# ieellee/uLLSAM

Hardware: AMD Instinct MI355X
Metric: images/s end-to-end (ViT+LLM+mask) 1024^2 (higher is better)
Workload: dtype bf16; 1 GPU; uLLSAM mask path (app.py:580-645): SAM ViT-H + InternLM2-7b-shaped prefill S=1081 + prompt encoder + mask decoder + x4 upsample/threshold, 1 point prompt/image, batch 4/GPU; batch_per_gpu=4, global_batch=4, seq_len=1081, vit_linears=bf16

## Files before the change

### include/ullsam_hip.h

```cpp
#ifndef ULLSAM_HIP_H
#define ULLSAM_HIP_H
#ifdef __cplusplus
extern "C" {
#endif

#define ULLSAM_DT_F32 0
#define ULLSAM_DT_BF16 1
#define ULLSAM_ACT_NONE 0
#define ULLSAM_ACT_GELU 1
#define ULLSAM_ACT_RELU 2
#define ULLSAM_ACT_SWIGLU 3

#define ULLSAM_ABI_VERSION 14

const char* ullsam_last_error_string(void);
int ullsam_abi_version(void);
int ullsam_device_count(void);
int ullsam_set_gemm_variant(int variant);
int ullsam_set_gemm_tuning(int key, int value);
int ullsam_set_attn_variant(int variant);
int ullsam_set_attn_debug(void* stamps);

#define ULLSAM_ACT_SPLITK_OK 256
int ullsam_gemm(int dtype, const void* A, long lda, const void* W, long ldw, void* C, long ldc, int out_f32,
                const float* bias, const float* residual, long ldr, int res_row_mod, int act, int M, int N, int K,
                void* workspace, long ws_bytes, void* stream);

int ullsam_gemm_qkv_rope(int dtype, const void* A, long lda, const void* W, long ldw, const float* bias, int B, int S, int K, int KVH,
                         int G, const int* pos, const float* cos_tab, const float* sin_tab, int tab_rows, void* q_out, void* k_cache,
                         void* v_cache, int cap, int cache_pos0, void* workspace, long ws_bytes, void* stream);

int ullsam_gemm_rmsnorm(const float* x, long ldx, const float* norm_w, float eps, const void* W, long ldw, void* C, long ldc, int out_f32,
                        const float* bias, const float* residual, long ldr, int act, int M, int N, int K, void* stream);
int ullsam_decode_qkv_rope(const void* a, const float* x, long ldx, const float* norm_w, float eps, const void* W, long ldw, const float* bias,
                           int B, int K, int KVH, int G, const int* pos, const float* cos_tab, const float* sin_tab, int tab_rows, void* q_out,
                           void* k_cache, void* v_cache, int cap, int cache_pos0, void* stream);

int ullsam_train_matmul(const float* A, const float* B, float* C, int M, int N, int K, int batch, long a_b, long a_m, long a_k, long b_b,
                        long b_k, long b_n, long c_b, long c_m, long c_n, int accumulate, void* stream);
int ullsam_train_matmul_bf16(const float* A, const float* B, float* C, int M, int N, int K, int batch, long a_b, long a_m, long a_k, long b_b,
                             long b_k, long b_n, long c_b, long c_m, long c_n, int accumulate, void* stream);
int ullsam_train_matmul_heads(const float* A, const float* B, float* C, int M, int N, int K, int outer, int heads, long a_o, long a_h, int a_hdiv, long a_m, long a_k,
                              long b_o, long b_h, int b_hdiv, long b_k, long b_n, long c_o, long c_h, long c_m, long c_n, int accumulate, int bf16, int tri, void* stream);
int ullsam_train_matmul_splitk(const float* A, const float* B, float* C, int M, int N, int K, int batch, long a_b, long a_m, long a_k, long b_b,
                               long b_k, long b_n, long c_b, long c_m, long c_n, int accumulate, int ksplit, float* partial, void* stream);
int ullsam_train_set_matmul_mfma(int on);
int ullsam_train_set_matmul_vec(int on);
int ullsam_train_colsum(const float* x, float* out, long rows, int cols, long ld, float* partial, void* stream);
int ullsam_train_ln_bwd(const float* x, const float* w, const float* dy, float* dx, float* dw, float* db, long rows, int D, float eps, float* ws, void* stream);
int ullsam_train_act(const float* x, const float* dy, float* out, long n, int kind, void* stream);
int ullsam_train_scale_shift(const float* x, const float* s, const float* t, const float* dy, float* out, float* ds, float* dt, long n, float* partial, void* stream);
int ullsam_train_attention(const float* q, const float* k, const float* v, const float* dout, float* out, float* dq, float* dk, float* dv,
                           int B, int H, int groups, int hd, int Sq, int Sk, int causal, const int* key_mask, long q_bs, long q_ts, long q_hs,
                           long k_bs, long k_ts, long k_hs, long v_bs, long v_ts, long v_hs, long o_bs, long o_ts, long o_hs, float scale,
                           const float* bias_h, const float* bias_w, float* dbias_h, float* dbias_w, int kw, void* stream);
int ullsam_train_col2im3x3(const float* dcols, float* dx, int B, int H, int W, int C, void* stream);
int ullsam_train_attn_rows(float* S, float* dP, const float* bias_h, const float* bias_w, float* dbias_h, float* dbias_w, const int* key_mask,
                           int B, int H, int Sq, int Sk, int kw, int causal, int have_p, void* stream);
int ullsam_train_set_rows_reg(int on);
int ullsam_train_rmsnorm_bwd(const float* x, const float* w, const float* dy, float* dx, float* dw_rows, long rows, int D, float eps, void* stream);
int ullsam_train_rope(const float* x, const int* pos, const float* cos_tab, const float* sin_tab, float* out, long tokens, int heads, int hd,
                      int tab_rows, int adjoint, void* stream);
int ullsam_train_swiglu(const float* g, const float* u, const float* dy, float* out, float* dg, float* du, long n, void* stream);
int ullsam_train_resize_bwd(const float* dout, float* din, long planes, int ih, int iw, int oh, int ow, void* stream);
int ullsam_train_seg_loss(const float* x, const float* t, float* sums, float* losses, int P, long npix, float smooth, float* partial, void* stream);
int ullsam_train_seg_loss_bwd(const float* x, const float* t, const float* sums, const float* gscale, float* dx, int P, long npix, float smooth, void* stream);
int ullsam_train_cross_entropy(const float* logits, long ld, const long long* labels, float* lse, float* loss_rows, float* out2, long rows, int V, void* stream);
int ullsam_train_cross_entropy_bwd(const float* logits, long ld, const long long* labels, const float* lse, const float* out2, const float* gscale, float* dlogits,
                                   long ldx, long rows, int V, void* stream);
int ullsam_train_cross_entropy_bwd_bf16(const float* logits, long ld, const long long* labels, const float* lse, const float* out2, const float* gscale,
                                        void* dlog, long ldd, void* dlogT, long ldt, long rows, int V, void* stream);
int ullsam_train_embedding_bwd(const float* dx, long ldx, const int* sorted_ids, const int* order, const int* skip, long rows, int D, int V, int padding_idx,
                               void* table_grad, int out_dtype, void* stream);
int ullsam_train_index_add_rows(const float* src, const int* idx, float* dst, long rows, int C, int nrows_dst, void* stream);

int ullsam_norm(const void* in, int in_dtype, long in_stride, void* out, int out_dtype, long out_stride, const float* w,
                const float* b, long rows, int D, float eps, int rms, int act, const float* post_scale,
                const float* post_shift, void* stream);
int ullsam_set_norm_variant(int v);

int ullsam_norm_fanout(const float* in, long rows, int D, const float* w, const float* b, float eps, float* out_f32, void* out_c,
                       void* out_c_pe, int c_dtype, const float* pe, long pe_rows, void* stream);

int ullsam_vit_attention(int dtype, const void* qkv, void* out, const void* rel_h, const void* rel_w, const void* qkv_bias,
                         int B, int heads, int hd, int grid_h, int grid_w, int window, void* stream);

int ullsam_causal_attention(int dtype, const void* q, const void* k, const void* v, void* out, const int* key_mask, int B,
                            int H, int KVH, int hd, int Sq, int Sk, int k_cap, int q_pos0, void* stream);

int ullsam_naive_attention(int dtype, const void* q, const void* k, const void* v, void* out, const int* key_mask, int B,
                           int H, int KVH, int hd, int Sq, int Sk, long q_bs, long q_ts, long q_hs, long k_bs, long k_ts,
                           long k_hs, long v_bs, long v_ts, long v_hs, long o_bs, long o_ts, long o_hs, float scale,
                           void* stream);

int ullsam_decode_attention(const void* q, const void* kc, const void* vc, const int* key_mask, void* out, int B, int H, int KVH,
                            int hd, int Sk, int cap, float scale, float* workspace, int nsplit, void* stream);

int ullsam_fewkeys_attention(const float* q, const float* k, const float* v, float* out, int B, int H, int hd, int Sq,
                             int Sk, float scale, long q_batch_stride, void* stream);

int ullsam_tok2img_attention(int kv_dtype, const float* q, const void* k, const void* v, float* out, int P, int H, int hd, int T,
                             int N, long k_batch_stride, long v_batch_stride, float scale, float* workspace, int nsplit,
                             void* stream);

int ullsam_patch_im2col(int dtype, const float* pixels, void* out, int B, int C, int Hs, int Ws, int S, int patch,
                        const float* mean, const float* stdv, void* stream);
int ullsam_im2col3x3(int dtype, const void* in, void* out, int B, int H, int W, int C, void* stream);
int ullsam_add_cast(const void* a, int a_dtype, long a_rows, const float* b, long b_rows, void* out, int out_dtype,
                    long rows, int cols, void* stream);
int ullsam_transpose_f32(const float* in, float* out, int B, int R, int C, void* stream);
int ullsam_transpose_to_bf16(int in_dtype, const void* in, void* out, int R, int C, int Rp, void* stream);
int ullsam_cast_transpose_bf16(const float* in, void* out_rm, void* out_t, float* colsum_out, float* colsum_ws, int R, int C, int Rp, void* stream);
int ullsam_pixel_shuffle_ln(int dtype, const float* in_nhwc, void* out, const float* w, const float* b, int B, int H, int W,
// ... 201 lines not shown
```

### ullsam_amd/_lib.py

```python
from __future__ import annotations

import ctypes as C
import os

_HERE = os.path.dirname(os.path.abspath(__file__))
LIB_PATH = os.environ.get("ULLSAM_HIP_LIB") or os.path.join(_HERE, "lib", "libullsam_hip.so")

ABI_VERSION = 14

_lib = None

vp, i32, i64, f32 = C.c_void_p, C.c_int, C.c_long, C.c_float

SIGNATURES = {
    "ullsam_gemm": [i32, vp, i64, vp, i64, vp, i64, i32, vp, vp, i64, i32, i32, i32, i32, i32, vp, i64, vp],
    "ullsam_gemm_qkv_rope": [i32, vp, i64, vp, i64, vp, i32, i32, i32, i32, i32, vp, vp, vp, i32, vp, vp, vp, i32, i32, vp, i64, vp],
    "ullsam_gemm_rmsnorm": [vp, i64, vp, f32, vp, i64, vp, i64, i32, vp, vp, i64, i32, i32, i32, i32, vp],
    "ullsam_decode_qkv_rope": [vp, vp, i64, vp, f32, vp, i64, vp, i32, i32, i32, i32, vp, vp, vp, i32, vp, vp, vp, i32, i32, vp],
    "ullsam_train_matmul": [vp, vp, vp, i32, i32, i32, i32] + [i64] * 9 + [i32, vp],
    "ullsam_train_matmul_bf16": [vp, vp, vp, i32, i32, i32, i32] + [i64] * 9 + [i32, vp],
    "ullsam_train_matmul_splitk": [vp, vp, vp, i32, i32, i32, i32] + [i64] * 9 + [i32, i32, vp, vp],
    "ullsam_train_matmul_heads": [vp, vp, vp, i32, i32, i32, i32, i32, i64, i64, i32, i64, i64, i64, i64, i32, i64, i64, i64, i64, i64, i64, i32, i32, i32, vp],
    "ullsam_train_colsum": [vp, vp, i64, i32, i64, vp, vp],
    "ullsam_train_ln_bwd": [vp, vp, vp, vp, vp, vp, i64, i32, f32, vp, vp],
    "ullsam_train_act": [vp, vp, vp, i64, i32, vp],
    "ullsam_train_scale_shift": [vp, vp, vp, vp, vp, vp, vp, i64, vp, vp],
    "ullsam_train_attention": [vp] * 8 + [i32] * 7 + [vp] + [i64] * 12 + [f32, vp, vp, vp, vp, i32, vp],
    "ullsam_train_col2im3x3": [vp, vp, i32, i32, i32, i32, vp],
    "ullsam_train_attn_rows": [vp, vp, vp, vp, vp, vp, vp, i32, i32, i32, i32, i32, i32, i32, vp],
    "ullsam_train_rmsnorm_bwd": [vp, vp, vp, vp, vp, i64, i32, f32, vp],
    "ullsam_train_rope": [vp, vp, vp, vp, vp, i64, i32, i32, i32, i32, vp],
    "ullsam_train_swiglu": [vp, vp, vp, vp, vp, vp, i64, vp],
    "ullsam_train_resize_bwd": [vp, vp, i64, i32, i32, i32, i32, vp],
    "ullsam_train_seg_loss": [vp, vp, vp, vp, i32, i64, f32, vp, vp],
    "ullsam_train_seg_loss_bwd": [vp, vp, vp, vp, vp, i32, i64, f32, vp],
    "ullsam_train_cross_entropy": [vp, i64, vp, vp, vp, vp, i64, i32, vp],
    "ullsam_train_cross_entropy_bwd": [vp, i64, vp, vp, vp, vp, vp, i64, i64, i32, vp],
    "ullsam_train_cross_entropy_bwd_bf16": [vp, i64, vp, vp, vp, vp, vp, i64, vp, i64, i64, i32, vp],
    "ullsam_train_embedding_bwd": [vp, i64, vp, vp, vp, i64, i32, i32, i32, vp, i32, vp],
    "ullsam_train_index_add_rows": [vp, vp, vp, i64, i32, i32, vp],
    "ullsam_norm": [vp, i32, i64, vp, i32, i64, vp, vp, i64, i32, f32, i32, i32, vp, vp, vp],
    "ullsam_norm_fanout": [vp, i64, i32, vp, vp, f32, vp, vp, vp, i32, vp, i64, vp],
    "ullsam_vit_attention": [i32, vp, vp, vp, vp, vp, i32, i32, i32, i32, i32, i32, vp],
    "ullsam_causal_attention": [i32, vp, vp, vp, vp, vp, i32, i32, i32, i32, i32, i32, i32, i32, vp],
    "ullsam_naive_attention": [i32, vp, vp, vp, vp, vp, i32, i32, i32, i32, i32, i32] + [i64] * 12 + [f32, vp],
    "ullsam_fewkeys_attention": [vp, vp, vp, vp, i32, i32, i32, i32, i32, f32, i64, vp],
    "ullsam_decode_attention": [vp, vp, vp, vp, vp, i32, i32, i32, i32, i32, i32, f32, vp, i32, vp],
    "ullsam_tok2img_attention": [i32, vp, vp, vp, vp, i32, i32, i32, i32, i32, i64, i64, f32, vp, i32, vp],
    "ullsam_patch_im2col": [i32, vp, vp, i32, i32, i32, i32, i32, i32, vp, vp, vp],
    "ullsam_im2col3x3": [i32, vp, vp, i32, i32, i32, i32, vp],
    "ullsam_add_cast": [vp, i32, i64, vp, i64, vp, i32, i64, i32, vp],
    "ullsam_transpose_f32": [vp, vp, i32, i32, i32, vp],
    "ullsam_transpose_to_bf16": [i32, vp, vp, i32, i32, i32, vp],
    "ullsam_cast_transpose_bf16": [vp, vp, vp, vp, vp, i32, i32, i32, vp],
    "ullsam_pixel_shuffle_ln": [i32, vp, vp, vp, vp, i32, i32, i32, i32, f32, vp],
    "ullsam_pixel_unshuffle": [vp, vp, i32, i32, i32, i32, vp],
    "ullsam_scan_image_tokens": [vp, vp, vp, i32, i32, C.c_longlong, vp],
    "ullsam_embed_tokens": [i32, vp, vp, vp, vp, vp, i32, i32, i32, i32, i64, vp],
    "ullsam_gather_rows": [vp, vp, vp, i32, i32, i32, i32, vp],
    "ullsam_rope_split": [i32, vp, vp, vp, vp, vp, vp, vp, i32, i32, i32, i32, i32, i32, i32, i32, vp],
    "ullsam_argmax": [vp, vp, i32, i64, i64, vp],
    "ullsam_sample_topk_topp": [vp, vp, i32, i64, i64, f32, i32, f32, vp, C.c_ulonglong, vp, vp, vp, vp, vp],
    "ullsam_small_linear": [vp, i64, vp, vp, vp, i64, vp, i64, i32, i32, i32, i32, vp],
    "ullsam_i2t_block": [vp, i64, vp, i64, vp, vp, vp, vp, vp, vp, vp, vp, f32, vp, i64, vp, vp, vp, i32, i32, i32, f32, vp],
    "ullsam_kv_proj": [vp, vp, vp, vp, vp, vp, vp, vp, i64, vp],
    "ullsam_up2_hyper_masks": [vp, vp, vp, vp, vp, i32, i32, i32, i32, vp],
    "ullsam_dec_tok_attn": [vp] * 14 + [f32, vp, vp, i32, i32, i32, i32, vp],
    "ullsam_dec_tok_mlp": [vp] * 10 + [f32] + [vp] * 6 + [f32] + [vp] * 4 + [i32, i32, i32, vp],
    "ullsam_dec_heads": [vp, vp, vp, vp, vp, i32, i32, i32, i32, i32, vp],
    "ullsam_concat_token_rows": [vp, i32, vp, i32, vp, i32, i32, vp],
    "ullsam_up1_ln_gelu": [vp, vp, vp, vp, vp, f32, vp, i64, vp],
    "ullsam_skinny_linear": [vp, i64, vp, vp, vp, i64, vp, i64, i32, i32, i32, i32, vp],
    "ullsam_sparse_embed": [vp, vp, vp, vp, vp, vp, i32, i32, i32, i32, f32, f32, vp],
    "ullsam_dense_pe": [vp, vp, i32, i32, i32, vp],
    "ullsam_mask_downscale": [vp, vp, i32, i32, i32, i32, i32, i32] + [vp] * 10 + [vp],
    "ullsam_hyper_masks": [i32, vp, vp, vp, i32, i32, i32, i32, i32, vp],
    "ullsam_resize_bilinear": [vp, i64, i32, i32, i32, vp, vp, i32, i32, i32, f32, vp],
    "ullsam_mask_iou_counts": [vp, vp, vp, i32, i64, vp],
    "ullsam_stability_score": [vp, i64, i64, f32, f32, vp, vp, vp],
    "ullsam_mask_to_box": [vp, i64, i32, i32, vp, vp],
    "ullsam_rle_pack": [vp, i64, i32, i32, vp, vp, vp, vp],
    "ullsam_rle_emit": [vp, vp, i64, i32, i32, vp, vp, vp],
    "ullsam_amg_postprocess": [vp, vp, i64] + [i32] * 11 + [f32, f32, vp, vp, vp, vp, vp, vp],
    "ullsam_nms_mask": [vp, i32, f32, vp, vp],
    "ullsam_threshold_u8": [vp, vp, i64, f32, vp],
    "ullsam_rle_to_mask": [vp, vp, i64, i32, i32, vp, vp, vp],
    "ullsam_label_regions": [vp, i64, i32, i32, i32, vp, vp],
    "ullsam_remove_small_regions": [vp, vp, i64, i32, i32, i32, i32, vp, i64, vp, vp],
    "ullsam_rle_paint_labels": [vp, vp, vp, i64, i32, i32, vp, vp, vp],
    "ullsam_label_stats": [vp, i64, i32, i32, vp, vp, vp],
    "ullsam_label_compact": [vp, vp, vp, i64, i32, vp, vp, vp, vp, vp, vp],
    "ullsam_label_remap": [vp, vp, i64, i32, i32, vp, vp],
    "ullsam_label_overlap": [vp, vp, i32, i32, i32, i32, vp, vp, vp],
    "ullsam_resize_nearest_i32": [vp, i64, i32, i32, i32, i32, i32, i32, i32, i32, vp, i64, vp],
    "ullsam_mosaic_seams": [vp, i32, i32, i32, vp, i64, vp, i32, i32, vp, vp, i64, i32, vp, vp, vp],
    "ullsam_mosaic_union": [vp, vp, i64, vp, i64, i64, i64, vp, vp, vp],
    "ullsam_mosaic_stats": [vp, i32, i32, i32, vp, i64, vp, i32, vp, i32, i32, vp, vp, vp, vp],
    "ullsam_mosaic_compact": [vp, vp, vp, i64, i32, vp, vp, vp, vp, vp],
    "ullsam_mosaic_paste": [vp, i32, i32, i32, vp, i64, vp, i32, vp, i32, i32, vp, vp],
# ... 95 lines not shown
```

### ullsam_amd/csrc/gemm.hip

```cpp
#include "common.h"
#include <type_traits>

struct GemmArgs {
    const void* A;
    const void* W;
    void* C;
    const float* bias;
    const float* residual;
    int M, N, K;
    long lda, ldw, ldc, ldr;
    int res_row_mod;
    int act;
    int out_f32;
    int vec_ok;
    int tiles_m, tiles_n;
    int full_tiles, ksplit;
    float* ws;
    size_t ws_bytes;
    const int* rope_pos; const float* rope_cos; const float* rope_sin; void* rope_q; void* rope_k; void* rope_v;
    int rope_S, rope_KVH, rope_G, rope_cap, rope_pos0, rope_rows;
    const float* row_scale;
    const float* col_scale;
    unsigned long long* dbg;
    const float* norm_x; const float* norm_w; float norm_eps; long ldx;
    int group_m;
};

#ifndef ULLSAM_RING_ASM_DMA
#define ULLSAM_RING_ASM_DMA 1
#endif
static constexpr bool g_asm_dma = ULLSAM_RING_ASM_DMA != 0;
static int g_split_tail = 1;
static int g_gemm_variant = 0;
static int g_dbg = 0;
static int g_auto_mask = 7;
static int g_group_m = 4;

template <typename T>
__device__ __forceinline__ Frag<T> lds_frag(const char* tile, int row, int ks, int g);
template <>
__device__ __forceinline__ Frag<bf16> lds_frag<bf16>(const char* tile, int row, int ks, int g) {
    const int c = (ks * 4 + g) ^ (row & 7);
    return load_frag(reinterpret_cast<const bf16*>(tile + row * 128 + (c << 4)));
}
template <>
__device__ __forceinline__ Frag<float> lds_frag<float>(const char* tile, int row, int ks, int g) {
    (void)ks;
    const int c0 = (2 * g) ^ (row & 7), c1 = (2 * g + 1) ^ (row & 7);
    const float4 a = *reinterpret_cast<const float4*>(tile + row * 128 + (c0 << 4));
    const float4 b = *reinterpret_cast<const float4*>(tile + row * 128 + (c1 << 4));
    Frag<float> f;
    f.v[0] = a.x; f.v[1] = a.y; f.v[2] = a.z; f.v[3] = a.w;
    f.v[4] = b.x; f.v[5] = b.y; f.v[6] = b.z; f.v[7] = b.w;
    return f;
}

template <typename OutT>
__device__ __forceinline__ void store_row8(OutT* dst, const float* v, int n_valid, bool vec);
template <>
__device__ __forceinline__ void store_row8<float>(float* dst, const float* v, int n_valid, bool vec) {
    if (vec && n_valid == 8) {
        *reinterpret_cast<float4*>(dst) = make_float4(v[0], v[1], v[2], v[3]);
        *reinterpret_cast<float4*>(dst + 4) = make_float4(v[4], v[5], v[6], v[7]);
    } else {
        for (int e = 0; e < n_valid; ++e) dst[e] = v[e];
    }
}
template <>
__device__ __forceinline__ void store_row8<bf16>(bf16* dst, const float* v, int n_valid, bool vec) {
    if (vec && n_valid == 8) {
        bf16x8_t o;
#pragma unroll
        for (int e = 0; e < 8; ++e) o[e] = (bf16)v[e];
        *reinterpret_cast<bf16x8_t*>(dst) = o;
    } else {
        for (int e = 0; e < n_valid; ++e) dst[e] = (bf16)v[e];
    }
}


template <typename T, typename OutT, int BM, int NTHREADS, int BN = 128, int EMODE = 0, bool RING16 = false>
__device__ __forceinline__ void epilogue_rows(const GemmArgs& p, const float* Cs, int m0, int n0, int tn, int tid) {
    constexpr int TPR = BN / 8;
    constexpr int RPP = NTHREADS / TPR;
    constexpr int PASSES = (BM + RPP - 1) / RPP;
    constexpr bool RAGGED = BM % RPP != 0;
    static_assert(NTHREADS % TPR == 0, "threads per pass must cover whole rows");
    if (RAGGED && tid >= NTHREADS) return;
    OutT* C = reinterpret_cast<OutT*>(p.C);
    if (p.act == 3) {
#pragma unroll
        for (int pass = 0; pass < PASSES; ++pass) {
            const int row = pass * RPP + tid / TPR;
            const int t = tid % TPR;
            const int grp = t >> 4, j0 = (t & 15) * 4;
            const int gm = m0 + row;
            if (gm >= p.M) continue;
            const float4 g = *reinterpret_cast<const float4*>(Cs + row * BN + grp * 128 + j0);
            const float4 u = *reinterpret_cast<const float4*>(Cs + row * BN + grp * 128 + 64 + j0);
            float4 o;
            if constexpr (RING16) {
                o = make_float4(g.x * __builtin_amdgcn_rcpf(1.0f + __expf(-g.x)) * u.x, g.y * __builtin_amdgcn_rcpf(1.0f + __expf(-g.y)) * u.y,
                                g.z * __builtin_amdgcn_rcpf(1.0f + __expf(-g.z)) * u.z, g.w * __builtin_amdgcn_rcpf(1.0f + __expf(-g.w)) * u.w);
            } else {
                o = make_float4(silu_f(g.x) * u.x, silu_f(g.y) * u.y, silu_f(g.z) * u.z, silu_f(g.w) * u.w);
            }
            OutT* dst = C + (size_t)gm * p.ldc + (size_t)tn * (BN / 2) + grp * 64 + j0;
// ... 491 lines not shown
#pragma unroll
    for (int e = 0; e < 4; ++e) { first[e] = odd ? recv[e] : lo[e]; second[e] = odd ? hi[e] : recv[e]; }
}

template <typename T, int EMODE = 0>
static int launch_gemm_v3_impl(GemmArgs a, hipStream_t stream) {
    static PerDeviceOnce attr_set;
    if (attr_set.first()) {
        (void)hipFuncSetAttribute(reinterpret_cast<const void*>(gemm256_kernel<T, EMODE>), hipFuncAttributeMaxDynamicSharedMemorySize, 131072);
    }
    a.tiles_m = (a.M + 255) / 256;
    a.tiles_n = (a.N + 255) / 256;
    const int T_ = a.tiles_m * a.tiles_n;
    const int nk = a.K / (128 / (int)sizeof(T));
    const int tail = T_ % 256;
    a.full_tiles = T_;
    a.ksplit = 1;
    if (g_split_tail && a.ws && T_ > 256 && tail > 0 && tail <= 64 && nk >= 64) {
        int S = 256 / tail;
        if (S > 8) S = 8;
        if (S > nk / 8) S = nk / 8;
        if (S >= 2 && (size_t)tail * S * 262144 <= a.ws_bytes) {
            a.full_tiles = T_ - tail;
            a.ksplit = S;
        }
    }
    gemm256_kernel<T, EMODE><<<dim3(a.full_tiles + (T_ - a.full_tiles) * a.ksplit), dim3(512), 131072, stream>>>(a);
    ULLSAM_LAUNCH_CHECK();
    if (a.ksplit > 1) {
        const int tail_tiles = T_ - a.full_tiles;
        if (tail_tiles * a.ksplit <= 128) gemm256_tail_reduce_kernel<T, 4, 128, EMODE><<<dim3(tail_tiles * 64), dim3(128), 0, stream>>>(a);
        else gemm256_tail_reduce_kernel<T, 16, 256, EMODE><<<dim3(tail_tiles * 16), dim3(256), 0, stream>>>(a);
        ULLSAM_LAUNCH_CHECK();
    }
    return 0;
}
template <typename T>
static int launch_gemm_v3(GemmArgs a, hipStream_t stream) {
    if (a.act == 4) return launch_gemm_v3_impl<T, 1>(a, stream);
    return launch_gemm_v3_impl<T, 0>(a, stream);
}

__device__ __forceinline__ void glds16_sbase(const char* base, unsigned int off, unsigned int lds_addr) {
    unsigned int keep;
    asm volatile("s_mov_b32 %0, m0\n\ts_mov_b32 m0, %3\n\ts_nop 0\n\tglobal_load_lds_dwordx4 %1, %2\n\ts_mov_b32 m0, %0"
                 : "=&s"(keep) : "v"(off), "s"(base), "s"(lds_addr) : "memory");
}

template <int MI0, int MI1, int NTW, bool STAMP = false, int EMODE = 0>
__global__ __launch_bounds__(512) void gemm_ring8_kernel(GemmArgs p) {
    extern __shared__ __attribute__((aligned(16))) char smem[];
    const unsigned long long t_entry = STAMP ? __builtin_amdgcn_s_memtime() : 0ull;
    typedef bf16 T;
    constexpr int BM = 16 * (MI0 + MI1), BN = 64 * NTW, MI = MI0 > MI1 ? MI0 : MI1;
    constexpr int PA = BM / 16, PB = BN / 16;
    constexpr int ASZ = BM * 64, STG = ASZ + BN * 64;
    static_assert(PA >= 8 && PA <= 24 && PB >= 8 && PB <= 24, "piece assignment below: one to three pieces per wave and operand");
    if constexpr (EMODE == 2) {
        p.K /= (int)gridDim.y;
        p.A = reinterpret_cast<const char*>(p.A) + (size_t)blockIdx.y * p.K * 2;
        p.W = reinterpret_cast<const char*>(p.W) + (size_t)blockIdx.y * p.K * 2;
        p.C = reinterpret_cast<float*>(p.C) + (size_t)blockIdx.y * p.M * p.ldc;
    }

    const int nblk = p.full_tiles;
    const int bid = blockIdx.x;
    const int q8 = nblk >> 3, r8 = nblk & 7, xcd = bid & 7;
    const int swz = (xcd < r8 ? xcd * (q8 + 1) : r8 * (q8 + 1) + (xcd - r8) * q8) + (bid >> 3);
    const int GM = p.group_m;
    const int width = GM * p.tiles_n;
    const int group = swz / width;
    const int first_m = group * GM;
    const int gsize = min(p.tiles_m - first_m, GM);
    const int tm = first_m + (swz % width) % gsize;
    const int tn = (swz % width) / gsize;
    const int m0 = tm * BM, n0 = tn * BN;

    const int tid = threadIdx.x, lane = tid & 63;
    const int wave = __builtin_amdgcn_readfirstlane(tid >> 6);
    const int wm = wave >> 2, wn = wave & 3, grp = wave >> 2;
    const int g4 = lane >> 4, mm = lane & 15;

    const char* a_base = reinterpret_cast<const char*>(p.A) + (size_t)m0 * p.lda * 2;
    const char* b_base = reinterpret_cast<const char*>(p.W) + (size_t)n0 * p.ldw * 2;
    const int na = (PA - wave + 7) / 8, nb = (PB - wave + 7) / 8;
    static_assert(NTW == 4 || NTW == 5, "epilogue layouts below: four sub-tiles in two pairs, optionally a fifth on its own");
    constexpr int WW = 16 * NTW;
    const int perm = EMODE == 1 ? 2 : p.out_f32 ? 0 : (p.act == 3 ? 2 : 1);
    auto w_row = [&](int R) {
        const int wb = R / WW, q = R - wb * WW, j = q >> 4, r = q & 15;
        if (perm == 1) return j < 4 ? WW * wb + 32 * (j >> 1) + 8 * (r >> 2) + 4 * (j & 1) + (r & 3) : WW * wb + 64 + r;
        if (perm == 2) return 128 * (wb >> 1) + 64 * (j >> 1) + 32 * (wb & 1) + 8 * (r >> 2) + 4 * (j & 1) + (r & 3);
        return R;
    };
    unsigned int a_off[3], b_off[3];
#pragma unroll
    for (int i = 0; i < 3; ++i) {
        const int row = (wave + 8 * i) * 16 + (lane >> 2);
        const int c = (lane & 3) ^ ((row >> 2) & 2);
        a_off[i] = (unsigned int)((size_t)(min(m0 + row, p.M - 1) - m0) * p.lda * 2) + (c << 4);
        b_off[i] = (unsigned int)((size_t)(min(n0 + w_row(row), p.N - 1) - n0) * p.ldw * 2) + (c << 4);
    }
    const int st1 = p.K >> 5;

    const int mi = wm == 0 ? MI0 : MI1;
    const int row_w = wm == 0 ? 0 : MI0 * 16;
    f32x4 acc[MI][NTW];
#pragma unroll
    for (int i = 0; i < MI; ++i)
#pragma unroll
        for (int j = 0; j < NTW; ++j) acc[i][j] = (f32x4){0.f, 0.f, 0.f, 0.f};

    auto stage = [&](int s) {
        char* base = smem + (s & 3) * STG;
        const char* ak = a_base + (size_t)s * 64;
        const char* bk = b_base + (size_t)s * 64;
#pragma unroll
        for (int i = 0; i < 3; ++i) {
            if (i < na) __builtin_amdgcn_global_load_lds(GLB_PTR(ak + a_off[i]), LDS_PTR(base + (wave + 8 * i) * 1024), 16, 0, 0);
            if (i < nb) __builtin_amdgcn_global_load_lds(GLB_PTR(bk + b_off[i]), LDS_PTR(base + ASZ + (wave + 8 * i) * 1024), 16, 0, 0);
        }
    };
    auto frag = [&](const char* tile, int row) -> Frag<T> {
        return load_frag(reinterpret_cast<const T*>(tile + row * 64 + ((g4 ^ ((row >> 2) & 2)) << 4)));
    };
    const int npc = na + nb;
    auto wait_one_left = [&]() {
        if (npc == 4) asm volatile("s_waitcnt vmcnt(4)" ::: "memory");
        else if (npc == 2) asm volatile("s_waitcnt vmcnt(2)" ::: "memory");
        else if (npc == 5) asm volatile("s_waitcnt vmcnt(5)" ::: "memory");
        else if (npc == 6) asm volatile("s_waitcnt vmcnt(6)" ::: "memory");
        else asm volatile("s_waitcnt vmcnt(3)" ::: "memory");
    };

    const bool has_bias = p.bias && p.act != 3 && EMODE == 0;
    char* const bias_lds = smem + (st1 & 3) * STG;
    auto bias_dma = [&]() __attribute__((always_inline)) {
        if (has_bias && wave < (BN * 4 + 1023) / 1024) {
            const int c = min(n0 + wave * 256 + lane * 4, p.N - 4);
            __builtin_amdgcn_global_load_lds(GLB_PTR(p.bias + c), LDS_PTR(bias_lds + wave * 1024), 16, 0, 0);
        }
    };
    stage(0);
    if (1 < st1) { stage(1); wait_one_left(); }
    else asm volatile("s_waitcnt vmcnt(0)" ::: "memory");
    __builtin_amdgcn_s_barrier();
    if (grp == 1) __builtin_amdgcn_s_barrier();
    auto stamp = [&](int kk) {
        if (STAMP && p.dbg && (tid & 255) == 0) p.dbg[((size_t)bid * 2 + grp) * 4 + kk] = __builtin_amdgcn_s_memtime();
    };
    auto stamp16 = [&](int kk) {
        if (STAMP && p.dbg && (tid & 255) == 0) p.dbg[(1 << 19) + ((size_t)bid * 2 + grp) * 8 + kk] = __builtin_amdgcn_s_memtime();
    };
    stamp(0);
    {
        auto body = [&](int s, auto NA_c, auto NB_c, auto MORE_c) __attribute__((always_inline)) {
            constexpr int NA = decltype(NA_c)::value, NB = decltype(NB_c)::value;
            constexpr bool MORE = decltype(MORE_c)::value;
            const char* Ab = smem + (s & 3) * STG;
            const char* Bb = Ab + ASZ;
            Frag<T> a8[MI], b[NTW];
            {
                char* base = smem + ((s + 2) & 3) * STG;
                const char* ak = a_base + (size_t)(s + 2) * 64;
                const char* bk = b_base + (size_t)(s + 2) * 64;
                auto request = [&](int qi) __attribute__((always_inline)) {
                    const int i = qi >> 1;
                    if (g_asm_dma) {
                        if (MORE && !(qi & 1) && i < NA) glds16_sbase(ak, a_off[i], (unsigned int)(uintptr_t)LDS_PTR(base + (wave + 8 * i) * 1024));
                        if (MORE && (qi & 1) && i < NB) glds16_sbase(bk, b_off[i], (unsigned int)(uintptr_t)LDS_PTR(base + ASZ + (wave + 8 * i) * 1024));
                    } else {
                        if (MORE && !(qi & 1) && i < NA) __builtin_amdgcn_global_load_lds(GLB_PTR(ak + a_off[i]), LDS_PTR(base + (wave + 8 * i) * 1024), 16, 0, 0);
                        if (MORE && (qi & 1) && i < NB) __builtin_amdgcn_global_load_lds(GLB_PTR(bk + b_off[i]), LDS_PTR(base + ASZ + (wave + 8 * i) * 1024), 16, 0, 0);
                    }
                    __builtin_amdgcn_sched_barrier(0);
                };
                int qi = 0;
                request(qi++);
#pragma unroll
                for (int r = 0; r < NTW + MI; ++r) {
                    if (r < NTW) b[r] = frag(Bb, wn * (16 * NTW) + r * 16 + mm);
                    else if ((r - NTW) < MI1 || (r - NTW) < mi) a8[r - NTW] = frag(Ab, row_w + (r - NTW) * 16 + mm);
                    __builtin_amdgcn_sched_barrier(0);
                    if ((r % 3) == 2 && qi < 6) request(qi++);
                }
#pragma unroll
                for (; qi < 6; ++qi) request(qi);
            }
            if constexpr (!MORE) asm volatile("s_waitcnt vmcnt(0)" ::: "memory");
            else if constexpr (NA + NB == 4) asm volatile("s_waitcnt vmcnt(4)" ::: "memory");
            else if constexpr (NA + NB == 5) asm volatile("s_waitcnt vmcnt(5)" ::: "memory");
            else if constexpr (NA + NB == 6) asm volatile("s_waitcnt vmcnt(6)" ::: "memory");
            else if constexpr (NA + NB == 3) asm volatile("s_waitcnt vmcnt(3)" ::: "memory");
            else asm volatile("s_waitcnt vmcnt(2)" ::: "memory");
            __builtin_amdgcn_sched_barrier(0);
            __builtin_amdgcn_s_barrier();
            __builtin_amdgcn_s_setprio(1);
#pragma unroll
            for (int i = 0; i < MI; ++i)
                if (i < MI1 || i < mi) {
#pragma unroll
                    for (int j = 0; j < NTW; ++j) mma16(b[j], a8[i], acc[i][j]);
                }
            __builtin_amdgcn_s_setprio(0);
            __builtin_amdgcn_sched_barrier(0);
            __builtin_amdgcn_s_barrier();
        };
        auto run = [&](auto NA_c, auto NB_c) __attribute__((always_inline)) {
            int s = 0;
            for (; s + 2 < st1; ++s) body(s, NA_c, NB_c, std::true_type{});
            bias_dma();
            for (; s < st1; ++s) body(s, NA_c, NB_c, std::false_type{});
        };
        constexpr int NA_LO = PA / 8, NA_HI = (PA + 7) / 8, NB_LO = PB / 8, NB_HI = (PB + 7) / 8;
        if (NA_HI != NA_LO && na == NA_HI) {
            if (NB_HI != NB_LO && nb == NB_HI) run(std::integral_constant<int, NA_HI>{}, std::integral_constant<int, NB_HI>{});
            else run(std::integral_constant<int, NA_HI>{}, std::integral_constant<int, NB_LO>{});
        } else {
            if (NB_HI != NB_LO && nb == NB_HI) run(std::integral_constant<int, NA_LO>{}, std::integral_constant<int, NB_HI>{});
            else run(std::integral_constant<int, NA_LO>{}, std::integral_constant<int, NB_LO>{});
        }
    }
    if (grp == 0) __builtin_amdgcn_s_barrier();
    stamp(1);
    float bv[4 * NTW];
#pragma unroll
    for (int e = 0; e < 4 * NTW; ++e) bv[e] = 0.f;
    if (has_bias) {
#pragma unroll
        for (int t = 0; t < NTW; ++t) {
            const int col = wn * WW + ((p.out_f32 || t == 4) ? 16 * t + 4 * g4 : 32 * (t >> 1) + 8 * g4 + 4 * (t & 1));
            const float4 x = *reinterpret_cast<const float4*>(bias_lds + col * 4);
            bv[4 * t] = x.x; bv[4 * t + 1] = x.y; bv[4 * t + 2] = x.z; bv[4 * t + 3] = x.w;
        }
    }

    {
        const bool odd = mm & 1;
        const int row0 = m0 + row_w + mm;
        const int rowp = row0 & ~1;
        const bool direct = p.vec_ok && (p.N & 7) == 0 && (p.M & 1) == 0 && (p.out_f32 || !p.residual);
        auto gst = [&](void* ptr, u32x4 v) __attribute__((always_inline)) { *reinterpret_cast<u32x4*>(ptr) = v; };
        if constexpr (EMODE == 1) {
            const int slot = (n0 >> 7) + (wn >> 1), d = 32 * (wn & 1) + 8 * g4;
            const int gs = p.rope_G + 2, kv = slot / gs, g = slot - kv * gs;
            const bool live = slot < p.rope_KVH * gs;
            const bool rotate = g != gs - 1;
            float bl[8], bh[8];
// ... 172 lines not shown
                if (perm == 1) return j < 4 ? WW * wn + 32 * (j >> 1) + 8 * g4 + 4 * (j & 1) : WW * wn + 64 + 4 * g4;
                if (perm == 2) return 128 * (wn >> 1) + 64 * (j >> 1) + 32 * (wn & 1) + 8 * g4 + 4 * (j & 1);
                return WW * wn + 16 * j + 4 * g4;
            };
            auto staged = [&](auto half_c) __attribute__((always_inline)) {
                constexpr int half = decltype(half_c)::value;
                constexpr int ROWS = 16 * (half == 0 ? MI0 : MI1);
                constexpr int NT_E = (512 / (BN / 8)) * (BN / 8);
                __syncthreads();
                if (wm == half) {
#pragma unroll
                    for (int i = 0; i < (half == 0 ? MI0 : MI1); ++i)
#pragma unroll
                        for (int j = 0; j < NTW; ++j)
                            *reinterpret_cast<float4*>(Cs + (i * 16 + mm) * BN + ncol(j)) = make_float4(acc[i][j][0], acc[i][j][1], acc[i][j][2], acc[i][j][3]);
                }
                __syncthreads();
                if (p.out_f32) epilogue_rows<T, float, ROWS, NT_E, BN>(p, Cs, m0 + half * 16 * MI0, n0, tn, tid);
                else epilogue_rows<T, T, ROWS, NT_E, BN, 0, true>(p, Cs, m0 + half * 16 * MI0, n0, tn, tid);
            };
            staged(std::integral_constant<int, 0>{});
            staged(std::integral_constant<int, 1>{});
        }
    }
    stamp(2);
    if (STAMP && p.dbg && (tid & 255) == 0) p.dbg[((size_t)bid * 2 + grp) * 4 + 3] = t_entry;
}

template <int MI0, int MI1, int NTW, int EMODE = 0>
static int launch_gemm_ring8(GemmArgs a, hipStream_t stream) {
    constexpr int BM = 16 * (MI0 + MI1), BN = 64 * NTW;
    constexpr int LDS = (4 * (BM + BN) * 64 > 16 * MI0 * BN * 4) ? 4 * (BM + BN) * 64 : 16 * MI0 * BN * 4;
    static_assert(LDS <= 163840, "160 KiB of LDS per CU");
    static PerDeviceOnce attr_set;
    if (attr_set.first()) {
        (void)hipFuncSetAttribute(reinterpret_cast<const void*>(gemm_ring8_kernel<MI0, MI1, NTW, false, EMODE>), hipFuncAttributeMaxDynamicSharedMemorySize, LDS);
        if constexpr (EMODE == 0) (void)hipFuncSetAttribute(reinterpret_cast<const void*>(gemm_ring8_kernel<MI0, MI1, NTW, true>), hipFuncAttributeMaxDynamicSharedMemorySize, LDS);
    }
    a.tiles_m = (a.M + BM - 1) / BM;
    a.tiles_n = (a.N + BN - 1) / BN;
    a.full_tiles = a.tiles_m * a.tiles_n;
    a.ksplit = 1;
    if constexpr (EMODE == 0) {
        if (a.dbg) {
            gemm_ring8_kernel<MI0, MI1, NTW, true><<<dim3(a.full_tiles), dim3(512), LDS, stream>>>(a);
            ULLSAM_LAUNCH_CHECK();
            return 0;
        }
    }
    gemm_ring8_kernel<MI0, MI1, NTW, false, EMODE><<<dim3(a.full_tiles), dim3(512), LDS, stream>>>(a);
    ULLSAM_LAUNCH_CHECK();
    return 0;
}
template <typename TO>
__global__ __launch_bounds__(256) void splitk_finish_kernel(const float* __restrict__ ws, TO* __restrict__ C, long ldc, const float* __restrict__ bias,
                                                            const float* __restrict__ residual, long ldr, int res_row_mod, int M, int N, int S) {
    const long q = (long)blockIdx.x * 256 + threadIdx.x, nq = N >> 2;
    if (q >= (long)M * nq) return;
    const int m = (int)(q / nq), c = (int)(q - (long)m * nq) * 4;
    const size_t plane = (size_t)M * N;
    const float* src = ws + (size_t)m * N + c;
    float4 v[8];
#pragma unroll
    for (int k = 0; k < 8; ++k) if (k < S) v[k] = *reinterpret_cast<const float4*>(src + k * plane);
    float4 s = v[0];
#pragma unroll
    for (int k = 1; k < 8; ++k) if (k < S) { s.x += v[k].x; s.y += v[k].y; s.z += v[k].z; s.w += v[k].w; }
    if (bias) { const float4 b = *reinterpret_cast<const float4*>(bias + c); s.x += b.x; s.y += b.y; s.z += b.z; s.w += b.w; }
    if (residual) {
        const int rr = res_row_mod > 0 ? m % res_row_mod : m;
        const float4 r = *reinterpret_cast<const float4*>(residual + (size_t)rr * ldr + c);
        s.x += r.x; s.y += r.y; s.z += r.z; s.w += r.w;
    }
    if constexpr (sizeof(TO) == 4) *reinterpret_cast<float4*>(C + (size_t)m * ldc + c) = s;
    else *reinterpret_cast<uint2*>(C + (size_t)m * ldc + c) = make_uint2(pack_bf16x2(s.x, s.y), pack_bf16x2(s.z, s.w));
}
template <int MI0, int MI1, int NTW>
static int launch_gemm_ring_splitk(const GemmArgs& a, int S, hipStream_t stream) {
    constexpr int BM = 16 * (MI0 + MI1), BN = 64 * NTW;
    constexpr int LDS = (4 * (BM + BN) * 64 > 16 * MI0 * BN * 4) ? 4 * (BM + BN) * 64 : 16 * MI0 * BN * 4;
    static PerDeviceOnce attr_set;
    if (attr_set.first()) (void)hipFuncSetAttribute(reinterpret_cast<const void*>(gemm_ring8_kernel<MI0, MI1, NTW, false, 2>), hipFuncAttributeMaxDynamicSharedMemorySize, LDS);
    GemmArgs b = a;
    b.C = a.ws; b.ldc = a.N; b.out_f32 = 1; b.bias = nullptr; b.residual = nullptr; b.act = 0; b.vec_ok = 1; b.dbg = nullptr;
    b.tiles_m = (a.M + BM - 1) / BM;
    b.tiles_n = (a.N + BN - 1) / BN;
    b.full_tiles = b.tiles_m * b.tiles_n;
    b.ksplit = 1;
    gemm_ring8_kernel<MI0, MI1, NTW, false, 2><<<dim3(b.full_tiles, S), dim3(512), LDS, stream>>>(b);
    ULLSAM_LAUNCH_CHECK();
    const long quads = (long)a.M * (a.N >> 2);
    if (a.out_f32) splitk_finish_kernel<float><<<dim3((unsigned)((quads + 255) / 256)), 256, 0, stream>>>(a.ws, static_cast<float*>(a.C), a.ldc, a.bias, a.residual, a.ldr, a.res_row_mod, a.M, a.N, S);
    else splitk_finish_kernel<bf16><<<dim3((unsigned)((quads + 255) / 256)), 256, 0, stream>>>(a.ws, static_cast<bf16*>(a.C), a.ldc, a.bias, a.residual, a.ldr, a.res_row_mod, a.M, a.N, S);
    ULLSAM_LAUNCH_CHECK();
    return 0;
}
static int g_ring_splitk = 1;
static int ring_splitk_plan(const GemmArgs& a, int* shape) {
    if (a.act != 0 || !a.vec_ok || !a.ws || (a.N & 7) != 0 || a.M < 1024 || a.N < 256 || a.dbg) return 0;
    const long t272 = (long)((a.M + 271) / 272) * ((a.N + 255) / 256), t256 = (long)((a.M + 255) / 256) * ((a.N + 255) / 256);
    const long t320 = a.N % 320 == 0 ? (long)((a.M + 255) / 256) * (a.N / 320) : 1l << 40;
    const double a272 = 1.0625 * t272, a256 = 1.0 * t256, a320 = 1.25 * t320;
    long t; if (a320 <= a272 && a320 <= a256) { t = t320; *shape = 8; } else if (a272 < a256) { t = t272; *shape = 9; } else { t = t256; *shape = 6; }
    if (t > 128) return 0;
    int S = (int)(256 / t); if (S > 8) S = 8;
    while (S >= 2 && (a.K % (64 * S) != 0 || a.K / S < 1280 || (size_t)S * a.M * a.N * 4 > a.ws_bytes)) --S;
    return (S >= 2 && S * t >= 224) ? S : 0;
}
#include "gemm_ring8p.h"
static int g_persist = 2;
static int cu_count() {
    static int n[32] = {};
    int d = 0;
    (void)hipGetDevice(&d);
    d &= 31;
    if (!n[d]) { int v = 0; if (hipDeviceGetAttribute(&v, hipDeviceAttributeMultiprocessorCount, d) != hipSuccess || v <= 0) v = 256; n[d] = v; }
    return n[d];
}
template <int BM, int BN, int NTW, int EMODE>
static bool ring_persist_ok(const GemmArgs& a) {
    if (!g_persist || a.N % BN != 0 || a.K % 128 != 0 || a.K < 384 || (a.dbg && !(g_dbg & 2))) return false;
    const long tiles = (long)((a.M + BM - 1) / BM) * (a.N / BN);
    if (tiles <= cu_count()) return false;
    if (((size_t)(a.M + BM) * a.lda + a.K) * 2 >= (1ull << 32) || ((size_t)a.N * a.ldw + a.K) * 2 >= (1ull << 32)) return false;
    if (EMODE == 1) return true;
    if (!(a.vec_ok && (a.N & 7) == 0 && (a.M & 1) == 0)) return false;
    if (!a.out_f32) return !a.residual && (a.act != 3 || NTW == 4);
    return a.act == 0;
}
template <int MI0, int MI1, int NTW, int EMODE = 0>
static int launch_ring(const GemmArgs& a, hipStream_t stream) {
    return ring_persist_ok<16 * (MI0 + MI1), 64 * NTW, NTW, EMODE>(a) ? launch_gemm_ring8p<MI0, MI1, NTW, EMODE>(a, stream, cu_count())
                                                                      : launch_gemm_ring8<MI0, MI1, NTW, EMODE>(a, stream);
}
static int launch_gemm_v6(const GemmArgs& a, hipStream_t stream) { return launch_ring<8, 8, 4>(a, stream); }
static int launch_gemm_v8(const GemmArgs& a, hipStream_t stream) { return launch_ring<8, 8, 5>(a, stream); }
static int launch_gemm_v9(const GemmArgs& a, hipStream_t stream) { return launch_ring<9, 8, 4>(a, stream); }
static int launch_gemm_ring_rope(const GemmArgs& a, hipStream_t stream, int force) {
    auto cost = [&](int bm) { const long t = (long)((a.M + bm - 1) / bm) * ((a.N + 255) / 256); return (double)((t + 255) / 256) * bm / 256.0; };
    const double c208 = cost(208), c256 = cost(256), c272 = cost(272);
    int pick = (c208 < c256 && c208 < c272) ? 208 : (c272 < c256 ? 272 : 256);
    if (force) pick = force;
    if (pick == 208) return launch_ring<7, 6, 4, 1>(a, stream);
    if (pick == 272) return launch_ring<9, 8, 4, 1>(a, stream);
    return launch_ring<8, 8, 4, 1>(a, stream);
}

typedef __attribute__((ext_vector_type(8))) int i32x8;
__device__ __forceinline__ int f8_swz(int row) { return (row & 6) | ((row >> 3) & 1); }
__device__ __forceinline__ i32x8 lds_frag8(const char* tile, int row, int g) {
    const int f = f8_swz(row);
    const int4 lo = *reinterpret_cast<const int4*>(tile + row * 128 + (((2 * g) ^ f) << 4));
    const int4 hi = *reinterpret_cast<const int4*>(tile + row * 128 + (((2 * g + 1) ^ f) << 4));
    return (i32x8){lo.x, lo.y, lo.z, lo.w, hi.x, hi.y, hi.z, hi.w};
}
__global__ __launch_bounds__(512) void gemm256f8_kernel(GemmArgs p) {
    extern __shared__ __attribute__((aligned(16))) char smem[];
    constexpr int STAGE = 65536;
    const int nblk = p.tiles_m * p.tiles_n;
    const int bid = blockIdx.x;
    const int q8 = nblk >> 3, r8 = nblk & 7, xcd = bid & 7;
    const int swz = (xcd < r8 ? xcd * (q8 + 1) : r8 * (q8 + 1) + (xcd - r8) * q8) + (bid >> 3);
    const int GM = 4;
    const int width = GM * p.tiles_n;
    const int group = swz / width;
    const int first_m = group * GM;
    const int gsize = min(p.tiles_m - first_m, GM);
    const int tm = first_m + (swz % width) % gsize;
    const int tn = (swz % width) / gsize;
    const int m0 = tm * 256, n0 = tn * 256;
    const int tid = threadIdx.x, lane = tid & 63;
    const int wave = __builtin_amdgcn_readfirstlane(tid >> 6);
    const int wm = wave >> 2, wn = wave & 3, grp = wave >> 2;
    const int g4 = lane >> 4, mm = lane & 15;

    const char* a_base = reinterpret_cast<const char*>(p.A) + (size_t)m0 * p.lda;
    const char* b_base = reinterpret_cast<const char*>(p.W) + (size_t)n0 * p.ldw;
    unsigned int a_off[4], b_off[4];
#pragma unroll
    for (int i = 0; i < 4; ++i) {
        const int row = (wave * 4 + i) * 8 + (lane >> 3);
        const int c = (lane & 7) ^ f8_swz(row);
        a_off[i] = (unsigned int)((size_t)(min(m0 + row, p.M - 1) - m0) * p.lda) + (c << 4);
        b_off[i] = (unsigned int)((size_t)(min(n0 + row, p.N - 1) - n0) * p.ldw) + (c << 4);
    }
    const int nk = p.K >> 7;
    f32x4 acc[8][4];
#pragma unroll
    for (int i = 0; i < 8; ++i)
#pragma unroll
        for (int j = 0; j < 4; ++j) acc[i][j] = (f32x4){0.f, 0.f, 0.f, 0.f};
    auto stage = [&](int buf, int kt) {
        char* base = smem + buf * STAGE;
        const char* ak = a_base + (size_t)kt * 128;
        const char* bk = b_base + (size_t)kt * 128;
#pragma unroll
        for (int i = 0; i < 4; ++i) {
            __builtin_amdgcn_global_load_lds(GLB_PTR(ak + a_off[i]), LDS_PTR(base + (wave * 4 + i) * 1024), 16, 0, 0);
            __builtin_amdgcn_global_load_lds(GLB_PTR(bk + b_off[i]), LDS_PTR(base + 32768 + (wave * 4 + i) * 1024), 16, 0, 0);
        }
    };
    const int one = 0x7f7f7f7f;
    stage(0, 0);
    asm volatile("s_waitcnt vmcnt(0)" ::: "memory");
    __builtin_amdgcn_s_barrier();
    if (grp == 1) __builtin_amdgcn_s_barrier();
    for (int kt = 0; kt < nk; ++kt) {
        const char* Ab = smem + (kt & 1) * STAGE;
        const char* Bb = Ab + 32768;
        i32x8 a[4], b[4];
        if (kt + 1 < nk) stage((kt + 1) & 1, kt + 1);
#pragma unroll
        for (int j = 0; j < 4; ++j) b[j] = lds_frag8(Bb, wn * 64 + j * 16 + mm, g4);
#pragma unroll
        for (int i = 0; i < 4; ++i) a[i] = lds_frag8(Ab, wm * 128 + i * 16 + mm, g4);
        __builtin_amdgcn_sched_barrier(0);
        __builtin_amdgcn_s_barrier();
        __builtin_amdgcn_s_setprio(1);
#pragma unroll
        for (int i = 0; i < 4; ++i)
#pragma unroll
            for (int j = 0; j < 4; ++j) acc[i][j] = __builtin_amdgcn_mfma_scale_f32_16x16x128_f8f6f4(a[i], b[j], acc[i][j], 0, 0, 0, one, 0, one);
        __builtin_amdgcn_s_setprio(0);
        __builtin_amdgcn_sched_barrier(0);
        __builtin_amdgcn_s_barrier();
#pragma unroll
        for (int i = 0; i < 4; ++i) a[i] = lds_frag8(Ab, wm * 128 + (4 + i) * 16 + mm, g4);
        asm volatile("s_waitcnt vmcnt(0)" ::: "memory");
        __builtin_amdgcn_sched_barrier(0);
        __builtin_amdgcn_s_barrier();
        __builtin_amdgcn_s_setprio(1);
#pragma unroll
        for (int i = 0; i < 4; ++i)
#pragma unroll
            for (int j = 0; j < 4; ++j) acc[4 + i][j] = __builtin_amdgcn_mfma_scale_f32_16x16x128_f8f6f4(a[i], b[j], acc[4 + i][j], 0, 0, 0, one, 0, one);
        __builtin_amdgcn_s_setprio(0);
        __builtin_amdgcn_sched_barrier(0);
        __builtin_amdgcn_s_barrier();
    }
    if (grp == 0) __builtin_amdgcn_s_barrier();

    float* Cs = reinterpret_cast<float*>(smem);
#pragma unroll
    for (int half = 0; half < 2; ++half) {
        __syncthreads();
        if (wm == half) {
#pragma unroll
            for (int i = 0; i < 8; ++i)
#pragma unroll
                for (int j = 0; j < 4; ++j)
#pragma unroll
                    for (int r = 0; r < 4; ++r) Cs[(i * 16 + 4 * g4 + r) * 256 + wn * 64 + j * 16 + mm] = acc[i][j][r];
        }
        __syncthreads();
        if (p.out_f32) epilogue_rows<bf16, float, 128, 512, 256, 2>(p, Cs, m0 + half * 128, n0, tn, tid);
        else epilogue_rows<bf16, bf16, 128, 512, 256, 2>(p, Cs, m0 + half * 128, n0, tn, tid);
    }
}

extern "C" int ullsam_gemm_fp8(const void* A8, long lda, const float* a_scale, const void* W8, long ldw, const float* w_scale, void* C,
                               long ldc, int out_f32, const float* bias, const float* residual, long ldr, int act, int M, int N, int K,
                               void* stream) {
    ULLSAM_CHECK(M > 0 && N > 0 && K > 0 && K % 128 == 0, "ullsam_gemm_fp8: K=%d must be a positive multiple of 128", K);
    ULLSAM_CHECK(((uintptr_t)A8 & 15) == 0 && ((uintptr_t)W8 & 15) == 0 && lda % 16 == 0 && ldw % 16 == 0, "ullsam_gemm_fp8: 16-byte aligned rows needed");
    ULLSAM_CHECK(a_scale && w_scale, "ullsam_gemm_fp8: scales are required");
    ULLSAM_CHECK(act >= 0 && act <= 2, "ullsam_gemm_fp8: bad act %d", act);
    GemmArgs a;
    a.A = A8; a.W = W8; a.C = C; a.bias = bias; a.residual = residual;
    a.M = M; a.N = N; a.K = K; a.lda = lda; a.ldw = ldw; a.ldc = ldc; a.ldr = ldr;
    a.res_row_mod = 0; a.act = act; a.out_f32 = out_f32;
    const int osz = out_f32 ? 4 : 2;
    bool vec = ((uintptr_t)C & 15) == 0 && (ldc * osz) % 16 == 0 && (N % 8 == 0);
    if (residual) vec = vec && ((uintptr_t)residual & 15) == 0 && (ldr % 4 == 0);
    a.group_m = 4;
    a.vec_ok = vec ? 1 : 0;
    a.ws = nullptr; a.ws_bytes = 0; a.ksplit = 1;
    a.row_scale = a_scale; a.col_scale = w_scale; a.dbg = nullptr;
    a.tiles_m = (M + 255) / 256; a.tiles_n = (N + 255) / 256; a.full_tiles = a.tiles_m * a.tiles_n;
    static PerDeviceOnce attr_set;
    if (attr_set.first()) (void)hipFuncSetAttribute(reinterpret_cast<const void*>(gemm256f8_kernel), hipFuncAttributeMaxDynamicSharedMemorySize, 131072);
    gemm256f8_kernel<<<dim3(a.full_tiles), dim3(512), 131072, reinterpret_cast<hipStream_t>(stream)>>>(a);
    ULLSAM_LAUNCH_CHECK();
    return 0;
}

extern "C" int ullsam_set_gemm_tuning(int key, int value) {
    if (key == 0 && value >= 1 && value <= 1024) { g_group_m = value; return 0; }
    if (key == 1 && value >= 0 && value <= 7) { g_auto_mask = value; return 0; }
    if (key == 2 && (value == 0 || value == 2)) { g_persist = value; return 0; }
    if (key == 3 && value >= 0 && value <= 2) { g_ring_splitk = value; return 0; }
    ullsam_set_error("ullsam_set_gemm_tuning: unknown key %d / bad value %d", key, value);
    return -1;
}
extern "C" int ullsam_set_gemm_variant(int v) {
    g_gemm_variant = v & 15; g_split_tail = (v & 64) ? 0 : 1; g_dbg = (v >> 15) & 3;
    return 0;
}

template <typename T, int EMODE = 0>
static int launch_gemm(GemmArgs a, hipStream_t stream) {
    static PerDeviceOnce attr_set;
    if (attr_set.first()) {
        (void)hipFuncSetAttribute(reinterpret_cast<const void*>(gemm128_kernel<T, EMODE>), hipFuncAttributeMaxDynamicSharedMemorySize, 65536);
    }
    const int T_ = a.tiles_m * a.tiles_n;
    const int C_ = 512;
    a.full_tiles = T_;
    a.ksplit = 1;
    const int nk = a.K / (128 / (int)sizeof(T));
    const int tail = T_ % C_;
    if (g_split_tail && a.ws && T_ > C_ && tail > 0 && tail <= C_ / 2 && nk >= 128) {
        int S = C_ / tail;
        if (S > 16) S = 16;
        if (S > nk / 4) S = nk / 4;
        if (S >= 2 && (size_t)tail * S * 65536 <= a.ws_bytes) {
            a.full_tiles = T_ - tail;
            a.ksplit = S;
        }
    }
    const int grid = a.full_tiles + (T_ - a.full_tiles) * a.ksplit;
    gemm128_kernel<T, EMODE><<<dim3(grid), dim3(256), 65536, stream>>>(a);
    ULLSAM_LAUNCH_CHECK();
    if (a.ksplit > 1) {
        gemm_tail_reduce_kernel<T, EMODE><<<dim3((T_ - a.full_tiles) * 4), dim3(256), 0, stream>>>(a);
        ULLSAM_LAUNCH_CHECK();
    }
    return 0;
}

#ifndef ULLSAM_SKINNY_NT
#define ULLSAM_SKINNY_NT 1
#endif
__device__ __forceinline__ uint4 load_w16(const bf16* ptr) {
#if ULLSAM_SKINNY_NT
    const u32x4 v = __builtin_nontemporal_load(reinterpret_cast<const u32x4*>(ptr));
    return make_uint4(v[0], v[1], v[2], v[3]);
#else
    return *reinterpret_cast<const uint4*>(ptr);
#endif
}
template <bool W8> struct SkinnyW { using elem = bf16; using vec = uint4; };
template <> struct SkinnyW<true> { using elem = unsigned char; using vec = uint2; };
__device__ __forceinline__ uint2 load_w16(const unsigned char* ptr) {
#if ULLSAM_SKINNY_NT
    const u32x2 v = __builtin_nontemporal_load(reinterpret_cast<const u32x2*>(ptr));
    return make_uint2(v[0], v[1]);
#else
    return *reinterpret_cast<const uint2*>(ptr);
#endif
}
__device__ __forceinline__ uint4 widen_w(const uint4 w) { return w; }
__device__ __forceinline__ uint4 widen_w(const uint2 w) {
    typedef __bf16 bf16x2_t __attribute__((ext_vector_type(2)));
    uint4 o;
    o.x = __builtin_bit_cast(unsigned int, (bf16x2_t)__builtin_amdgcn_cvt_scalef32_pk_bf16_fp8(w.x, 1.0f, false));
    o.y = __builtin_bit_cast(unsigned int, (bf16x2_t)__builtin_amdgcn_cvt_scalef32_pk_bf16_fp8(w.x, 1.0f, true));
    o.z = __builtin_bit_cast(unsigned int, (bf16x2_t)__builtin_amdgcn_cvt_scalef32_pk_bf16_fp8(w.y, 1.0f, false));
    o.w = __builtin_bit_cast(unsigned int, (bf16x2_t)__builtin_amdgcn_cvt_scalef32_pk_bf16_fp8(w.y, 1.0f, true));
    return o;
}

__device__ __forceinline__ void bf16x8_to_f32(const uint4 u, float (&o)[8]) {
    const unsigned int d[4] = {u.x, u.y, u.z, u.w};
#pragma unroll
    for (int j = 0; j < 4; ++j) { o[2 * j] = __uint_as_float(d[j] << 16); o[2 * j + 1] = __uint_as_float(d[j] & 0xffff0000u); }
}
__device__ __forceinline__ void dot2c(float& acc, const unsigned int a, const unsigned int b) {
    asm("v_dot2c_f32_bf16 %0, %1, %2" : "+v"(acc) : "v"(a), "v"(b));
}
__device__ __forceinline__ void dot_fence() { asm volatile("s_nop 4" ::: "memory"); }
template <int NV>
__device__ __forceinline__ float wave_sum_many(float (&v)[NV]) {
    static_assert(NV == 16 || NV == 32, "");
// ... 386 lines not shown
        const int gs = p.rope_G + 2, kv = slot / gs, g = slot - kv * gs;
        const int b = m / p.rope_S, sq = m - b * p.rope_S;
        bf16* dst;
        float o1 = x1, o2 = x2;
        if (g == gs - 1) {
            dst = reinterpret_cast<bf16*>(p.rope_v) + (((long)b * p.rope_KVH + kv) * p.rope_cap + p.rope_pos0 + sq) * 128;
        } else {
            const int ps = min(max(p.rope_pos[m], 0), p.rope_rows - 1);
            const float* cp = p.rope_cos + (size_t)ps * 128 + d;
            const float* sp = p.rope_sin + (size_t)ps * 128 + d;
            o1 = x1 * cp[0] - x2 * sp[0];
            o2 = x2 * cp[64] + x1 * sp[64];
            dst = g == gs - 2 ? reinterpret_cast<bf16*>(p.rope_k) + (((long)b * p.rope_KVH + kv) * p.rope_cap + p.rope_pos0 + sq) * 128
                              : reinterpret_cast<bf16*>(p.rope_q) + (long)m * ((long)p.rope_KVH * p.rope_G * 128) + ((long)kv * p.rope_G + g) * 128;
        }
        dst[d] = (bf16)o1;
        dst[d + 64] = (bf16)o2;
        return;
    }
    const long n = n0 + r;
    if (n >= p.N) return;
    float v = total(tid, n);
    if (p.bias) v += p.bias[n];
    if (p.act == 1) v = gelu_erf(v);
    else if (p.act == 2) v = fmaxf(v, 0.f);
    if (p.residual) v += p.residual[(size_t)(p.res_row_mod > 0 ? m % p.res_row_mod : m) * p.ldr + n];
    if (p.out_f32) reinterpret_cast<float*>(p.C)[(size_t)m * p.ldc + n] = v;
    else reinterpret_cast<bf16*>(p.C)[(size_t)m * p.ldc + n] = (bf16)v;
}

template <bool W8 = false>
static int launch_gemm_skinny(const GemmArgs& a, hipStream_t stream) {
    const bool normed = a.norm_x != nullptr;
    if (normed && (a.M > 4 || a.K > 4096 || a.K % 2048 != 0 || a.ldx % 4 != 0)) { ullsam_set_error("skinny GEMM: the fused RMSNorm prologue needs M <= 4, K <= 4096, K %% 2048 == 0 (M=%d K=%d)", a.M, a.K); return -1; }
    if (a.act == 4 && (a.M > 4 || a.K % 2048 != 0 || a.N % 128 != 0)) { ullsam_set_error("skinny GEMM: the RoPE epilogue needs M <= 4, K %% 2048 == 0 (M=%d K=%d)", a.M, a.K); return -1; }
    if (a.act == 4 || (a.act != 3 && a.N <= 8192 && a.K % 2048 == 0)) {
        const dim3 g4((unsigned)((a.N + 3) / 4)), g8((unsigned)((a.N + 7) / 8));
        const size_t lds = normed ? (size_t)4 * a.K * 2 : 0;
        if (normed) gemm_skinny_ksplit_kernel<4, 8, true, W8><<<g8, 256, lds, stream>>>(a);
        else if (a.act == 4) gemm_skinny_ksplit_kernel<4, 8, false, W8><<<g8, 256, 0, stream>>>(a);
        else if (a.M > 4) gemm_skinny_ksplit_kernel<8, 4, false, W8><<<g4, 256, 0, stream>>>(a);
        else gemm_skinny_ksplit_kernel<4, 8, false, W8><<<g8, 256, 0, stream>>>(a);
        ULLSAM_LAUNCH_CHECK();
        return 0;
    }
    const int MM = a.M <= 4 ? 4 : 8;
    const size_t lds = (size_t)MM * a.K * 2;
    const long waves = a.act == 3 ? (long)a.N / 4 : ((long)a.N + 3) / 4;
    if (MM == 4 && (normed || a.act == 3) && waves >= 4096 && lds + 256 <= 64 * 1024) {
        static PerDeviceOnce cu_once; static int n_cu = 256;
        if (cu_once.first()) { int dev = 0; hipDeviceProp_t pr; if (hipGetDevice(&dev) == hipSuccess && hipGetDeviceProperties(&pr, dev) == hipSuccess && pr.multiProcessorCount > 0) n_cu = pr.multiProcessorCount; }
        const int n_wg = n_cu * 2;
        int W = 8; double best = 1e30;
        for (int w = 8; w >= 4; --w) {
            const long per = (long)n_wg * w, trips = (waves + per - 1) / per;
            const double waste = (double)(trips * per) / (double)waves;
            if (waste < best - 1e-9) { best = waste; W = w; }
        }
        if (normed) gemm_skinny_persist_kernel<true, W8><<<n_wg, W * 64, lds, stream>>>(a, (int)waves);
        else gemm_skinny_persist_kernel<false, W8><<<n_wg, W * 64, lds, stream>>>(a, (int)waves);
        ULLSAM_LAUNCH_CHECK();
        return 0;
    }
    const dim3 grid((unsigned)((waves + 3) / 4));
    static PerDeviceOnce attr4, attr8;
    if (normed) {
        gemm_skinny_kernel<4, true, W8><<<grid, 256, lds, stream>>>(a);
    } else if (MM == 4) {
        if (attr4.first()) { (void)hipFuncSetAttribute(reinterpret_cast<const void*>(gemm_skinny_kernel<4, false, W8>), hipFuncAttributeMaxDynamicSharedMemorySize, 159 * 1024); }
        gemm_skinny_kernel<4, false, W8><<<grid, 256, lds, stream>>>(a);
    } else {
        if (attr8.first()) { (void)hipFuncSetAttribute(reinterpret_cast<const void*>(gemm_skinny_kernel<8, false, W8>), hipFuncAttributeMaxDynamicSharedMemorySize, 159 * 1024); }
        gemm_skinny_kernel<8, false, W8><<<grid, 256, lds, stream>>>(a);
    }
    ULLSAM_LAUNCH_CHECK();
    return 0;
}

struct RopeEpilogue { const int* pos; const float* cos; const float* sin; void* q; void* k; void* v; int S, KVH, G, cap, pos0, rows; };
struct NormPrologue { const float* x; long ldx; const float* w; float eps; };

static int gemm_impl(int dtype, const void* A, long lda, const void* W, long ldw, void* C, long ldc, int out_f32,
                     const float* bias, const float* residual, long ldr, int res_row_mod, int act, int M, int N,
                     int K, void* workspace, long ws_bytes, void* stream, const RopeEpilogue* rope, const NormPrologue* norm = nullptr) {
    ULLSAM_CHECK(dtype == ULLSAM_DT_F32 || dtype == ULLSAM_DT_BF16, "ullsam_gemm: bad dtype %d", dtype);
    ULLSAM_CHECK(M > 0 && N > 0 && K > 0, "ullsam_gemm: empty problem M=%d N=%d K=%d", M, N, K);
    const int esz = dtype == ULLSAM_DT_F32 ? 4 : 2;
    const int bk = 128 / esz;
    ULLSAM_CHECK(K % bk == 0, "ullsam_gemm: K=%d must be a multiple of %d", K, bk);
    ULLSAM_CHECK(((uintptr_t)A & 15) == 0 && ((uintptr_t)W & 15) == 0, "ullsam_gemm: A/W must be 16-byte aligned");
    ULLSAM_CHECK((lda * esz) % 16 == 0 && (ldw * esz) % 16 == 0, "ullsam_gemm: lda/ldw rows must be 16-byte multiples");
    const bool split_ok = (act & 256) != 0;
    act &= 255;
    ULLSAM_CHECK(act >= 0 && act <= 4 && (act == 4) == (rope != nullptr), "ullsam_gemm: bad act %d", act);
    if (act == 3) ULLSAM_CHECK(N % 128 == 0 && !bias && !residual, "ullsam_gemm: swiglu needs N%%128==0, no bias/residual");
    GemmArgs a;
    a.rope_pos = nullptr; a.rope_cos = a.rope_sin = nullptr; a.rope_q = a.rope_k = a.rope_v = nullptr;
    a.rope_S = a.rope_KVH = a.rope_G = a.rope_cap = a.rope_pos0 = a.rope_rows = 0;
    if (rope) {
        a.rope_pos = rope->pos; a.rope_cos = rope->cos; a.rope_sin = rope->sin; a.rope_q = rope->q; a.rope_k = rope->k; a.rope_v = rope->v;
        a.rope_S = rope->S; a.rope_KVH = rope->KVH; a.rope_G = rope->G; a.rope_cap = rope->cap; a.rope_pos0 = rope->pos0; a.rope_rows = rope->rows;
    }
    a.norm_x = nullptr; a.norm_w = nullptr; a.norm_eps = 0.f; a.ldx = 0;
    if (norm) {
        ULLSAM_CHECK(norm->x && norm->w && ((uintptr_t)norm->x & 15) == 0 && ((uintptr_t)norm->w & 15) == 0 && norm->ldx % 4 == 0,
                     "ullsam_gemm: the RMSNorm prologue needs 16-byte aligned fp32 rows and weight");
        a.norm_x = norm->x; a.norm_w = norm->w; a.norm_eps = norm->eps; a.ldx = norm->ldx;
    }
    a.A = A; a.W = W; a.C = C; a.bias = bias; a.residual = residual;
    a.M = M; a.N = N; a.K = K;
    a.lda = lda; a.ldw = ldw; a.ldc = ldc; a.ldr = ldr;
    a.res_row_mod = res_row_mod; a.act = act; a.out_f32 = out_f32;
    const int osz = out_f32 ? 4 : esz;
    const int n_out = act == 3 ? N / 2 : N;
    bool vec = ((uintptr_t)C & 15) == 0 && (ldc * osz) % 16 == 0 && (n_out % 8 == 0);
    if (residual) vec = vec && ((uintptr_t)residual & 15) == 0 && (ldr % 4 == 0);
    a.vec_ok = vec ? 1 : 0;
    a.ws = reinterpret_cast<float*>(workspace);
    a.ws_bytes = workspace ? (size_t)ws_bytes : 0;
    a.group_m = g_group_m;
    a.row_scale = nullptr;
    a.col_scale = nullptr;
    a.dbg = (g_dbg && workspace && ws_bytes >= (56l << 20)) ? reinterpret_cast<unsigned long long*>(reinterpret_cast<char*>(workspace) + (48l << 20)) : nullptr;
    a.ksplit = 1;
    a.tiles_m = (M + 127) / 128;
    a.tiles_n = (N + 127) / 128;
    a.full_tiles = a.tiles_m * a.tiles_n;
    hipStream_t s = reinterpret_cast<hipStream_t>(stream);
    const int variant = g_gemm_variant;
    if ((variant == 0 || norm) && (act != 4 || (M <= 4 && K % 2048 == 0)) && dtype == ULLSAM_DT_BF16 && M <= 8 && K % 512 == 0 && lda % 8 == 0 && ldw % 8 == 0 &&
        (size_t)(M <= 4 ? 4 : 8) * K * 2 <= 144 * 1024 && (act != 3 || N % 128 == 0))
        return launch_gemm_skinny<false>(a, s);
    ULLSAM_CHECK(!norm, "ullsam_gemm: the RMSNorm prologue exists in the decode-step kernels only (bf16, M <= 4, K <= 4096; got M=%d K=%d)", M, K);
    const long t256 = (long)((M + 255) / 256) * ((N + 255) / 256);
    const double fill = (double)t256 / (double)(((t256 + 255) / 256) * 256);
    const long tail256 = t256 % 256;
    const bool v3_split = g_split_tail && workspace && t256 > 256 && tail256 > 0 && tail256 <= 64 && K >= 64 * bk;
    const bool big = M >= 1024 && N >= 256 && K >= 8 * bk && (act != 3 || N % 256 == 0);
    const bool bias_v4 = !bias || (N % 4 == 0 && ((uintptr_t)bias & 15) == 0);
    const bool ring_ok = dtype == ULLSAM_DT_BF16 && act <= 3 && K % 64 == 0 && K >= 128 && bias_v4 && (act != 3 || N % 256 == 0);
    if (act == 4 && dtype == ULLSAM_DT_BF16 && M >= 1024 && K % 64 == 0 && K >= 256 && (variant == 0 || variant == 6 || variant == 9 || variant == 10) &&
        (((uintptr_t)rope->q | (uintptr_t)rope->k | (uintptr_t)rope->v) & 15) == 0 && (!bias || ((uintptr_t)bias & 15) == 0))
        return launch_gemm_ring_rope(a, s, variant == 6 ? 256 : variant == 9 ? 272 : variant == 10 ? 208 : 0);
    if (variant == 6 || variant == 8 || variant == 9) {
        if (!ring_ok || (variant == 8 && act == 3)) { ullsam_set_error("ullsam_gemm: the ring kernels need bf16, K %% 64 == 0, K >= 128, no RoPE epilogue (256x320: no SwiGLU)"); return -1; }
        return variant == 6 ? launch_gemm_v6(a, s) : variant == 8 ? launch_gemm_v8(a, s) : launch_gemm_v9(a, s);
    }
    if (variant == 1) return a.act == 4 ? (dtype == ULLSAM_DT_F32 ? launch_gemm<float, 1>(a, s) : launch_gemm<bf16, 1>(a, s))
                                        : (dtype == ULLSAM_DT_F32 ? launch_gemm<float>(a, s) : launch_gemm<bf16>(a, s));
    if (variant == 3) {
        if (act == 3 && N % 256 != 0) { ullsam_set_error("ullsam_gemm: the 256x256 kernel's SwiGLU epilogue needs N %% 256 == 0"); return -1; }
        return dtype == ULLSAM_DT_F32 ? launch_gemm_v3<float>(a, s) : launch_gemm_v3<bf16>(a, s);
    }
    if (ring_ok && variant == 0 && (g_ring_splitk == 2 || (g_ring_splitk == 1 && split_ok))) {
        int shape = 0;
        const int S = ring_splitk_plan(a, &shape);
        if (S) return shape == 8 ? launch_gemm_ring_splitk<8, 8, 5>(a, S, s) : shape == 9 ? launch_gemm_ring_splitk<9, 8, 4>(a, S, s) : launch_gemm_ring_splitk<8, 8, 4>(a, S, s);
    }
    if (ring_ok && M >= 1024 && N >= 256 && K >= 256) {
        const double c256 = v3_split ? (double)(t256 / 256) + 0.5 : (double)((t256 + 255) / 256);
        const long t320 = (long)((M + 255) / 256) * (N / 320), t272 = (long)((M + 271) / 272) * ((N + 255) / 256);
        const double c320 = (N % 320 == 0 && act != 3 && (g_auto_mask & 2)) ? 1.25 * (double)((t320 + 255) / 256) : 1e9;
        const double c272 = (g_auto_mask & 4) ? 1.0625 * (double)((t272 + 255) / 256) : 1e9;
        if (c320 <= 0.96 * c256 || (act == 1 && c320 <= c256)) return launch_gemm_v8(a, s);
        if (c272 <= 0.96 * c256) return launch_gemm_v9(a, s);
        if ((g_auto_mask & 1) && big && fill >= 0.74 && !v3_split) return launch_gemm_v6(a, s);
    }
    const bool v3 = big && (fill >= 0.74 || v3_split);
    if (v3) return dtype == ULLSAM_DT_F32 ? launch_gemm_v3<float>(a, s) : launch_gemm_v3<bf16>(a, s);
    if (a.act == 4) return dtype == ULLSAM_DT_F32 ? launch_gemm<float, 1>(a, s) : launch_gemm<bf16, 1>(a, s);
    return dtype == ULLSAM_DT_F32 ? launch_gemm<float>(a, s) : launch_gemm<bf16>(a, s);
}

extern "C" int ullsam_gemm(int dtype, const void* A, long lda, const void* W, long ldw, void* C, long ldc, int out_f32,
                           const float* bias, const float* residual, long ldr, int res_row_mod, int act, int M, int N,
                           int K, void* workspace, long ws_bytes, void* stream) {
    ULLSAM_CHECK(act != 4, "ullsam_gemm: act 4 is ullsam_gemm_qkv_rope");
    return gemm_impl(dtype, A, lda, W, ldw, C, ldc, out_f32, bias, residual, ldr, res_row_mod, act, M, N, K, workspace, ws_bytes, stream, nullptr);
}

extern "C" int ullsam_gemm_rmsnorm(const float* x, long ldx, const float* norm_w, float eps, const void* W, long ldw, void* C, long ldc,
                                   int out_f32, const float* bias, const float* residual, long ldr, int act, int M, int N, int K, void* stream) {
    ULLSAM_CHECK(act != 4, "ullsam_gemm_rmsnorm: act 4 is ullsam_decode_qkv_rope");
    NormPrologue n{x, ldx, norm_w, eps};
    return gemm_impl(ULLSAM_DT_BF16, nullptr, K, W, ldw, C, ldc, out_f32, bias, residual, ldr, 0, act, M, N, K, nullptr, 0, stream, nullptr, &n);
}

extern "C" int ullsam_decode_qkv_rope(const void* a, const float* x, long ldx, const float* norm_w, float eps, const void* W, long ldw,
                                      const float* bias, int B, int K, int KVH, int G, const int* pos, const float* cos_tab,
                                      const float* sin_tab, int tab_rows, void* q_out, void* k_cache, void* v_cache, int cap, int cache_pos0,
                                      void* stream) {
    ULLSAM_CHECK(B > 0 && B <= 4 && KVH > 0 && G > 0 && tab_rows > 0 && K % 2048 == 0, "ullsam_decode_qkv_rope: B=%d (1..4) K=%d (%% 2048)", B, K);
    ULLSAM_CHECK(cache_pos0 + 1 <= cap, "ullsam_decode_qkv_rope: cache overflow (%d + 1 > %d)", cache_pos0, cap);
    RopeEpilogue r{pos, cos_tab, sin_tab, q_out, k_cache, v_cache, 1, KVH, G, cap, cache_pos0, tab_rows};
    NormPrologue n{x, ldx, norm_w, eps};
    const int N = KVH * (G + 2) * 128;
    return gemm_impl(ULLSAM_DT_BF16, norm_w ? nullptr : a, K, W, ldw, q_out, (long)KVH * G * 128, 0, bias, nullptr, 0, 0, 4, B, N, K, nullptr, 0,
                     stream, &r, norm_w ? &n : nullptr);
}

static int gemm_w8_impl(const char* who, const void* A, const NormPrologue* norm, const void* W8, long ldw, const float* w_scale, void* C, long ldc, int out_f32,
                        const float* bias, const float* residual, long ldr, int act, int M, int N, int K, void* stream, const RopeEpilogue* rope) {
    ULLSAM_CHECK(W8 && w_scale && C, "%s: null weights, scales or output", who);
    ULLSAM_CHECK(M > 0 && M <= 8 && N > 0 && K > 0 && K % 512 == 0, "%s: decode-step shapes only (1 <= M <= 8, K %% 512 == 0; got M=%d N=%d K=%d)", who, M, N, K);
    ULLSAM_CHECK((size_t)(M <= 4 ? 4 : 8) * K * 2 <= 144 * 1024, "%s: K=%d: the activation rows do not fit the LDS", who, K);
    ULLSAM_CHECK(act >= 0 && act <= 4 && (act == 4) == (rope != nullptr), "%s: bad act %d", who, act);
    ULLSAM_CHECK(((uintptr_t)W8 & 7) == 0 && ldw % 8 == 0 && ldw >= K, "%s: weight rows must be 8-byte aligned (ldw=%ld)", who, ldw);
    if (act == 3) ULLSAM_CHECK(N % 128 == 0 && !bias && !residual, "%s: swiglu needs N %% 128 == 0, no bias / residual", who);
    GemmArgs a{};
    if (rope) {
        a.rope_pos = rope->pos; a.rope_cos = rope->cos; a.rope_sin = rope->sin; a.rope_q = rope->q; a.rope_k = rope->k; a.rope_v = rope->v;
        a.rope_S = rope->S; a.rope_KVH = rope->KVH; a.rope_G = rope->G; a.rope_cap = rope->cap; a.rope_pos0 = rope->pos0; a.rope_rows = rope->rows;
    }
    if (norm) {
        ULLSAM_CHECK(norm->x && norm->w && ((uintptr_t)norm->x & 15) == 0 && ((uintptr_t)norm->w & 15) == 0 && norm->ldx % 4 == 0,
                     "%s: the RMSNorm prologue needs 16-byte aligned fp32 rows and weight", who);
        a.norm_x = norm->x; a.norm_w = norm->w; a.norm_eps = norm->eps; a.ldx = norm->ldx;
    } else {
        ULLSAM_CHECK(A && ((uintptr_t)A & 15) == 0, "%s: bf16 activations must be 16-byte aligned", who);
    }
    a.A = A; a.W = W8; a.C = C; a.bias = bias; a.residual = residual; a.col_scale = w_scale;
    a.M = M; a.N = N; a.K = K;
    a.lda = K; a.ldw = ldw; a.ldc = ldc; a.ldr = ldr;
    a.act = act; a.out_f32 = out_f32;
    a.group_m = g_group_m; a.ksplit = 1;
    return launch_gemm_skinny<true>(a, reinterpret_cast<hipStream_t>(stream));
}

extern "C" int ullsam_gemm_w8(const void* A, const float* x, long ldx, const float* norm_w, float eps, const void* W8, long ldw, const float* w_scale,
                              void* C, long ldc, int out_f32, const float* bias, const float* residual, long ldr, int act, int M, int N, int K,
                              void* stream) {
    ULLSAM_CHECK(act != 4, "ullsam_gemm_w8: act 4 is ullsam_decode_qkv_rope_w8");
    NormPrologue n{x, ldx, norm_w, eps};
    return gemm_w8_impl("ullsam_gemm_w8", norm_w ? nullptr : A, norm_w ? &n : nullptr, W8, ldw, w_scale, C, ldc, out_f32, bias, residual, ldr, act, M, N, K, stream, nullptr);
}

extern "C" int ullsam_decode_qkv_rope_w8(const void* a, const float* x, long ldx, const float* norm_w, float eps, const void* W8, long ldw,
                                         const float* w_scale, const float* bias, int B, int K, int KVH, int G, const int* pos, const float* cos_tab,
                                         const float* sin_tab, int tab_rows, void* q_out, void* k_cache, void* v_cache, int cap, int cache_pos0,
                                         void* stream) {
    ULLSAM_CHECK(B > 0 && B <= 4 && KVH > 0 && G > 0 && tab_rows > 0 && K > 0 && K % 2048 == 0, "ullsam_decode_qkv_rope_w8: B=%d (1..4) K=%d (%% 2048)", B, K);
    ULLSAM_CHECK(cache_pos0 >= 0 && cache_pos0 + 1 <= cap, "ullsam_decode_qkv_rope_w8: cache overflow (%d + 1 > %d)", cache_pos0, cap);
    ULLSAM_CHECK(pos && cos_tab && sin_tab && q_out && k_cache && v_cache, "ullsam_decode_qkv_rope_w8: null argument");
    RopeEpilogue r{pos, cos_tab, sin_tab, q_out, k_cache, v_cache, 1, KVH, G, cap, cache_pos0, tab_rows};
    NormPrologue n{x, ldx, norm_w, eps};
    const int N = KVH * (G + 2) * 128;
    return gemm_w8_impl("ullsam_decode_qkv_rope_w8", norm_w ? nullptr : a, norm_w ? &n : nullptr, W8, ldw, w_scale, q_out, (long)KVH * G * 128, 0, bias, nullptr, 0, 4, B, N, K,
                        stream, &r);
}

extern "C" int ullsam_gemm_qkv_rope(int dtype, const void* A, long lda, const void* W, long ldw, const float* bias, int B, int S, int K,
                                    int KVH, int G, const int* pos, const float* cos_tab, const float* sin_tab, int tab_rows, void* q_out,
                                    void* k_cache, void* v_cache, int cap, int cache_pos0, void* workspace, long ws_bytes, void* stream) {
    ULLSAM_CHECK(B > 0 && S > 0 && KVH > 0 && G > 0 && tab_rows > 0, "ullsam_gemm_qkv_rope: bad dims");
    ULLSAM_CHECK(cache_pos0 + S <= cap, "ullsam_gemm_qkv_rope: cache overflow (%d + %d > %d)", cache_pos0, S, cap);
    ULLSAM_CHECK(((uintptr_t)q_out & 15) == 0 && ((uintptr_t)k_cache & 15) == 0 && ((uintptr_t)v_cache & 15) == 0, "ullsam_gemm_qkv_rope: 16-byte aligned outputs needed");
    RopeEpilogue r{pos, cos_tab, sin_tab, q_out, k_cache, v_cache, S, KVH, G, cap, cache_pos0, tab_rows};
    const int N = KVH * (G + 2) * 128;
    return gemm_impl(dtype, A, lda, W, ldw, q_out, (long)KVH * G * 128, 0, bias, nullptr, 0, 0, 4, B * S, N, K, workspace, ws_bytes, stream, &r);
}
```

### ullsam_amd/csrc/gemm_ring8p.h

```cpp

__device__ __forceinline__ void blds16(u32x4 desc, unsigned int voff, unsigned int soff, unsigned int lds_addr) {
    unsigned int keep;
    asm volatile("s_mov_b32 %0, m0\n\ts_mov_b32 m0, %4\n\ts_nop 0\n\tbuffer_load_dwordx4 %1, %2, %3 offen lds\n\ts_mov_b32 m0, %0"
                 : "=&s"(keep) : "v"(voff), "s"(desc), "s"(soff), "s"(lds_addr) : "memory");
}
#pragma clang diagnostic push
#pragma clang diagnostic ignored "-Winline-asm"
template <int MOFF>
__device__ __forceinline__ void blds16_imm(u32x4 desc, unsigned int voff, unsigned int soff, unsigned int wave_lds_base) {
    asm volatile("s_add_i32 m0, %3, %4\n\ts_nop 0\n\tbuffer_load_dwordx4 %0, %1, %2 offen lds"
                 :: "v"(voff), "s"(desc), "s"(soff), "s"(wave_lds_base), "n"(MOFF) : "memory", "m0");
}
template <int N> __device__ __forceinline__ void wait_vmcnt() {
    static_assert(N >= 0 && N <= 6, "counted waits of the ring: one stage of a wave's pieces (at most three per operand) in flight");
    asm volatile("s_waitcnt vmcnt(%0)" :: "n"(N) : "memory");
}
#pragma clang diagnostic pop
__device__ __forceinline__ int fresh_lane() {
    int ln;
    asm volatile("v_mbcnt_lo_u32_b32 %0, -1, 0\n\tv_mbcnt_hi_u32_b32 %0, -1, %0" : "=v"(ln));
    return ln;
}
__device__ __forceinline__ u32x4 raw_desc(const void* base, unsigned int bytes) {
    const uintptr_t b = reinterpret_cast<uintptr_t>(base);
    u32x4 d;
    d[0] = __builtin_amdgcn_readfirstlane((unsigned int)b);
    d[1] = __builtin_amdgcn_readfirstlane((unsigned int)(b >> 32) & 0xffffu);
    d[2] = __builtin_amdgcn_readfirstlane(bytes);
    d[3] = 0x00020000u;
    return d;
}

template <int MI0, int MI1, int NTW, int EMODE = 0, bool STAMP = false>
__global__ __launch_bounds__(512) void gemm_ring8p_kernel(GemmArgs p) {
    extern __shared__ __attribute__((aligned(16))) char smem[];
    typedef bf16 T;
    constexpr int BM = 16 * (MI0 + MI1), BN = 64 * NTW;
    constexpr int PA = BM / 16, PB = BN / 16;
    constexpr int ASZ = BM * 64, STG = ASZ + BN * 64;
    constexpr int BIAS_LDS = 4 * STG;
    static_assert(PA >= 8 && PA <= 24 && PB >= 8 && PB <= 24, "piece assignment below: one to three pieces per wave and operand");
    static_assert(NTW == 4 || NTW == 5, "epilogue layouts below: four sub-tiles in two pairs, optionally a fifth on its own");
    constexpr int WW = 16 * NTW;

    const int nblk = p.full_tiles;
    const int q8 = nblk >> 3, r8 = nblk & 7;
    const int GMr = p.group_m;
    const int width = GMr * p.tiles_n;
    auto tile_of = [&](int v, int& tm, int& tn) __attribute__((always_inline)) {
        const int xcd = v & 7;
        const int swz = (xcd < r8 ? xcd * (q8 + 1) : r8 * (q8 + 1) + (xcd - r8) * q8) + (v >> 3);
        const int group = swz / width;
        const int first_m = group * GMr;
        const int gsize = min(p.tiles_m - first_m, GMr);
        const int rem = swz - group * width;
        tn = rem / gsize;
        tm = first_m + (rem - tn * gsize);
    };

    const int tid = threadIdx.x, lane = tid & 63;
    const int wave = __builtin_amdgcn_readfirstlane(tid >> 6);
    const int wm = wave >> 2, wn = wave & 3, grp = wave >> 2;
    const int na = (PA - wave + 7) / 8, nb = (PB - wave + 7) / 8;
    const int perm = EMODE == 1 ? 2 : p.out_f32 ? 0 : (p.act == 3 ? 2 : 1);
    auto w_row = [&](int R) {
        const int wb = R / WW, q = R - wb * WW, j = q >> 4, r = q & 15;
        if (perm == 1) return j < 4 ? WW * wb + 32 * (j >> 1) + 8 * (r >> 2) + 4 * (j & 1) + (r & 3) : WW * wb + 64 + r;
        if (perm == 2) return 128 * (wb >> 1) + 64 * (j >> 1) + 32 * (wb & 1) + 8 * (r >> 2) + 4 * (j & 1) + (r & 3);
        return R;
    };
    unsigned int a_off[3], b_off[3];
    auto set_offsets = [&](int ln) __attribute__((always_inline)) {
#pragma unroll
        for (int i = 0; i < 3; ++i) {
            const int row = (wave + 8 * i) * 16 + (ln >> 2);
            const int c = (ln & 3) ^ ((row >> 2) & 2);
            a_off[i] = (unsigned int)row * (unsigned int)(p.lda * 2) + (c << 4);
            b_off[i] = (unsigned int)w_row(row) * (unsigned int)(p.ldw * 2) + (c << 4);
        }
    };
    set_offsets(lane);
    const u32x4 a_desc = raw_desc(p.A, (unsigned int)(((size_t)(p.M - 1) * p.lda + p.K) * 2));
    const u32x4 b_desc = raw_desc(p.W, (unsigned int)(((size_t)(p.N - 1) * p.ldw + p.K) * 2));
    const unsigned int a_tile = (unsigned int)(p.lda * 2) * BM, b_tile = (unsigned int)(p.ldw * 2) * BN;
    const int st1 = p.K >> 5;
    const unsigned int wbase = __builtin_amdgcn_readfirstlane((unsigned int)(uintptr_t)LDS_PTR(smem + wave * 1024));
    const bool has_bias = p.bias && p.act != 3 && EMODE == 0;
    const int G = gridDim.x;

    auto bias_dma = [&](int n0t, int buf) __attribute__((always_inline)) {
        if (has_bias && wave < 2) {
            const int c = min(n0t + wave * 256 + fresh_lane() * 4, p.N - 4);
            glds16_sbase(reinterpret_cast<const char*>(p.bias), (unsigned int)c * 4u, (unsigned int)(uintptr_t)LDS_PTR(smem + BIAS_LDS + buf * 2048 + wave * 1024));
        }
    };
    auto request_stage = [&](unsigned int ra, unsigned int rb, int slot) __attribute__((always_inline)) {
        char* base = smem + slot * STG;
#pragma unroll
        for (int i = 0; i < 3; ++i) {
            if (i < na) blds16(a_desc, a_off[i], ra, (unsigned int)(uintptr_t)LDS_PTR(base + (wave + 8 * i) * 1024));
            if (i < nb) blds16(b_desc, b_off[i], rb, (unsigned int)(uintptr_t)LDS_PTR(base + ASZ + (wave + 8 * i) * 1024));
        }
    };
    auto stamp = [&](int tile_k, int kk) __attribute__((always_inline)) {
        if (STAMP && p.dbg && (tid & 255) == 0 && tile_k < 8) p.dbg[(((size_t)blockIdx.x * 2 + grp) * 8 + tile_k) * 4 + kk] = __builtin_amdgcn_s_memtime();
    };

    int tm0, tn0;
    tile_of(blockIdx.x, tm0, tn0);
    bias_dma(tn0 * BN, 0);
    request_stage(tm0 * a_tile, tn0 * b_tile, 0);
    request_stage(tm0 * a_tile + 64, tn0 * b_tile + 64, 1);
    asm volatile("s_waitcnt vmcnt(0)" ::: "memory");
    __builtin_amdgcn_s_barrier();
    if (grp == 1) __builtin_amdgcn_s_barrier();

    auto core = [&](auto MIW_c, auto ROWW_c) __attribute__((always_inline)) {
        constexpr int MIW = decltype(MIW_c)::value;
        constexpr int DG = 2;
        const int row_w = decltype(ROWW_c)::value >= 0 ? decltype(ROWW_c)::value : wm * (MI0 * 16);
        f32x4 acc[MIW][NTW];
#pragma unroll
        for (int i = 0; i < MIW; ++i)
#pragma unroll
            for (int j = 0; j < NTW; ++j) acc[i][j] = (f32x4){0.f, 0.f, 0.f, 0.f};
        unsigned int rd_a = 0, rd_b = 0;
        auto set_lane_state = [&]() __attribute__((always_inline)) {
            const int ln = fresh_lane();
            set_offsets(ln);
            const unsigned int lane_part = (unsigned int)((ln & 15) * 64 + (((ln >> 4) ^ (((ln & 15) >> 2) & 2)) << 4));
            rd_a = (unsigned int)(uintptr_t)LDS_PTR(smem) + (unsigned int)row_w * 64u + lane_part;
            rd_b = (unsigned int)(uintptr_t)LDS_PTR(smem) + (unsigned int)(ASZ + wn * (16 * NTW) * 64) + lane_part;
        };
        auto stage = [&](auto J_c, unsigned int so_a, unsigned int so_b, auto NA_c, auto NB_c) __attribute__((always_inline)) {
            constexpr int J = decltype(J_c)::value;
            constexpr int NA = decltype(NA_c)::value, NB = decltype(NB_c)::value;
            constexpr int RS = (J + DG) & 3, KOFF = 64 * (J + DG);
            const unsigned int rq_a = so_a + KOFF, rq_b = so_b + KOFF;
            unsigned int t_a = rd_a, t_b = rd_b;
            if constexpr (J != 0) {
                asm volatile("v_add_u32 %0, %1, %2" : "=v"(t_a) : "n"(J * STG), "v"(rd_a));
                asm volatile("v_add_u32 %0, %1, %2" : "=v"(t_b) : "n"(J * STG), "v"(rd_b));
            }
            auto frag_at = [&](unsigned int addr) -> Frag<T> {
                Frag<T> f;
                f.v = *reinterpret_cast<const __attribute__((address_space(3))) bf16x8_t*>(addr);
                return f;
            };
            Frag<T> a8[MIW], b[NTW];
            {
                auto request = [&](auto QI_c) __attribute__((always_inline)) {
                    constexpr int qi = decltype(QI_c)::value, i = qi >> 1;
                    if constexpr (!(qi & 1) && i < NA) blds16_imm<RS * STG + i * 8192>(a_desc, a_off[i], rq_a, wbase);
                    if constexpr ((qi & 1) && i < NB) blds16_imm<RS * STG + ASZ + i * 8192>(b_desc, b_off[i], rq_b, wbase);
                    __builtin_amdgcn_sched_barrier(0);
                };
                auto rd = [&](auto R_c) __attribute__((always_inline)) {
                    constexpr int r = decltype(R_c)::value;
                    if constexpr (r < NTW + MIW) {
                        if constexpr (r < NTW) b[r] = frag_at(t_b + r * 1024);
                        else a8[r - NTW] = frag_at(t_a + (r - NTW) * 1024);
                        __builtin_amdgcn_sched_barrier(0);
                    }
                };
                request(std::integral_constant<int, 0>{});
                rd(std::integral_constant<int, 0>{}); rd(std::integral_constant<int, 1>{}); rd(std::integral_constant<int, 2>{});
                request(std::integral_constant<int, 1>{});
                rd(std::integral_constant<int, 3>{}); rd(std::integral_constant<int, 4>{}); rd(std::integral_constant<int, 5>{});
                request(std::integral_constant<int, 2>{});
                rd(std::integral_constant<int, 6>{}); rd(std::integral_constant<int, 7>{}); rd(std::integral_constant<int, 8>{});
                request(std::integral_constant<int, 3>{});
                rd(std::integral_constant<int, 9>{}); rd(std::integral_constant<int, 10>{}); rd(std::integral_constant<int, 11>{});
                request(std::integral_constant<int, 4>{});
                rd(std::integral_constant<int, 12>{}); rd(std::integral_constant<int, 13>{});
                request(std::integral_constant<int, 5>{});
            }
            wait_vmcnt<NA + NB>();
            __builtin_amdgcn_sched_barrier(0);
            __builtin_amdgcn_s_barrier();
            __builtin_amdgcn_s_setprio(1);
#pragma unroll
            for (int i = 0; i < MIW; ++i)
#pragma unroll
                for (int j = 0; j < NTW; ++j) mma16(b[j], a8[i], acc[i][j]);
            __builtin_amdgcn_s_setprio(0);
            __builtin_amdgcn_sched_barrier(0);
            __builtin_amdgcn_s_barrier();
        };
        auto run_tile = [&](auto NA_c, auto NB_c, unsigned int sa, unsigned int sb, unsigned int san, unsigned int sbn) __attribute__((always_inline)) {
            using I0 = std::integral_constant<int, 0>; using I1 = std::integral_constant<int, 1>; using I2 = std::integral_constant<int, 2>; using I3 = std::integral_constant<int, 3>;
            const int ntrip = st1 >> 2;
            unsigned int ra = sa, rb = sb;
            for (int t = 0; t < ntrip; ++t) {
                const bool last = t == ntrip - 1;
                const unsigned int ha = last ? san - 256u : ra, hb = last ? sbn - 256u : rb;
                stage(I0{}, ra, rb, NA_c, NB_c);
                stage(I1{}, ra, rb, NA_c, NB_c);
                stage(I2{}, ha, hb, NA_c, NB_c);
                stage(I3{}, ha, hb, NA_c, NB_c);
                ra += 256; rb += 256;
            }
        };

        int v = blockIdx.x, tm = tm0, tn = tn0, par = 0, tile_k = 0;
        while (true) {
            stamp(tile_k, 0);
            const int vn = v + G;
            const bool has_next = vn < nblk;
            int tmn = tm, tnn = tn;
            if (has_next) tile_of(vn, tmn, tnn);
            const unsigned int sa = tm * a_tile, sb = tn * b_tile, san = tmn * a_tile, sbn = tnn * b_tile;
            {
                set_lane_state();
                constexpr int NA_LO = PA / 8, NA_HI = (PA + 7) / 8, NB_LO = PB / 8, NB_HI = (PB + 7) / 8;
                if (NA_HI != NA_LO && na == NA_HI) {
                    if (NB_HI != NB_LO && nb == NB_HI) run_tile(std::integral_constant<int, NA_HI>{}, std::integral_constant<int, NB_HI>{}, sa, sb, san, sbn);
                    else run_tile(std::integral_constant<int, NA_HI>{}, std::integral_constant<int, NB_LO>{}, sa, sb, san, sbn);
                } else {
                    if (NB_HI != NB_LO && nb == NB_HI) run_tile(std::integral_constant<int, NA_LO>{}, std::integral_constant<int, NB_HI>{}, sa, sb, san, sbn);
                    else run_tile(std::integral_constant<int, NA_LO>{}, std::integral_constant<int, NB_LO>{}, sa, sb, san, sbn);
                }
            }
            stamp(tile_k, 1);
            auto border_sync = [&](int i, int at) __attribute__((always_inline)) {
                if (i == at && grp == 0) { __builtin_amdgcn_sched_barrier(0); __builtin_amdgcn_s_barrier(); __builtin_amdgcn_sched_barrier(0); }
            };
            const int m0 = tm * BM, n0 = tn * BN;
            const int lane_e = fresh_lane();
            const int g4 = lane_e >> 4, mm = lane_e & 15;
            const char* bias_lds = smem + BIAS_LDS + par * 2048;
            float bv[4 * NTW];
#pragma unroll
            for (int e = 0; e < 4 * NTW; ++e) bv[e] = 0.f;
            if (has_bias) {
#pragma unroll
                for (int t = 0; t < NTW; ++t) {
                    const int col = wn * WW + ((p.out_f32 || t == 4) ? 16 * t + 4 * g4 : 32 * (t >> 1) + 8 * g4 + 4 * (t & 1));
                    const float4 x = *reinterpret_cast<const float4*>(bias_lds + col * 4);
                    bv[4 * t] = x.x; bv[4 * t + 1] = x.y; bv[4 * t + 2] = x.z; bv[4 * t + 3] = x.w;
                }
            }
            {
                const bool odd = mm & 1;
                const int row0 = m0 + row_w + mm;
                const int rowp = row0 & ~1;
                auto gst = [&](void* ptr, u32x4 vv) __attribute__((always_inline)) { *reinterpret_cast<u32x4*>(ptr) = vv; };
                if constexpr (EMODE == 1) {
                    const int slot = (n0 >> 7) + (wn >> 1), d = 32 * (wn & 1) + 8 * g4;
                    const int gs = p.rope_G + 2, kv = slot / gs, g = slot - kv * gs;
                    const bool live = slot < p.rope_KVH * gs;
                    const bool rotate = g != gs - 1;
                    float bl[8], bh[8];
    #pragma unroll
                    for (int e = 0; e < 8; ++e) { bl[e] = (p.bias && live) ? p.bias[slot * 128 + d + e] : 0.f; bh[e] = (p.bias && live) ? p.bias[slot * 128 + d + 64 + e] : 0.f; }
                    T* const Q = reinterpret_cast<T*>(p.rope_q);
                    T* const KVc = reinterpret_cast<T*>(g == gs - 2 ? p.rope_k : p.rope_v);
                    int ps[MIW];
    #pragma unroll
                    for (int i = 0; i < MIW; ++i) {
                        const int gm = row0 + 16 * i;
                        ps[i] = (live && rotate && gm < p.M) ? min(max(p.rope_pos[gm], 0), p.rope_rows - 1) : 0;
                    }
                    float4 cn[2], sn[2];
                    auto load_cs = [&](int i, float4 (&c)[2], float4 (&s_)[2]) __attribute__((always_inline)) {
                        const float* cp = p.rope_cos + (size_t)ps[i] * 128 + d;
                        const float* sp = p.rope_sin + (size_t)ps[i] * 128 + d;
                        c[0] = *reinterpret_cast<const float4*>(cp); c[1] = *reinterpret_cast<const float4*>(cp + 4);
                        s_[0] = *reinterpret_cast<const float4*>(sp); s_[1] = *reinterpret_cast<const float4*>(sp + 4);
                    };
                    if (rotate) load_cs(0, cn, sn);
    #pragma unroll
                    for (int i = 0; i < MIW; ++i) {
                        border_sync(i, 1);
                        const float4 c0 = cn[0], c1 = cn[1], s0 = sn[0], s1 = sn[1];
                        if (rotate && i + 1 < MIW) load_cs(i + 1, cn, sn);
                        const int gm = row0 + 16 * i;
                        if (gm >= p.M || !live) continue;
                        float x[8], y[8], lo[8], hi[8];
    #pragma unroll
                        for (int e = 0; e < 8; ++e) { x[e] = acc[i][e >> 2][e & 3] + bl[e]; y[e] = acc[i][2 + (e >> 2)][e & 3] + bh[e]; }
                        if (rotate) {
                            const float cv[8] = {c0.x, c0.y, c0.z, c0.w, c1.x, c1.y, c1.z, c1.w}, sv[8] = {s0.x, s0.y, s0.z, s0.w, s1.x, s1.y, s1.z, s1.w};
    #pragma unroll
// ... 186 lines not shown
```

### ullsam_amd/modeling/common.py

```python
from __future__ import annotations

from typing import Callable, Dict, Optional, Tuple, Type

import torch
from torch import nn

from .. import ops


class PackCache:

    def __init__(self):
        self._store: Dict[str, Tuple[tuple, torch.Tensor]] = {}

    def get(self, name: str, srcs, fn: Callable[[], torch.Tensor]) -> torch.Tensor:
        if isinstance(srcs, torch.Tensor):
            srcs = (srcs,)
        key = tuple((s.data_ptr(), s._version, s.dtype, str(s.device)) for s in srcs)
        hit = self._store.get(name)
        if hit is not None and hit[0] == key:
            return hit[1]
        with torch.no_grad():
            val = fn()
        self._store[name] = (key, val)
        return val


class Packed(nn.Module):

    def __init__(self):
        super().__init__()
        object.__setattr__(self, "_packs", PackCache())

    def pk(self, name, srcs, fn):
        return self._packs.get(name, srcs, fn)

    def f32(self, name: str, p: torch.Tensor) -> torch.Tensor:
        return self.pk(name + ":f32", p, lambda: p.detach().float().contiguous())

    def cdt(self, name: str, p: torch.Tensor, dtype: torch.dtype) -> torch.Tensor:
        return self.pk(name + ":cdt", p, lambda: p.detach().to(dtype).contiguous())


class Linear(Packed):

    def __init__(self, in_features: int, out_features: int, bias: bool = True):
        super().__init__()
        self.in_features, self.out_features = in_features, out_features
        self.weight = nn.Parameter(torch.empty(out_features, in_features))
        self.bias = nn.Parameter(torch.empty(out_features)) if bias else None
        nn.init.normal_(self.weight, std=in_features ** -0.5)
        if bias:
            nn.init.zeros_(self.bias)

    def w(self, dtype):
        return self.cdt("w", self.weight, dtype)

    def b(self):
        return None if self.bias is None else self.f32("b", self.bias)

    def w8(self):
        pair = self.pk("w8", self.weight, lambda: ops.rows_fp8(self.weight.detach().contiguous()))
        return pair

    def w8d(self):
        return self.pk("w8d", self.weight, lambda: ops.rows_fp8_pow2(self.weight.detach().contiguous()))

    def tok(self, x: torch.Tensor, act: int = ops.ACT_NONE, res: Optional[torch.Tensor] = None) -> torch.Tensor:
        M = x.numel() // self.in_features
        if M >= 64 and self.in_features % 128 == 0:
            wt = self.pk("w32t", self.weight, lambda: self.weight.detach().float().t().contiguous())
            return ops.skinny_linear(x, wt, self.b(), act, res)
        return ops.small_linear(x, self.f32("w32", self.weight), self.b(), act, res)

    def forward(self, x: torch.Tensor) -> torch.Tensor:
        dt = self.weight.dtype
        y = ops.gemm(ops.cast(x.reshape(-1, self.in_features).contiguous(), dt), self.w(dt), self.b())
        return y.reshape(*x.shape[:-1], self.out_features)


class LayerNorm(Packed):
    def __init__(self, dim: int, eps: float = 1e-5):
        super().__init__()
        self.eps = eps
        self.normalized_shape = (dim,)
        self.weight = nn.Parameter(torch.ones(dim))
        self.bias = nn.Parameter(torch.zeros(dim))

    def wb(self):
        return self.f32("w", self.weight), self.f32("b", self.bias)

    def forward(self, x: torch.Tensor) -> torch.Tensor:
        w, b = self.wb()
        return ops.norm(x.contiguous(), w, b, self.eps, x.dtype)


class LayerNorm2d(Packed):

    def __init__(self, num_channels: int, eps: float = 1e-6):
        super().__init__()
        self.weight = nn.Parameter(torch.ones(num_channels))
        self.bias = nn.Parameter(torch.zeros(num_channels))
        self.eps = eps

    def wb(self):
        return self.f32("w", self.weight), self.f32("b", self.bias)

    def forward(self, x: torch.Tensor) -> torch.Tensor:
        B, C, H, W = x.shape
        w, b = self.wb()
        nhwc = ops.transpose(x.float().contiguous().reshape(B, C, H * W), B, C, H * W)
        y = ops.norm(nhwc, w, b, self.eps, torch.float32)
        return ops.transpose(y, B, H * W, C).reshape(B, C, H, W).to(x.dtype)


class MLPBlock(Packed):

    def __init__(self, embedding_dim: int, mlp_dim: int, act: Type[nn.Module] = nn.GELU):
        super().__init__()
        self.lin1 = Linear(embedding_dim, mlp_dim)
        self.lin2 = Linear(mlp_dim, embedding_dim)
        self.act = act()
        self.act_code = ops.ACT_GELU if isinstance(self.act, nn.GELU) else ops.ACT_RELU

    def forward(self, x: torch.Tensor) -> torch.Tensor:
        dt = self.lin1.weight.dtype
        h = ops.gemm(ops.cast(x.reshape(-1, x.shape[-1]).contiguous(), dt), self.lin1.w(dt), self.lin1.b(), act=self.act_code)
        y = ops.gemm(h, self.lin2.w(dt), self.lin2.b())
        return y.reshape(x.shape)
```

### ullsam_amd/modeling/image_encoder.py

```python
from __future__ import annotations

from typing import Optional, Tuple, Type

import torch
from torch import nn

from .. import ops
from ..packing import pack_conv3x3
from .common import LayerNorm, LayerNorm2d, Linear, MLPBlock, Packed


class _Conv2dParams(Packed):

    def __init__(self, cin, cout, k, bias=True):
        super().__init__()
        self.weight = nn.Parameter(torch.empty(cout, cin, k, k))
        self.bias = nn.Parameter(torch.zeros(cout)) if bias else None
        nn.init.normal_(self.weight, std=(cin * k * k) ** -0.5)


class PatchEmbed(Packed):

    def __init__(self, kernel_size=(16, 16), stride=(16, 16), padding=(0, 0), in_chans=3, embed_dim=768):
        super().__init__()
# ... 21 lines not shown
        n = 2 * size - 1
        if p.shape[0] == n:
            return self.cdt(name, p, dtype)

        def make():
            t = p.detach().float().t().contiguous().reshape(p.shape[1], 1, p.shape[0])
            out, _ = ops.resize_bilinear(t, (1, n))
            return out.reshape(p.shape[1], n).t().contiguous().to(dtype)
        return self.pk(f"{name}:interp{n}", p, make)


class Block(Packed):

    def __init__(self, dim, num_heads, mlp_ratio=4.0, qkv_bias=True, norm_layer=LayerNorm, act_layer=nn.GELU,
                 use_rel_pos=False, rel_pos_zero_init=True, window_size=0, input_size=None):
        super().__init__()
        self.norm1 = _make_norm(norm_layer, dim)
        self.attn = Attention(dim, num_heads, qkv_bias, use_rel_pos, rel_pos_zero_init,
                              input_size if window_size == 0 else (window_size, window_size))
        self.norm2 = _make_norm(norm_layer, dim)
        self.mlp = MLPBlock(embedding_dim=dim, mlp_dim=int(dim * mlp_ratio), act=act_layer)
        self.window_size = window_size


def _make_norm(norm_layer, dim) -> LayerNorm:
    probe = norm_layer(dim)
    eps = getattr(probe, "eps", 1e-5)
    return LayerNorm(dim, eps=eps)


class ImageEncoderViT(Packed):
    def __init__(self, img_size: int = 1024, patch_size: int = 16, in_chans: int = 3, embed_dim: int = 768, depth: int = 12,
                 num_heads: int = 12, mlp_ratio: float = 4.0, out_chans: int = 256, qkv_bias: bool = True,
                 norm_layer: Type[nn.Module] = nn.LayerNorm, act_layer: Type[nn.Module] = nn.GELU, use_abs_pos: bool = True,
                 use_rel_pos: bool = False, rel_pos_zero_init: bool = True, window_size: int = 0,
                 global_attn_indexes: Tuple[int, ...] = ()) -> None:
        super().__init__()
        self.img_size = img_size
        self.patch_size = patch_size
        self.embed_dim, self.num_heads, self.out_chans = embed_dim, num_heads, out_chans
        self.patch_embed = PatchEmbed((patch_size, patch_size), (patch_size, patch_size), in_chans=in_chans, embed_dim=embed_dim)
        self.pos_embed: Optional[nn.Parameter] = None
        g = img_size // patch_size
        if use_abs_pos:
            self.pos_embed = nn.Parameter(torch.zeros(1, g, g, embed_dim))
        self.blocks = nn.ModuleList()
        for i in range(depth):
            self.blocks.append(Block(dim=embed_dim, num_heads=num_heads, mlp_ratio=mlp_ratio, qkv_bias=qkv_bias,
                                     norm_layer=norm_layer, act_layer=act_layer, use_rel_pos=use_rel_pos,
                                     rel_pos_zero_init=rel_pos_zero_init,
                                     window_size=window_size if i not in global_attn_indexes else 0, input_size=(g, g)))
        self.neck = nn.Sequential(_Conv2dParams(embed_dim, out_chans, 1, bias=False), LayerNorm2d(out_chans),
                                  _Conv2dParams(out_chans, out_chans, 3, bias=False), LayerNorm2d(out_chans))
        if not use_rel_pos:
            raise NotImplementedError("the HIP attention kernel implements SAM's use_rel_pos=True configuration")
        self.fp8_linears = False
        self.stage_probe = None

    @property
    def compute_dtype(self) -> torch.dtype:
        return self.patch_embed.proj.weight.dtype

    def forward_tokens(self, x: torch.Tensor, pixel_mean: Optional[torch.Tensor] = None,
                       pixel_std: Optional[torch.Tensor] = None) -> torch.Tensor:
        dt = self.compute_dtype
        S, p = self.img_size, self.patch_size
        g = S // p
        N = g * g
        B = x.shape[0]
        D = self.embed_dim
        cols = ops.patch_im2col(x.float().contiguous(), S, p, dt, pixel_mean, pixel_std)
        pe = self.patch_embed.proj
        wp = self.pk("patch_w", pe.weight, lambda: pe.weight.detach().reshape(D, -1).to(dt).contiguous())
        pos = None if self.pos_embed is None else self.f32("pos", self.pos_embed).reshape(N, D)
        xres = ops.gemm(cols, wp, None if pe.bias is None else self.f32("patch_b", pe.bias), residual=pos, res_row_mod=N, out_f32=True)
        fp8 = bool(self.fp8_linears) and dt == torch.bfloat16 and D % 128 == 0
        for bi, blk in enumerate(self.blocks):
            at = blk.attn
            if fp8:
                q8, sa = ops.rows_fp8(xres, *blk.norm1.wb(), blk.norm1.eps)
                qkv = ops.gemm_fp8(q8, sa, *at.qkv.w8(), at.qkv.b())
            else:
                xn = ops.norm(xres, *blk.norm1.wb(), blk.norm1.eps, dt)
                qkv = ops.gemm(xn, at.qkv.w(dt), at.qkv.b())
            qb = at.qkv.bias if at.qkv.bias is not None else torch.zeros(3 * D, device=x.device)
            n_rel = blk.window_size if blk.window_size > 0 else g
            att = ops.vit_attention(qkv, at.rel_table("rh", at.rel_pos_h, n_rel, dt), at.rel_table("rw", at.rel_pos_w, n_rel, dt), at.cdt("qb", qb, dt),
                                    B, self.num_heads, at.head_dim, g, g, blk.window_size)
            ops.gemm(att, at.proj.w(dt), at.proj.b(), residual=xres, out_f32=True, out=xres)
            if fp8:
                q8, sa = ops.rows_fp8(xres, *blk.norm2.wb(), blk.norm2.eps)
                h = ops.gemm_fp8(q8, sa, *blk.mlp.lin1.w8(), blk.mlp.lin1.b(), act=blk.mlp.act_code)
            else:
                xn = ops.norm(xres, *blk.norm2.wb(), blk.norm2.eps, dt)
                h = ops.gemm(xn, blk.mlp.lin1.w(dt), blk.mlp.lin1.b(), act=blk.mlp.act_code)
            ops.gemm(h, blk.mlp.lin2.w(dt), blk.mlp.lin2.b(), residual=xres, out_f32=True, out=xres)
            if self.stage_probe is not None:
                self.stage_probe(bi, xres)
        n0, n1, n2, n3 = self.neck[0], self.neck[1], self.neck[2], self.neck[3]
        C = self.out_chans
        w0 = self.pk("neck0", n0.weight, lambda: n0.weight.detach().reshape(C, D).to(dt).contiguous())
        y = ops.gemm(ops.cast(xres, dt), w0, out_f32=True)
        yn = ops.norm(y, *n1.wb(), n1.eps, dt)
        w2 = self.pk("neck2", n2.weight, lambda: pack_conv3x3(n2.weight.detach()).to(dt).contiguous())
        z = ops.gemm(ops.im2col3x3(yn, B, g, g, C), w2, out_f32=True)
        out = ops.norm(z, *n3.wb(), n3.eps, torch.float32)
        return out.reshape(B, N, C)

    def forward(self, x: torch.Tensor) -> torch.Tensor:
        from .. import training
        if training.wants_autograd(self, x):
            return training.vision_forward(self, x)
        with torch.no_grad():
            B = x.shape[0]
            g = self.img_size // self.patch_size
            tok = self.forward_tokens(x)
            return ops.transpose(tok, B, g * g, self.out_chans).reshape(B, self.out_chans, g, g).to(self.compute_dtype)
```

### ullsam_amd/modeling/modeling_internlm2.py

```python
from __future__ import annotations

from typing import List, Optional, Tuple

import torch
from torch import nn

from .. import ops
from ..packing import pack_w13
from ..sampling import row_seeds
from .common import Linear, Packed
from .configuration_internlm2 import InternLM2Config
from .outputs import BaseModelOutputWithPast, CausalLMOutputWithPast


class InternLM2RMSNorm(Packed):

    def __init__(self, hidden_size, eps=1e-6):
        super().__init__()
        self.weight = nn.Parameter(torch.ones(hidden_size))
        self.variance_epsilon = eps

    def w(self):
        return self.f32("w", self.weight)

    def forward(self, hidden_states: torch.Tensor) -> torch.Tensor:
        return ops.norm(hidden_states.contiguous(), self.w(), None, self.variance_epsilon, hidden_states.dtype, rms=True)


class InternLM2MLP(Packed):
    def __init__(self, config):
        super().__init__()
        self.w1 = Linear(config.hidden_size, config.intermediate_size, bias=False)
        self.w3 = Linear(config.hidden_size, config.intermediate_size, bias=False)
        self.w2 = Linear(config.intermediate_size, config.hidden_size, bias=False)
        if config.hidden_act != "silu":
            raise NotImplementedError("the fused SwiGLU epilogue implements hidden_act='silu'")

    def w13(self, dt):
        return self.pk("w13", (self.w1.weight, self.w3.weight), lambda: pack_w13(self.w1.weight.detach().to(dt), self.w3.weight.detach().to(dt)))

    def w13_w8d(self, dt):
        return self.pk("w13:w8d", (self.w1.weight, self.w3.weight), lambda: ops.rows_fp8_pow2(self.w13(dt)))


class InternLM2Attention(Packed):
    def __init__(self, config: InternLM2Config):
        super().__init__()
        self.hidden_size = config.hidden_size
        self.num_heads = config.num_attention_heads
        self.head_dim = self.hidden_size // self.num_heads
        self.num_key_value_heads = config.num_key_value_heads
        self.num_key_value_groups = self.num_heads // self.num_key_value_heads
        if self.head_dim * self.num_heads != self.hidden_size:
            raise ValueError(f"hidden_size must be divisible by num_heads (got `hidden_size`: {self.hidden_size}"
                             f" and `num_heads`: {self.num_heads}).")
        self.wqkv = Linear(self.hidden_size, (self.num_heads + 2 * self.num_key_value_heads) * self.head_dim, bias=config.bias)
        self.wo = Linear(self.num_heads * self.head_dim, self.hidden_size, bias=config.bias)


class InternLM2DecoderLayer(Packed):
    def __init__(self, config: InternLM2Config):
        super().__init__()
        self.attention = InternLM2Attention(config)
        self.feed_forward = InternLM2MLP(config)
        self.attention_norm = InternLM2RMSNorm(config.hidden_size, eps=config.rms_norm_eps)
        self.ffn_norm = InternLM2RMSNorm(config.hidden_size, eps=config.rms_norm_eps)


class _Embedding(Packed):
    def __init__(self, n, d, padding_idx=None):
        super().__init__()
        self.padding_idx = padding_idx
        self.weight = nn.Parameter(torch.empty(n, d))

    def forward(self, ids: torch.Tensor) -> torch.Tensor:
        shp = ids.shape
        out = ops.embed_tokens(self.weight.detach(), ids.reshape(1, -1).contiguous(), None, None)
        return out.reshape(*shp, self.weight.shape[1])


class KVCache:

    def __init__(self, layers, B, kvh, cap, hd, dtype, device):
        self.k = [torch.empty((B, kvh, cap, hd), dtype=dtype, device=device) for _ in range(layers)]
        self.v = [torch.empty((B, kvh, cap, hd), dtype=dtype, device=device) for _ in range(layers)]
        self.len, self.cap = 0, cap

    def to_tuple(self):
        return tuple((k[:, :, :self.len], v[:, :, :self.len]) for k, v in zip(self.k, self.v))

    def grow(self, cap: int):
        if cap <= self.cap:
            return
        for buf in (self.k, self.v):
            for i, old in enumerate(buf):
                new = torch.empty((old.shape[0], old.shape[1], cap, old.shape[3]), dtype=old.dtype, device=old.device)
                new[:, :, :self.len].copy_(old[:, :, :self.len])
                buf[i] = new
        self.cap = cap


class InternLM2Model(Packed):
    def __init__(self, config: InternLM2Config):
        super().__init__()
        self.config = config
        self.padding_idx = config.pad_token_id
        self.vocab_size = config.vocab_size
        self.tok_embeddings = _Embedding(config.vocab_size, config.hidden_size, self.padding_idx)
        self.layers = nn.ModuleList([InternLM2DecoderLayer(config) for _ in range(config.num_hidden_layers)])
        self.norm = InternLM2RMSNorm(config.hidden_size, eps=config.rms_norm_eps)
        self._rope = None
        self.collect_all_hidden_states = False
        self.fuse_decode = True
        self.fp8_decode = False
        self.stage_probe = None

    def get_input_embeddings(self):
        return self.tok_embeddings

    @property
    def compute_dtype(self):
        return self.layers[0].attention.wqkv.weight.dtype

    def rope_tables(self, seq_len: int, device):
        cfg = self.config
        hd = cfg.hidden_size // cfg.num_attention_heads
        rs = cfg.rope_scaling
        dynamic = rs is not None and rs["type"] == "dynamic"
        if self._rope is not None and self._rope[0][0] >= seq_len and self._rope[0][1] == str(device):
            return self._rope[1], self._rope[2]
        base = float(cfg.rope_theta)
        scale_t = 1.0
        rows = max(seq_len, 2048)
        if rs is not None and rs["type"] == "linear":
            scale_t = float(rs["factor"])
        elif dynamic and seq_len > cfg.max_position_embeddings:
            f = float(rs["factor"])
            base = base * ((f * seq_len / cfg.max_position_embeddings) - (f - 1)) ** (hd / (hd - 2))
            rows = seq_len
        elif dynamic:
            rows = min(rows, cfg.max_position_embeddings)
        inv_freq = 1.0 / (base ** (torch.arange(0, hd, 2).float() / hd))
        t = torch.arange(rows, dtype=inv_freq.dtype) / scale_t
        freqs = torch.einsum("i,j->ij", t, inv_freq)
        emb = torch.cat((freqs, freqs), dim=-1)
        cos, sin = emb.cos().to(device).contiguous(), emb.sin().to(device).contiguous()
        self._rope = ((rows, str(device)), cos, sin)
        return cos, sin

    def new_cache(self, B: int, cap: int, device) -> KVCache:
        c = self.config
        return KVCache(c.num_hidden_layers, B, c.num_key_value_heads, cap, c.hidden_size // c.num_attention_heads, self.compute_dtype, device)

    def run_layers(self, x: torch.Tensor, B: int, S: int, pos: torch.Tensor, key_mask: Optional[torch.Tensor],
                   cache: Optional[KVCache], collect: Optional[list] = None) -> torch.Tensor:
        cfg = self.config
        dt = self.compute_dtype
        H, KVH = cfg.num_attention_heads, cfg.num_key_value_heads
        hd, G = cfg.hidden_size // H, H // KVH
        past = cache.len if cache is not None else 0
        Sk = past + S
        cos, sin = self.rope_tables(Sk, x.device)
        tmp_k = tmp_v = None
        if cache is None:
            tmp_k = torch.empty((B, KVH, S, hd), dtype=dt, device=x.device)
            tmp_v = torch.empty_like(tmp_k)
        fused = S == 1 and cache is not None and hd == 128 and ops.decode_fusable(B, cfg.hidden_size, dt) and self.fuse_decode
        w8 = bool(getattr(self, "fp8_decode", False)) and fused and x.is_cuda
        w8_wo, w8_w2 = w8 and ops.decode_w8_ok(B, H * hd), w8 and ops.decode_w8_ok(B, cfg.intermediate_size)
        for li, layer in enumerate(self.layers):
            if collect is not None:
                collect.append(x.reshape(B, S, -1).to(dt))
            at, ff = layer.attention, layer.feed_forward
            kc, vc = (cache.k[li], cache.v[li]) if cache is not None else (tmp_k, tmp_v)
            if w8:
                q = ops.decode_qkv_rope_w8(x, layer.attention_norm.w(), layer.attention_norm.variance_epsilon, *at.wqkv.w8d(), at.wqkv.b(), kc, vc,
                                           pos, cos, sin, B, KVH, G, past)
            elif fused:
                q = ops.decode_qkv_rope(x, layer.attention_norm.w(), layer.attention_norm.variance_epsilon, at.wqkv.w(dt), at.wqkv.b(), kc, vc,
                                        pos, cos, sin, B, KVH, G, past)
            else:
                xn = ops.norm(x, layer.attention_norm.w(), None, layer.attention_norm.variance_epsilon, dt, rms=True)
                if hd == 128 and S > 8:
                    q = ops.gemm_qkv_rope(xn, at.wqkv.w(dt), at.wqkv.b(), kc, vc, pos, cos, sin, B, S, KVH, G, past)
                else:
                    qkv = ops.gemm(xn, at.wqkv.w(dt), at.wqkv.b())
                    q = ops.rope_split(qkv, kc, vc, pos, cos, sin, B, S, KVH, G, hd, past)
            if S > 1:
                a = ops.causal_attention(q, kc, vc, key_mask, B, H, KVH, hd, S, Sk, past)
            elif dt == torch.bfloat16 and hd == 128 and G <= 8:
                a = ops.decode_attention(q, kc, vc, key_mask, B, H, KVH, hd, Sk)
            else:
                cap = kc.shape[2]
                a = ops.naive_attention(q, kc, vc, B, H, KVH, hd, 1, Sk, (H * hd, H * hd, hd), (KVH * cap * hd, hd, cap * hd),
                                        (KVH * cap * hd, hd, cap * hd), (H * hd, H * hd, hd), hd ** -0.5, key_mask=key_mask)
            if w8_wo:
                ops.gemm_w8(a, *at.wo.w8d(), at.wo.b(), residual=x, out_f32=True, out=x)
            else:
                ops.gemm(a, at.wo.w(dt), at.wo.b(), residual=x, out_f32=True, out=x)
            if w8:
                hmid = ops.gemm_w8(x, *ff.w13_w8d(dt), act=ops.ACT_SWIGLU, norm_w=layer.ffn_norm.w(), eps=layer.ffn_norm.variance_epsilon)
            elif fused:
                hmid = ops.gemm_rmsnorm(x, layer.ffn_norm.w(), layer.ffn_norm.variance_epsilon, ff.w13(dt), act=ops.ACT_SWIGLU)
            else:
                xn = ops.norm(x, layer.ffn_norm.w(), None, layer.ffn_norm.variance_epsilon, dt, rms=True)
                hmid = ops.gemm(xn, ff.w13(dt), act=ops.ACT_SWIGLU)
            if w8_w2:
                ops.gemm_w8(hmid, *ff.w2.w8d(), None, residual=x, out_f32=True, out=x)
            else:
                ops.gemm(hmid, ff.w2.w(dt), None, residual=x, out_f32=True, out=x)
            if self.stage_probe is not None:
                self.stage_probe(li, x)
        if cache is not None:
            cache.len = Sk
        return ops.norm(x, self.norm.w(), None, self.norm.variance_epsilon, dt, rms=True)

    @torch.no_grad()
    def forward(self, input_ids=None, attention_mask=None, position_ids=None, past_key_values=None, inputs_embeds=None,
                use_cache=None, output_attentions=None, output_hidden_states=None, return_dict=None):
        cfg = self.config
        if output_attentions:
            raise NotImplementedError("attention probabilities are never materialised by the fused attention kernels")
        use_cache = use_cache if use_cache is not None else cfg.use_cache
        if input_ids is not None and inputs_embeds is not None:
            raise ValueError("You cannot specify both input_ids and inputs_embeds at the same time")
        if input_ids is None and inputs_embeds is None:
            raise ValueError("You have to specify either input_ids or inputs_embeds")
        if inputs_embeds is None:
            B, S = input_ids.shape[:2]
            x = ops.embed_tokens(self.tok_embeddings.weight.detach(), input_ids.contiguous(), None, None)
            dev = input_ids.device
        else:
            B, S = inputs_embeds.shape[:2]
            dev = inputs_embeds.device
            x = inputs_embeds.reshape(B * S, -1).float().contiguous().clone()
        cache = past_key_values if isinstance(past_key_values, KVCache) else None
        if past_key_values is not None and cache is None:
            raise TypeError("past_key_values must be the KVCache returned by a previous call (use_cache=True)")
        past = cache.len if cache is not None else 0
        if cache is None and use_cache:
            cache = self.new_cache(B, max(2 * S, S + 256), dev)
        if cache is not None and past + S > cache.cap:
            cache.grow(max(2 * cache.cap, past + S))
        if position_ids is None:
            position_ids = torch.arange(past, past + S, dtype=torch.long, device=dev).unsqueeze(0).expand(B, S)
        pos = position_ids.to(torch.int32).expand(B, S).contiguous()
        key_mask = None
        if attention_mask is not None:
            key_mask = attention_mask.to(torch.int32).contiguous()
            if key_mask.shape != (B, past + S):
                raise ValueError(f"Attention mask should be of size {(B, past + S)}, but is {tuple(key_mask.shape)}")
        collect = [] if (output_hidden_states and self.collect_all_hidden_states) else None
        h = self.run_layers(x, B, S, pos, key_mask, cache, collect).reshape(B, S, -1)
        all_h = None
        if output_hidden_states:
            all_h = tuple(collect) + (h,) if collect is not None else (None,) * len(self.layers) + (h,)
        return BaseModelOutputWithPast(last_hidden_state=h, past_key_values=cache if use_cache else None, hidden_states=all_h)


class InternLM2ForCausalLM(Packed):
    def __init__(self, config):
        super().__init__()
        self.config = config
        self.model = InternLM2Model(config)
        self.vocab_size = config.vocab_size
        self.output = Linear(config.hidden_size, config.vocab_size, bias=False)
        self.fp8_decode = False

    @property
    def fp8_decode(self) -> bool:
        return bool(getattr(self.model, "fp8_decode", False))

    @fp8_decode.setter
    def fp8_decode(self, on: bool):
        self.model.fp8_decode = bool(on)

    @fp8_decode.deleter
    def fp8_decode(self):
        if "fp8_decode" in self.model.__dict__:
            del self.model.fp8_decode

    def get_input_embeddings(self):
        return self.model.tok_embeddings

    def get_output_embeddings(self):
        return self.output

    def lm_head(self, hidden: torch.Tensor, prefill: bool = False) -> torch.Tensor:
        dt = self.model.compute_dtype
        h2 = hidden.reshape(-1, hidden.shape[-1]).contiguous()
        if not prefill and self.fp8_decode and self.model.fuse_decode and h2.is_cuda and ops.decode_fusable(h2.shape[0], h2.shape[1], dt):
            return ops.gemm_w8(ops.cast(h2, dt), *self.output.w8d(), None, out_f32=True).reshape(*hidden.shape[:-1], self.vocab_size)
        return ops.gemm(ops.cast(h2, dt), self.output.w(dt), None, out_f32=True).reshape(*hidden.shape[:-1], self.vocab_size)
# ... 122 lines not shown
```

### ullsam_amd/modeling/modeling_internvl_sam.py

```python
from __future__ import annotations

import math
import warnings
from typing import List, Optional

import torch
from torch import nn

from .. import ops
from .common import LayerNorm, Linear, Packed
from .configuration_internvl_chat import InternVLChatConfig
from .modeling_internlm2 import InternLM2ForCausalLM
from .outputs import CausalLMOutputWithPast

INTERNLM2_CHAT_SYSTEM = ("You are an AI assistant whose name is InternLM (书生·浦语).")


class InternVLSAMModel(Packed):
    config_class = InternVLChatConfig
    main_input_name = "pixel_values"
    base_model_prefix = "language_model"

    def __init__(self, config: InternVLChatConfig, vision_model=None, prompt_encoder=None, mask_decoder=None, language_model=None,
                 use_flash_attn=True):
        super().__init__()
        self.config = config
        self.patch_size = 16
        self.select_layer = config.select_layer
        self.template = config.template
        self.num_image_token = 64 * 64 * (config.downsample_ratio ** 2)
        self.downsample_ratio = config.downsample_ratio
        self.ps_version = config.ps_version
        if config.downsample_ratio != 0.5 or config.ps_version == "v1":
            raise NotImplementedError("the HIP shuffle kernels implement downsample_ratio=0.5, ps_version='v2' "
                                      "(what uLLSAM constructs, train_joint_v2.py:1424-1431)")
        if vision_model is not None:
            self.vision_model = vision_model
        if prompt_encoder is not None:
            self.prompt_encoder = prompt_encoder
        if mask_decoder is not None:
            self.mask_decoder = mask_decoder
        if language_model is not None:
            self.language_model = language_model
        elif config.llm_config.architectures[0] == "InternLM2ForCausalLM":
            self.language_model = InternLM2ForCausalLM(config.llm_config)
        else:
            raise NotImplementedError(f"{config.llm_config.architectures[0]} is not implemented.")
        sam_hidden_size = 256
        llm_hidden_size = config.llm_config.hidden_size
        c4 = sam_hidden_size * int(1 / self.downsample_ratio) ** 2
        self.mlp1 = nn.Sequential(LayerNorm(c4), Linear(c4, llm_hidden_size), nn.GELU(), Linear(llm_hidden_size, llm_hidden_size))
        self.mlp2 = nn.Sequential(LayerNorm(llm_hidden_size), Linear(llm_hidden_size, c4), nn.GELU(), Linear(c4, c4))
        self.img_context_token_id = 92546
        self.system_message = INTERNLM2_CHAT_SYSTEM

    @property
    def device(self):
        return self.mlp1[1].weight.device

    @property
    def dtype(self):
        return self.mlp1[1].weight.dtype

    def _mlp1_tokens(self, img_tok: torch.Tensor, B: int) -> torch.Tensor:
        dt = self.dtype
        ln, l1, l3 = self.mlp1[0], self.mlp1[1], self.mlp1[3]
        f = ops.pixel_shuffle_ln(img_tok, *ln.wb(), B, 64, 64, 256, ln.eps, dt)
        h = ops.gemm(f, l1.w(dt), l1.b(), act=ops.ACT_GELU)
        return ops.gemm(h, l3.w(dt), l3.b(), out_f32=True)

    def _mlp2_tokens(self, rows: torch.Tensor, B: int) -> torch.Tensor:
        dt = self.dtype
        ln, l1, l3 = self.mlp2[0], self.mlp2[1], self.mlp2[3]
        f = ops.norm(rows, *ln.wb(), ln.eps, dt)
        f = ops.gemm(f, l1.w(dt), l1.b(), act=ops.ACT_GELU)
        f = ops.gemm(f, l3.w(dt), l3.b(), out_f32=True)
        return ops.pixel_unshuffle(f, B, 64, 64, 256)

    @torch.no_grad()
    def extract_feature(self, pixel_values):
        B = pixel_values.shape[0]
        img_tok = self.vision_model.forward_tokens(pixel_values)
        vit = self._mlp1_tokens(img_tok, B).reshape(B, 1024, -1)
        feats = ops.transpose(img_tok, B, 4096, 256).reshape(B, 256, 64, 64).to(self.dtype)
        return vit.to(self.dtype), feats

    @torch.no_grad()
    def text_aware_dense_feature(self, features):
        B = features.shape[0]
        tok = self._mlp2_tokens(ops.cast(features.reshape(B * features.shape[1], -1).contiguous(), self.dtype), B)
        return ops.transpose(tok, B, 4096, 256).reshape(B, 256, 64, 64)

    def pixel_shuffle(self, x, scale_factor=0.5):
        n, h, w, c = x.size()
        x = x.reshape(n, h, int(w * scale_factor), int(c / scale_factor)).permute(0, 2, 1, 3).contiguous()
        x = x.reshape(n, int(w * scale_factor), int(h * scale_factor), int(c / (scale_factor * scale_factor)))
        return x.permute(0, 2, 1, 3).contiguous()

    def forward(self, pixel_values, input_ids=None, attention_mask=None, position_ids=None, image_flags=None, past_key_values=None,
                labels=None, use_cache=None, output_attentions=None, output_hidden_states=None, return_dict=None,
                img_context_token_id=None):
        if return_dict is False:
            raise NotImplementedError("tuple outputs are not provided; use return_dict=True (what app.py / train_joint_v2.py pass)")
        from .. import training
        if training.wants_autograd(self) and past_key_values is None and position_ids is None:
            return training.composite_forward(self, pixel_values, input_ids, attention_mask, labels, output_hidden_states)
        with torch.no_grad():
            return self._forward_inference(pixel_values, input_ids, attention_mask, position_ids, image_flags, past_key_values, labels, use_cache,
                                           output_attentions, output_hidden_states, return_dict, img_context_token_id)

    def _forward_inference(self, pixel_values, input_ids=None, attention_mask=None, position_ids=None, image_flags=None, past_key_values=None,
                           labels=None, use_cache=None, output_attentions=None, output_hidden_states=None, return_dict=None,
                           img_context_token_id=None):
        B, S = input_ids.shape
        dev = input_ids.device
        lm = self.language_model
        ids = input_ids.contiguous()
        rank, rng = ops.scan_image_tokens(ids, self.img_context_token_id)
        capturing = torch.cuda.is_current_stream_capturing()
        if not capturing:
            rng_host = torch.empty((B, 2), dtype=torch.int32, pin_memory=True)
            rng_host.copy_(rng, non_blocking=True)
            ev = torch.cuda.Event()
            ev.record()
        img_tok = self.vision_model.forward_tokens(pixel_values)
        vit_embeds = self._mlp1_tokens(img_tok, B)
        x = ops.embed_tokens(lm.model.tok_embeddings.weight.detach(), ids, rank, vit_embeds)
        out = lm(inputs_embeds=x.reshape(B, S, -1), attention_mask=attention_mask, position_ids=position_ids,
                 past_key_values=past_key_values, use_cache=use_cache, output_attentions=output_attentions,
                 output_hidden_states=output_hidden_states, labels=labels, lazy_logits=True)
        g = 64
        image_embeddings = ops.transpose(img_tok, B, g * g, 256).reshape(B, 256, g, g).to(self.dtype)
        hidden_states = out.hidden_states
        dense_tok = None
        if out.hidden_states is not None:
            n_img = int(self.num_image_token)
            rows = ops.gather_rows(out.hidden_states[-1].reshape(B * S, -1), rng, B, S, n_img)
            dense_tok = self._mlp2_tokens(rows, B)
            hidden_states = ops.transpose(dense_tok, B, g * g, 256).reshape(B, 256, g, g)
            if not capturing:
                ev.synchronize()
                r = rng_host.numpy()
                if (r[:, 1] <= r[:, 0]).any():
                    raise ValueError("Can not find vision token!")
                if ((r[:, 1] - r[:, 0]) != n_img).any():
                    raise RuntimeError(f"image-token span {(r[:, 1] - r[:, 0]).tolist()} != {n_img}: text_aware_dense_feature needs a "
                                       "32x32 token grid (the reference's reshape fails the same way)")
        ret = CausalLMOutputWithPast(loss=out.loss, logits=out._logits, logits_fn=out._logits_fn, past_key_values=out.past_key_values,
                                     hidden_states=hidden_states, attentions=None)
        ret.image_embeddings = image_embeddings
        ret.image_tokens = img_tok
        ret.dense_feature_tokens = dense_tok
        return ret

    @torch.no_grad()
    def generate(self, pixel_values=None, input_ids=None, attention_mask=None, visual_features=None, generation_config=None,
                 output_hidden_states=None, **generate_kwargs) -> torch.LongTensor:
        assert self.img_context_token_id is not None
        lm = self.language_model
# ... 43 lines not shown
```

### ullsam_amd/ops.py

```python
from __future__ import annotations

from typing import Optional

import numpy as np
import torch

from . import _lib

ACT_NONE, ACT_GELU, ACT_RELU, ACT_SWIGLU = 0, 1, 2, 3
ACT_SPLITK_OK = 256
_DT = {torch.float32: 0, torch.bfloat16: 1}


def dt_code(dtype: torch.dtype) -> int:
    try:
        return _DT[dtype]
    except KeyError:
        raise TypeError(f"ullsam_amd supports float32 and bfloat16 compute, got {dtype}") from None


def _stream() -> int:
    return torch.cuda.current_stream().cuda_stream


def _p(t: Optional[torch.Tensor]):
    return None if t is None else t.data_ptr()


def _chk(t: torch.Tensor, name: str, dtype=None):
    if not t.is_cuda:
        raise _lib.UllsamError(f"{name} must live on the GPU (ullsam_amd has no CPU path)")
    if t.device.index != torch.cuda.current_device():
        raise _lib.UllsamError(f"{name} lives on {t.device} but the current device is cuda:{torch.cuda.current_device()}; "
                               f"run the call under `with torch.cuda.device({t.device.index}):`")
    if not t.is_contiguous():
        raise ValueError(f"{name} must be contiguous")
    if dtype is not None and t.dtype != dtype:
        raise TypeError(f"{name} must be {dtype}, got {t.dtype}")
    return t


_WS = {}


def _gemm_workspace(device) -> torch.Tensor:
    key = (str(device), torch.cuda.current_stream().cuda_stream)
    ws = _WS.get(key)
    if ws is None:
        ws = _WS[key] = torch.empty(128 << 20, dtype=torch.uint8, device=device)
    return ws


def gemm(a: torch.Tensor, w: torch.Tensor, bias: Optional[torch.Tensor] = None, residual: Optional[torch.Tensor] = None,
         act: int = ACT_NONE, out_f32: bool = False, out: Optional[torch.Tensor] = None, res_row_mod: int = 0, splitk_ok: bool = False) -> torch.Tensor:
    _chk(a, "a"); _chk(w, "w", a.dtype)
    M, K = a.shape
    N = w.shape[0]
    assert w.shape[1] == K, (a.shape, w.shape)
    n_out = N // 2 if act == ACT_SWIGLU else N
    odt = torch.float32 if out_f32 else a.dtype
    if out is None:
        out = torch.empty((M, n_out), dtype=odt, device=a.device)
    else:
        _chk(out, "out", odt)
        assert out.shape == (M, n_out)
    if bias is not None:
        _chk(bias, "bias", torch.float32)
    ldr = 0
    if residual is not None:
        _chk(residual, "residual", torch.float32)
        ldr = residual.shape[-1]
    ws = _gemm_workspace(a.device)
    _lib.call("ullsam_gemm", dt_code(a.dtype), a.data_ptr(), K, w.data_ptr(), K, out.data_ptr(), n_out, int(out_f32),
              _p(bias), _p(residual), ldr, res_row_mod, act | (ACT_SPLITK_OK if splitk_ok else 0), M, N, K, ws.data_ptr(), ws.numel(), _stream())
    return out


def rows_fp8(x: torch.Tensor, ln_w: Optional[torch.Tensor] = None, ln_b: Optional[torch.Tensor] = None, eps: float = 0.0):
    _chk(x, "x")
    D = x.shape[-1]
    rows = x.numel() // D
    q = torch.empty((rows, D), dtype=torch.uint8, device=x.device)
    sc = torch.empty((rows,), dtype=torch.float32, device=x.device)
    if ln_w is not None:
        _chk(ln_w, "ln_w", torch.float32); _chk(ln_b, "ln_b", torch.float32)
    _lib.call("ullsam_rows_fp8", x.data_ptr(), dt_code(x.dtype), D, q.data_ptr(), D, sc.data_ptr(), _p(ln_w), _p(ln_b), rows, D, float(eps), _stream())
    return q, sc


def gemm_fp8(a8: torch.Tensor, a_scale: torch.Tensor, w8: torch.Tensor, w_scale: torch.Tensor, bias: Optional[torch.Tensor] = None,
             act: int = ACT_NONE, out_dtype: torch.dtype = torch.bfloat16, residual: Optional[torch.Tensor] = None) -> torch.Tensor:
    _chk(a8, "a8", torch.uint8); _chk(w8, "w8", torch.uint8); _chk(a_scale, "a_scale", torch.float32); _chk(w_scale, "w_scale", torch.float32)
    M, K = a8.shape
    N = w8.shape[0]
    assert w8.shape[1] == K and a_scale.numel() == M and w_scale.numel() == N
    out_f32 = out_dtype == torch.float32
    out = torch.empty((M, N), dtype=out_dtype, device=a8.device)
    if bias is not None:
        _chk(bias, "bias", torch.float32)
    ldr = 0
    if residual is not None:
        _chk(residual, "residual", torch.float32)
        ldr = residual.shape[-1]
    _lib.call("ullsam_gemm_fp8", a8.data_ptr(), K, a_scale.data_ptr(), w8.data_ptr(), K, w_scale.data_ptr(), out.data_ptr(), N, int(out_f32),
              _p(bias), _p(residual), ldr, act, M, N, K, _stream())
    return out


def norm(x: torch.Tensor, w: Optional[torch.Tensor], b: Optional[torch.Tensor], eps: float, out_dtype: torch.dtype,
         rms: bool = False, act: int = ACT_NONE, post_scale: Optional[torch.Tensor] = None,
         post_shift: Optional[torch.Tensor] = None, out: Optional[torch.Tensor] = None) -> torch.Tensor:
    _chk(x, "x")
    D = x.shape[-1]
    rows = x.numel() // D
    if out is None:
        out = torch.empty(x.shape, dtype=out_dtype, device=x.device)
    for t in (w, b, post_scale, post_shift):
        if t is not None:
            _chk(t, "norm param", torch.float32)
    _lib.call("ullsam_norm", x.data_ptr(), dt_code(x.dtype), D, out.data_ptr(), dt_code(out.dtype), D, _p(w), _p(b), rows, D,
              float(eps), int(rms), act, _p(post_scale), _p(post_shift), _stream())
    return out


def norm_fanout(x: torch.Tensor, w, b, eps: float, cdt: torch.dtype, pe: Optional[torch.Tensor], want_f32: bool = True,
                want_c: bool = True):
    _chk(x, "x", torch.float32)
    D = x.shape[-1]
    rows = x.numel() // D
    f32c = cdt == torch.float32
    out_f = torch.empty((rows, D), dtype=torch.float32, device=x.device) if (want_f32 or (f32c and want_c)) else None
    out_c = torch.empty((rows, D), dtype=cdt, device=x.device) if (want_c and not f32c) else None
    out_pe = torch.empty((rows, D), dtype=cdt, device=x.device) if pe is not None else None
    if pe is not None:
        _chk(pe, "pe", torch.float32)
    _lib.call("ullsam_norm_fanout", x.data_ptr(), rows, D, _p(w), _p(b), float(eps), _p(out_f), _p(out_c), _p(out_pe), dt_code(cdt),
              _p(pe), pe.numel() // D if pe is not None else 0, _stream())
    return out_f, (out_f if f32c else out_c), out_pe


def i2t_block(xin: torch.Tensor, res: torch.Tensor, wq: torch.Tensor, bq, ktok: torch.Tensor, vtok: torch.Tensor, wo: torch.Tensor, bo,
              lnw, lnb, eps: float, key_pe: Optional[torch.Tensor], P: int, T: int, N: int, scale: float, shared: bool, want_f32: bool = True,
              want_c: bool = True):
    _chk(xin, "xin", torch.bfloat16); _chk(res, "res", torch.float32); _chk(wq, "wq", torch.bfloat16); _chk(wo, "wo", torch.bfloat16)
    _chk(ktok, "ktok", torch.float32); _chk(vtok, "vtok", torch.float32)
    assert wq.shape == (128, 256) and wo.shape == (256, 128) and ktok.numel() == P * T * 128 and vtok.numel() == P * T * 128
    assert xin.numel() == (N if shared else P * N) * 256 and res.numel() == xin.numel()
    rows = P * N
    out_f = torch.empty((rows, 256), dtype=torch.float32, device=xin.device) if want_f32 else None
    out_c = torch.empty((rows, 256), dtype=torch.bfloat16, device=xin.device) if want_c else None
    out_pe = torch.empty((rows, 256), dtype=torch.bfloat16, device=xin.device) if key_pe is not None else None
    if key_pe is not None:
        _chk(key_pe, "key_pe", torch.float32)
    _lib.call("ullsam_i2t_block", xin.data_ptr(), N if shared else 0, res.data_ptr(), N if shared else 0, wq.data_ptr(), _p(bq), ktok.data_ptr(), vtok.data_ptr(),
              wo.data_ptr(), _p(bo), _p(lnw), _p(lnb), float(eps), _p(key_pe), key_pe.numel() // 256 if key_pe is not None else 0, _p(out_f), _p(out_c), _p(out_pe),
# ... 194 lines not shown
    _lib.call("ullsam_transpose_f32", x.data_ptr(), out.data_ptr(), B, R, C, _stream())
    return out


def transpose_to_bf16(x: torch.Tensor, pad_to: int = 1) -> torch.Tensor:
    _chk(x, "x")
    R, Cn = x.shape
    Rp = -(-R // pad_to) * pad_to
    out = torch.empty((Cn, Rp), dtype=torch.bfloat16, device=x.device)
    _lib.call("ullsam_transpose_to_bf16", dt_code(x.dtype), x.data_ptr(), out.data_ptr(), R, Cn, Rp, _stream())
    return out


def cast_transpose_bf16(x: torch.Tensor, pad_to: int = 64, row_major: bool = True, colsum: bool = False):
    _chk(x, "x", torch.float32)
    R, Cn = x.shape
    assert Cn % 4 == 0 and pad_to % 4 == 0
    Rp = -(-R // pad_to) * pad_to
    rm = torch.empty((R, Cn), dtype=torch.bfloat16, device=x.device) if row_major else None
    xt = torch.empty((Cn, Rp), dtype=torch.bfloat16, device=x.device)
    cs = ws = None
    if colsum:
        cs = torch.empty((Cn,), dtype=torch.float32, device=x.device)
        ws = torch.empty((-(-Rp // 64) * Cn,), dtype=torch.float32, device=x.device)
    _lib.call("ullsam_cast_transpose_bf16", x.data_ptr(), _p(rm), xt.data_ptr(), _p(cs), _p(ws), R, Cn, Rp, _stream())
    return rm, xt, cs


def pixel_shuffle_ln(x_nhwc: torch.Tensor, w, b, B, H, W, C, eps, dtype) -> torch.Tensor:
    _chk(x_nhwc, "x", torch.float32)
    out = torch.empty((B * (H // 2) * (W // 2), 4 * C), dtype=dtype, device=x_nhwc.device)
    _lib.call("ullsam_pixel_shuffle_ln", dt_code(dtype), x_nhwc.data_ptr(), out.data_ptr(), w.data_ptr(), b.data_ptr(), B, H, W, C,
              float(eps), _stream())
    return out


def pixel_unshuffle(x: torch.Tensor, B, H, W, C) -> torch.Tensor:
    _chk(x, "x", torch.float32)
    out = torch.empty((B, H * W, C), dtype=torch.float32, device=x.device)
    _lib.call("ullsam_pixel_unshuffle", x.data_ptr(), out.data_ptr(), B, H, W, C, _stream())
    return out


def scan_image_tokens(ids: torch.Tensor, img_id: int):
    _chk(ids, "input_ids", torch.int64)
    B, S = ids.shape
    rank = torch.empty((B, S), dtype=torch.int32, device=ids.device)
    rng = torch.empty((B, 2), dtype=torch.int32, device=ids.device)
    _lib.call("ullsam_scan_image_tokens", ids.data_ptr(), rank.data_ptr(), rng.data_ptr(), B, S, int(img_id), _stream())
    return rank, rng


def embed_tokens(table: torch.Tensor, ids: torch.Tensor, rank: Optional[torch.Tensor], vit: Optional[torch.Tensor]) -> torch.Tensor:
    _chk(table, "tok_embeddings"); _chk(ids, "ids", torch.int64)
    B, S = ids.shape
    V, D = table.shape
    n_img = 0
    if vit is not None:
        _chk(vit, "vit_embeds", torch.float32)
        n_img = vit.numel() // (B * D)
    out = torch.empty((B * S, D), dtype=torch.float32, device=ids.device)
    _lib.call("ullsam_embed_tokens", dt_code(table.dtype), table.data_ptr(), ids.data_ptr(), _p(rank), _p(vit), out.data_ptr(), B, S, D,
              max(n_img, 1), V, _stream())
    return out


def gather_rows(x: torch.Tensor, rng: torch.Tensor, B: int, S: int, n: int) -> torch.Tensor:
    _chk(x, "x"); _chk(rng, "range", torch.int32)
    D = x.shape[-1]
    out = torch.empty((B * n, D), dtype=x.dtype, device=x.device)
    _lib.call("ullsam_gather_rows", x.data_ptr(), out.data_ptr(), rng.data_ptr(), B, S, n, D * x.element_size(), _stream())
    return out


def rope_split(qkv, k_cache, v_cache, pos, cos_tab, sin_tab, B, S, KVH, G, hd, cache_pos0) -> torch.Tensor:
    _chk(qkv, "qkv"); _chk(pos, "position_ids", torch.int32); _chk(cos_tab, "cos", torch.float32); _chk(sin_tab, "sin", torch.float32)
    q = torch.empty((B * S, KVH * G * hd), dtype=qkv.dtype, device=qkv.device)
    _lib.call("ullsam_rope_split", dt_code(qkv.dtype), qkv.data_ptr(), q.data_ptr(), k_cache.data_ptr(), v_cache.data_ptr(),
              pos.data_ptr(), cos_tab.data_ptr(), sin_tab.data_ptr(), B, S, KVH, G, hd, k_cache.shape[2], cache_pos0, cos_tab.shape[0], _stream())
    return q


def gemm_qkv_rope(x: torch.Tensor, wqkv: torch.Tensor, bias: Optional[torch.Tensor], k_cache, v_cache, pos, cos_tab, sin_tab, B, S, KVH, G,
                  cache_pos0) -> torch.Tensor:
    _chk(x, "x"); _chk(wqkv, "wqkv", x.dtype); _chk(pos, "position_ids", torch.int32); _chk(cos_tab, "cos", torch.float32); _chk(sin_tab, "sin", torch.float32)
    _chk(k_cache, "k_cache", x.dtype); _chk(v_cache, "v_cache", x.dtype)
    K = x.shape[1]
    assert wqkv.shape == (KVH * (G + 2) * 128, K) and x.shape[0] == B * S and cos_tab.shape[1] == 128
    if bias is not None:
        _chk(bias, "bias", torch.float32)
    q = torch.empty((B * S, KVH * G * 128), dtype=x.dtype, device=x.device)
    ws = _gemm_workspace(x.device)
    _lib.call("ullsam_gemm_qkv_rope", dt_code(x.dtype), x.data_ptr(), K, wqkv.data_ptr(), K, _p(bias), B, S, K, KVH, G, pos.data_ptr(),
              cos_tab.data_ptr(), sin_tab.data_ptr(), cos_tab.shape[0], q.data_ptr(), k_cache.data_ptr(), v_cache.data_ptr(), k_cache.shape[2],
              cache_pos0, ws.data_ptr(), ws.numel(), _stream())
    return q


def decode_fusable(M: int, K: int, dtype: torch.dtype) -> bool:
    return dtype == torch.bfloat16 and 1 <= M <= 4 and K <= 4096 and K % 2048 == 0


def decode_w8_ok(M: int, K: int) -> bool:
    return 1 <= M <= 8 and K % 512 == 0 and (4 if M <= 4 else 8) * K * 2 <= 144 * 1024


def gemm_rmsnorm(x: torch.Tensor, norm_w: torch.Tensor, eps: float, w: torch.Tensor, act: int = ACT_NONE) -> torch.Tensor:
    _chk(x, "x", torch.float32); _chk(norm_w, "norm_w", torch.float32); _chk(w, "w", torch.bfloat16)
    M, K = x.shape
    N = w.shape[0]
    assert w.shape[1] == K and decode_fusable(M, K, w.dtype), (x.shape, w.shape)
    n_out = N // 2 if act == ACT_SWIGLU else N
    out = torch.empty((M, n_out), dtype=torch.bfloat16, device=x.device)
    _lib.call("ullsam_gemm_rmsnorm", x.data_ptr(), K, norm_w.data_ptr(), float(eps), w.data_ptr(), K, out.data_ptr(), n_out, 0, None, None, 0,
              act, M, N, K, _stream())
    return out


def decode_qkv_rope(x: torch.Tensor, norm_w: Optional[torch.Tensor], eps: float, wqkv: torch.Tensor, bias: Optional[torch.Tensor], k_cache, v_cache,
                    pos, cos_tab, sin_tab, B, KVH, G, cache_pos0) -> torch.Tensor:
    _chk(wqkv, "wqkv", torch.bfloat16); _chk(pos, "position_ids", torch.int32); _chk(cos_tab, "cos", torch.float32); _chk(sin_tab, "sin", torch.float32)
    _chk(k_cache, "k_cache", torch.bfloat16); _chk(v_cache, "v_cache", torch.bfloat16)
    _chk(x, "x", torch.float32 if norm_w is not None else torch.bfloat16)
    K = x.shape[1]
    assert wqkv.shape == (KVH * (G + 2) * 128, K) and x.shape[0] == B and cos_tab.shape[1] == 128 and decode_fusable(B, K, wqkv.dtype)
    if bias is not None:
        _chk(bias, "bias", torch.float32)
    if norm_w is not None:
        _chk(norm_w, "norm_w", torch.float32)
    q = torch.empty((B, KVH * G * 128), dtype=torch.bfloat16, device=x.device)
    _lib.call("ullsam_decode_qkv_rope", None if norm_w is not None else x.data_ptr(), x.data_ptr() if norm_w is not None else None, K, _p(norm_w),
              float(eps), wqkv.data_ptr(), K, _p(bias), B, K, KVH, G, pos.data_ptr(), cos_tab.data_ptr(), sin_tab.data_ptr(), cos_tab.shape[0],
              q.data_ptr(), k_cache.data_ptr(), v_cache.data_ptr(), k_cache.shape[2], cache_pos0, _stream())
    return q


def rows_fp8_pow2(w: torch.Tensor):
    _chk(w, "w")
    assert w.dim() == 2 and w.shape[1] % 4 == 0, w.shape
    N, K = w.shape
    q = torch.empty((N, K), dtype=torch.uint8, device=w.device)
    sc = torch.empty((N,), dtype=torch.float32, device=w.device)
    _lib.call("ullsam_rows_fp8_pow2", w.data_ptr(), dt_code(w.dtype), K, q.data_ptr(), K, sc.data_ptr(), N, K, _stream())
    return q, sc


def gemm_w8(a: torch.Tensor, w8: torch.Tensor, w_scale: torch.Tensor, bias: Optional[torch.Tensor] = None, residual: Optional[torch.Tensor] = None,
            act: int = ACT_NONE, out_f32: bool = False, out: Optional[torch.Tensor] = None, norm_w: Optional[torch.Tensor] = None, eps: float = 0.0) -> torch.Tensor:
    _chk(a, "a", torch.float32 if norm_w is not None else torch.bfloat16); _chk(w8, "w8", torch.uint8); _chk(w_scale, "w_scale", torch.float32)
    M, K = a.shape
    N = w8.shape[0]
    assert w8.shape[1] == K and w_scale.numel() == N, (a.shape, w8.shape, w_scale.shape)
    n_out = N // 2 if act == ACT_SWIGLU else N
    odt = torch.float32 if out_f32 else torch.bfloat16
    if out is None:
        out = torch.empty((M, n_out), dtype=odt, device=a.device)
    else:
        _chk(out, "out", odt)
        assert out.shape == (M, n_out)
    if bias is not None:
        _chk(bias, "bias", torch.float32)
        assert bias.numel() == N
    ldr = 0
    if residual is not None:
        _chk(residual, "residual", torch.float32)
        assert residual.shape == (M, n_out)
        ldr = residual.shape[-1]
    if norm_w is not None:
        _chk(norm_w, "norm_w", torch.float32)
        assert norm_w.numel() == K
    _lib.call("ullsam_gemm_w8", None if norm_w is not None else a.data_ptr(), a.data_ptr() if norm_w is not None else None, K, _p(norm_w), float(eps),
              w8.data_ptr(), K, w_scale.data_ptr(), out.data_ptr(), n_out, int(out_f32), _p(bias), _p(residual), ldr, act, M, N, K, _stream())
    return out


# ... 1374 lines not shown
```

### ullsam_amd/packing.py

```python
from __future__ import annotations

import torch


def pack_w13(w1: torch.Tensor, w3: torch.Tensor) -> torch.Tensor:
    I, K = w1.shape
    assert w3.shape == (I, K) and I % 64 == 0
    return torch.stack([w1.reshape(I // 64, 64, K), w3.reshape(I // 64, 64, K)], dim=1).reshape(2 * I, K).contiguous()


def pack_conv3x3(w: torch.Tensor) -> torch.Tensor:
    return w.permute(0, 2, 3, 1).reshape(w.shape[0], -1).contiguous()


def pack_convT_k2s2(w: torch.Tensor, b: torch.Tensor):
    cin, cout = w.shape[0], w.shape[1]
    return w.permute(2, 3, 1, 0).reshape(4 * cout, cin).contiguous(), b.repeat(4).contiguous()
```

Measured before the change: 52.53 images/s.

## Add K-panel packed weight layout for ring GEMM kernels

New measurement: 55.69 images/s, median of 6. +6.0%, better.

```diff
diff --git a/include/ullsam_hip.h b/include/ullsam_hip.h
--- a/include/ullsam_hip.h
+++ b/include/ullsam_hip.h
@@ -29,6 +29,13 @@
 int ullsam_gemm_qkv_rope(int dtype, const void* A, long lda, const void* W, long ldw, const float* bias, int B, int S, int K, int KVH,
                          int G, const int* pos, const float* cos_tab, const float* sin_tab, int tab_rows, void* q_out, void* k_cache,
                          void* v_cache, int cap, int cache_pos0, void* workspace, long ws_bytes, void* stream);
+
+int ullsam_gemm_panels(int dtype, const void* A, long lda, const void* W, long ldw, const void* w_panels, void* C, long ldc, int out_f32,
+                       const float* bias, const float* residual, long ldr, int res_row_mod, int act, int M, int N, int K,
+                       void* workspace, long ws_bytes, void* stream);
+int ullsam_gemm_qkv_rope_panels(int dtype, const void* A, long lda, const void* W, long ldw, const void* w_panels, const float* bias, int B, int S,
+                                int K, int KVH, int G, const int* pos, const float* cos_tab, const float* sin_tab, int tab_rows, void* q_out,
+                                void* k_cache, void* v_cache, int cap, int cache_pos0, void* workspace, long ws_bytes, void* stream);
 
 int ullsam_gemm_rmsnorm(const float* x, long ldx, const float* norm_w, float eps, const void* W, long ldw, void* C, long ldc, int out_f32,
                         const float* bias, const float* residual, long ldr, int act, int M, int N, int K, void* stream);
diff --git a/ullsam_amd/_lib.py b/ullsam_amd/_lib.py
--- a/ullsam_amd/_lib.py
+++ b/ullsam_amd/_lib.py
@@ -15,6 +15,8 @@
 SIGNATURES = {
     "ullsam_gemm": [i32, vp, i64, vp, i64, vp, i64, i32, vp, vp, i64, i32, i32, i32, i32, i32, vp, i64, vp],
     "ullsam_gemm_qkv_rope": [i32, vp, i64, vp, i64, vp, i32, i32, i32, i32, i32, vp, vp, vp, i32, vp, vp, vp, i32, i32, vp, i64, vp],
+    "ullsam_gemm_panels": [i32, vp, i64, vp, i64, vp, vp, i64, i32, vp, vp, i64, i32, i32, i32, i32, i32, vp, i64, vp],
+    "ullsam_gemm_qkv_rope_panels": [i32, vp, i64, vp, i64, vp, vp, i32, i32, i32, i32, i32, vp, vp, vp, i32, vp, vp, vp, i32, i32, vp, i64, vp],
     "ullsam_gemm_rmsnorm": [vp, i64, vp, f32, vp, i64, vp, i64, i32, vp, vp, i64, i32, i32, i32, i32, vp],
     "ullsam_decode_qkv_rope": [vp, vp, i64, vp, f32, vp, i64, vp, i32, i32, i32, i32, vp, vp, vp, i32, vp, vp, vp, i32, i32, vp],
     "ullsam_train_matmul": [vp, vp, vp, i32, i32, i32, i32] + [i64] * 9 + [i32, vp],
diff --git a/ullsam_amd/csrc/gemm.hip b/ullsam_amd/csrc/gemm.hip
--- a/ullsam_amd/csrc/gemm.hip
+++ b/ullsam_amd/csrc/gemm.hip
@@ -23,6 +23,7 @@
     const float* col_scale;
     unsigned long long* dbg;
     const float* norm_x; const float* norm_w; float norm_eps; long ldx;
+    const void* w_panels;
     int group_m;
 };
 
@@ -680,7 +681,9 @@
     const int g4 = lane >> 4, mm = lane & 15;
 
     const char* a_base = reinterpret_cast<const char*>(p.A) + (size_t)m0 * p.lda * 2;
-    const char* b_base = reinterpret_cast<const char*>(p.W) + (size_t)n0 * p.ldw * 2;
+    const bool panels = EMODE != 2 && p.w_panels != nullptr;
+    const unsigned int kst = __builtin_amdgcn_readfirstlane(panels ? 1024u : 64u);
+    const char* b_base = reinterpret_cast<const char*>(panels ? p.w_panels : p.W) + (size_t)n0 * p.ldw * 2;
     const int na = (PA - wave + 7) / 8, nb = (PB - wave + 7) / 8;
     static_assert(NTW == 4 || NTW == 5, "epilogue layouts below: four sub-tiles in two pairs, optionally a fifth on its own");
     constexpr int WW = 16 * NTW;
@@ -697,7 +700,9 @@
         const int row = (wave + 8 * i) * 16 + (lane >> 2);
         const int c = (lane & 3) ^ ((row >> 2) & 2);
         a_off[i] = (unsigned int)((size_t)(min(m0 + row, p.M - 1) - m0) * p.lda * 2) + (c << 4);
-        b_off[i] = (unsigned int)((size_t)(min(n0 + w_row(row), p.N - 1) - n0) * p.ldw * 2) + (c << 4);
+        const int wr = w_row(row);
+        b_off[i] = panels ? (unsigned int)(wr >> 4) * ((unsigned int)p.K * 32u) + (unsigned int)(wr & 15) * 64u + (c << 4)
+                          : (unsigned int)((size_t)(min(n0 + wr, p.N - 1) - n0) * p.ldw * 2) + (c << 4);
     }
     const int st1 = p.K >> 5;
 
@@ -712,7 +717,7 @@
     auto stage = [&](int s) {
         char* base = smem + (s & 3) * STG;
         const char* ak = a_base + (size_t)s * 64;
-        const char* bk = b_base + (size_t)s * 64;
+        const char* bk = b_base + (size_t)s * kst;
 #pragma unroll
         for (int i = 0; i < 3; ++i) {
             if (i < na) __builtin_amdgcn_global_load_lds(GLB_PTR(ak + a_off[i]), LDS_PTR(base + (wave + 8 * i) * 1024), 16, 0, 0);
@@ -761,7 +766,7 @@
             {
                 char* base = smem + ((s + 2) & 3) * STG;
                 const char* ak = a_base + (size_t)(s + 2) * 64;
-                const char* bk = b_base + (size_t)(s + 2) * 64;
+                const char* bk = b_base + (size_t)(s + 2) * kst;
                 auto request = [&](int qi) __attribute__((always_inline)) {
                     const int i = qi >> 1;
                     if (g_asm_dma) {
@@ -1100,7 +1105,7 @@
     static PerDeviceOnce attr_set;
     if (attr_set.first()) (void)hipFuncSetAttribute(reinterpret_cast<const void*>(gemm_ring8_kernel<MI0, MI1, NTW, false, 2>), hipFuncAttributeMaxDynamicSharedMemorySize, LDS);
     GemmArgs b = a;
-    b.C = a.ws; b.ldc = a.N; b.out_f32 = 1; b.bias = nullptr; b.residual = nullptr; b.act = 0; b.vec_ok = 1; b.dbg = nullptr;
+    b.C = a.ws; b.ldc = a.N; b.out_f32 = 1; b.bias = nullptr; b.residual = nullptr; b.act = 0; b.vec_ok = 1; b.dbg = nullptr; b.w_panels = nullptr;
     b.tiles_m = (a.M + BM - 1) / BM;
     b.tiles_n = (a.N + BN - 1) / BN;
     b.full_tiles = b.tiles_m * b.tiles_n;
@@ -1127,6 +1132,7 @@
 }
 #include "gemm_ring8p.h"
 static int g_persist = 2;
+static int g_ring_panels = 1;
 static int cu_count() {
     static int n[32] = {};
     int d = 0;
@@ -1147,7 +1153,9 @@
     return a.act == 0;
 }
 template <int MI0, int MI1, int NTW, int EMODE = 0>
-static int launch_ring(const GemmArgs& a, hipStream_t stream) {
+static int launch_ring(const GemmArgs& a0, hipStream_t stream) {
+    GemmArgs a = a0;
+    if (!(g_ring_panels && a.N % (64 * NTW) == 0 && a.K % 32 == 0 && a.ldw == a.K)) a.w_panels = nullptr;
     return ring_persist_ok<16 * (MI0 + MI1), 64 * NTW, NTW, EMODE>(a) ? launch_gemm_ring8p<MI0, MI1, NTW, EMODE>(a, stream, cu_count())
                                                                       : launch_gemm_ring8<MI0, MI1, NTW, EMODE>(a, stream);
 }
@@ -1293,7 +1301,7 @@
     a.group_m = 4;
     a.vec_ok = vec ? 1 : 0;
     a.ws = nullptr; a.ws_bytes = 0; a.ksplit = 1;
-    a.row_scale = a_scale; a.col_scale = w_scale; a.dbg = nullptr;
+    a.row_scale = a_scale; a.col_scale = w_scale; a.dbg = nullptr; a.w_panels = nullptr;
     a.tiles_m = (M + 255) / 256; a.tiles_n = (N + 255) / 256; a.full_tiles = a.tiles_m * a.tiles_n;
     static PerDeviceOnce attr_set;
     if (attr_set.first()) (void)hipFuncSetAttribute(reinterpret_cast<const void*>(gemm256f8_kernel), hipFuncAttributeMaxDynamicSharedMemorySize, 131072);
@@ -1307,6 +1315,7 @@
     if (key == 1 && value >= 0 && value <= 7) { g_auto_mask = value; return 0; }
     if (key == 2 && (value == 0 || value == 2)) { g_persist = value; return 0; }
     if (key == 3 && value >= 0 && value <= 2) { g_ring_splitk = value; return 0; }
+    if (key == 4 && (value == 0 || value == 1)) { g_ring_panels = value; return 0; }
     ullsam_set_error("ullsam_set_gemm_tuning: unknown key %d / bad value %d", key, value);
     return -1;
 }
@@ -1859,7 +1868,7 @@
 
 static int gemm_impl(int dtype, const void* A, long lda, const void* W, long ldw, void* C, long ldc, int out_f32,
                      const float* bias, const float* residual, long ldr, int res_row_mod, int act, int M, int N,
-                     int K, void* workspace, long ws_bytes, void* stream, const RopeEpilogue* rope, const NormPrologue* norm = nullptr) {
+                     int K, void* workspace, long ws_bytes, void* stream, const RopeEpilogue* rope, const NormPrologue* norm = nullptr, const void* w_panels = nullptr) {
     ULLSAM_CHECK(dtype == ULLSAM_DT_F32 || dtype == ULLSAM_DT_BF16, "ullsam_gemm: bad dtype %d", dtype);
     ULLSAM_CHECK(M > 0 && N > 0 && K > 0, "ullsam_gemm: empty problem M=%d N=%d K=%d", M, N, K);
     const int esz = dtype == ULLSAM_DT_F32 ? 4 : 2;
@@ -1884,7 +1893,9 @@
                      "ullsam_gemm: the RMSNorm prologue needs 16-byte aligned fp32 rows and weight");
         a.norm_x = norm->x; a.norm_w = norm->w; a.norm_eps = norm->eps; a.ldx = norm->ldx;
     }
-    a.A = A; a.W = W; a.C = C; a.bias = bias; a.residual = residual;
+    ULLSAM_CHECK(!w_panels || (dtype == ULLSAM_DT_BF16 && ((uintptr_t)w_panels & 1023) == 0 && N % 16 == 0 && K % 32 == 0),
+                 "ullsam_gemm: K-panels are bf16 [N / 16][K / 32][16][32], 1 KiB aligned (N=%d K=%d)", N, K);
+    a.A = A; a.W = W; a.C = C; a.bias = bias; a.residual = residual; a.w_panels = w_panels;
     a.M = M; a.N = N; a.K = K;
     a.lda = lda; a.ldw = ldw; a.ldc = ldc; a.ldr = ldr;
     a.res_row_mod = res_row_mod; a.act = act; a.out_f32 = out_f32;
@@ -1956,6 +1967,13 @@
     return gemm_impl(dtype, A, lda, W, ldw, C, ldc, out_f32, bias, residual, ldr, res_row_mod, act, M, N, K, workspace, ws_bytes, stream, nullptr);
 }
 
+extern "C" int ullsam_gemm_panels(int dtype, const void* A, long lda, const void* W, long ldw, const void* w_panels, void* C, long ldc, int out_f32,
+                                  const float* bias, const float* residual, long ldr, int res_row_mod, int act, int M, int N,
+                                  int K, void* workspace, long ws_bytes, void* stream) {
+    ULLSAM_CHECK(act != 4, "ullsam_gemm_panels: act 4 is ullsam_gemm_qkv_rope_panels");
+    return gemm_impl(dtype, A, lda, W, ldw, C, ldc, out_f32, bias, residual, ldr, res_row_mod, act, M, N, K, workspace, ws_bytes, stream, nullptr, nullptr, w_panels);
+}
+
 extern "C" int ullsam_gemm_rmsnorm(const float* x, long ldx, const float* norm_w, float eps, const void* W, long ldw, void* C, long ldc,
                                    int out_f32, const float* bias, const float* residual, long ldr, int act, int M, int N, int K, void* stream) {
     ULLSAM_CHECK(act != 4, "ullsam_gemm_rmsnorm: act 4 is ullsam_decode_qkv_rope");
@@ -2036,3 +2054,13 @@
     const int N = KVH * (G + 2) * 128;
     return gemm_impl(dtype, A, lda, W, ldw, q_out, (long)KVH * G * 128, 0, bias, nullptr, 0, 0, 4, B * S, N, K, workspace, ws_bytes, stream, &r);
 }
+extern "C" int ullsam_gemm_qkv_rope_panels(int dtype, const void* A, long lda, const void* W, long ldw, const void* w_panels, const float* bias, int B, int S,
+                                           int K, int KVH, int G, const int* pos, const float* cos_tab, const float* sin_tab, int tab_rows, void* q_out,
+                                           void* k_cache, void* v_cache, int cap, int cache_pos0, void* workspace, long ws_bytes, void* stream) {
+    ULLSAM_CHECK(B > 0 && S > 0 && KVH > 0 && G > 0 && tab_rows > 0, "ullsam_gemm_qkv_rope_panels: bad dims");
+    ULLSAM_CHECK(cache_pos0 + S <= cap, "ullsam_gemm_qkv_rope_panels: cache overflow (%d + %d > %d)", cache_pos0, S, cap);
+    ULLSAM_CHECK(((uintptr_t)q_out & 15) == 0 && ((uintptr_t)k_cache & 15) == 0 && ((uintptr_t)v_cache & 15) == 0, "ullsam_gemm_qkv_rope_panels: 16-byte aligned outputs needed");
+    RopeEpilogue r{pos, cos_tab, sin_tab, q_out, k_cache, v_cache, S, KVH, G, cap, cache_pos0, tab_rows};
+    const int N = KVH * (G + 2) * 128;
+    return gemm_impl(dtype, A, lda, W, ldw, q_out, (long)KVH * G * 128, 0, bias, nullptr, 0, 0, 4, B * S, N, K, workspace, ws_bytes, stream, &r, nullptr, w_panels);
+}
diff --git a/ullsam_amd/csrc/gemm_ring8p.h b/ullsam_amd/csrc/gemm_ring8p.h
--- a/ullsam_amd/csrc/gemm_ring8p.h
+++ b/ullsam_amd/csrc/gemm_ring8p.h
@@ -69,6 +69,10 @@
         if (perm == 2) return 128 * (wb >> 1) + 64 * (j >> 1) + 32 * (wb & 1) + 8 * (r >> 2) + 4 * (j & 1) + (r & 3);
         return R;
     };
+    const bool panels = p.w_panels != nullptr;
+    const int wp_shift = panels ? 4 : 0;
+    const unsigned int wp_mask = panels ? 15u : 0u, wp_block = panels ? (unsigned int)p.K * 32u : (unsigned int)(p.ldw * 2);
+    const unsigned int kst = __builtin_amdgcn_readfirstlane(panels ? 1024u : 64u);
     unsigned int a_off[3], b_off[3];
     auto set_offsets = [&](int ln) __attribute__((always_inline)) {
 #pragma unroll
@@ -76,12 +80,13 @@
             const int row = (wave + 8 * i) * 16 + (ln >> 2);
             const int c = (ln & 3) ^ ((row >> 2) & 2);
             a_off[i] = (unsigned int)row * (unsigned int)(p.lda * 2) + (c << 4);
-            b_off[i] = (unsigned int)w_row(row) * (unsigned int)(p.ldw * 2) + (c << 4);
+            const unsigned int wr = (unsigned int)w_row(row);
+            b_off[i] = (wr >> wp_shift) * wp_block + (wr & wp_mask) * 64u + (c << 4);
         }
     };
     set_offsets(lane);
     const u32x4 a_desc = raw_desc(p.A, (unsigned int)(((size_t)(p.M - 1) * p.lda + p.K) * 2));
-    const u32x4 b_desc = raw_desc(p.W, (unsigned int)(((size_t)(p.N - 1) * p.ldw + p.K) * 2));
+    const u32x4 b_desc = raw_desc(panels ? p.w_panels : p.W, (unsigned int)(((size_t)(p.N - 1) * p.ldw + p.K) * 2));
     const unsigned int a_tile = (unsigned int)(p.lda * 2) * BM, b_tile = (unsigned int)(p.ldw * 2) * BN;
     const int st1 = p.K >> 5;
     const unsigned int wbase = __builtin_amdgcn_readfirstlane((unsigned int)(uintptr_t)LDS_PTR(smem + wave * 1024));
@@ -110,7 +115,7 @@
     tile_of(blockIdx.x, tm0, tn0);
     bias_dma(tn0 * BN, 0);
     request_stage(tm0 * a_tile, tn0 * b_tile, 0);
-    request_stage(tm0 * a_tile + 64, tn0 * b_tile + 64, 1);
+    request_stage(tm0 * a_tile + 64, tn0 * b_tile + kst, 1);
     asm volatile("s_waitcnt vmcnt(0)" ::: "memory");
     __builtin_amdgcn_s_barrier();
     if (grp == 1) __builtin_amdgcn_s_barrier();
@@ -118,6 +123,7 @@
     auto core = [&](auto MIW_c, auto ROWW_c) __attribute__((always_inline)) {
         constexpr int MIW = decltype(MIW_c)::value;
         constexpr int DG = 2;
+        const unsigned int kstep[4] = {kst * DG, kst * (DG + 1), kst * (DG + 2), kst * (DG + 3)};
         const int row_w = decltype(ROWW_c)::value >= 0 ? decltype(ROWW_c)::value : wm * (MI0 * 16);
         f32x4 acc[MIW][NTW];
 #pragma unroll
@@ -136,7 +142,7 @@
             constexpr int J = decltype(J_c)::value;
             constexpr int NA = decltype(NA_c)::value, NB = decltype(NB_c)::value;
             constexpr int RS = (J + DG) & 3, KOFF = 64 * (J + DG);
-            const unsigned int rq_a = so_a + KOFF, rq_b = so_b + KOFF;
+            const unsigned int rq_a = so_a + KOFF, rq_b = so_b + kstep[J];
             unsigned int t_a = rd_a, t_b = rd_b;
             if constexpr (J != 0) {
                 asm volatile("v_add_u32 %0, %1, %2" : "=v"(t_a) : "n"(J * STG), "v"(rd_a));
@@ -190,15 +196,16 @@
         auto run_tile = [&](auto NA_c, auto NB_c, unsigned int sa, unsigned int sb, unsigned int san, unsigned int sbn) __attribute__((always_inline)) {
             using I0 = std::integral_constant<int, 0>; using I1 = std::integral_constant<int, 1>; using I2 = std::integral_constant<int, 2>; using I3 = std::integral_constant<int, 3>;
             const int ntrip = st1 >> 2;
+            const unsigned int ktrip = 4u * kst;
             unsigned int ra = sa, rb = sb;
             for (int t = 0; t < ntrip; ++t) {
                 const bool last = t == ntrip - 1;
-                const unsigned int ha = last ? san - 256u : ra, hb = last ? sbn - 256u : rb;
+                const unsigned int ha = last ? san - 256u : ra, hb = last ? sbn - ktrip : rb;
                 stage(I0{}, ra, rb, NA_c, NB_c);
                 stage(I1{}, ra, rb, NA_c, NB_c);
                 stage(I2{}, ha, hb, NA_c, NB_c);
                 stage(I3{}, ha, hb, NA_c, NB_c);
-                ra += 256; rb += 256;
+                ra += 256; rb += ktrip;
             }
         };
 
diff --git a/ullsam_amd/modeling/common.py b/ullsam_amd/modeling/common.py
--- a/ullsam_amd/modeling/common.py
+++ b/ullsam_amd/modeling/common.py
@@ -6,6 +6,7 @@
 from torch import nn
 
 from .. import ops
+from ..packing import pack_ring_panels
 
 
 class PackCache:
@@ -42,6 +43,14 @@
         return self.pk(name + ":cdt", p, lambda: p.detach().to(dtype).contiguous())
 
 
+def ring_panels(owner: "Packed", name: str, srcs, M: int, dtype, rows: Callable[[], torch.Tensor]) -> Optional[torch.Tensor]:
+    ps = (srcs,) if isinstance(srcs, torch.Tensor) else srcs
+    N, K = (sum(p.shape[0] for p in ps), ps[0].shape[1])
+    if not ops.ring_panels_wanted(M, N, K, dtype) or (torch.is_grad_enabled() and any(p.requires_grad for p in ps)):
+        return None
+    return owner.pk(f"{name}:panels:{dtype}", srcs, lambda: pack_ring_panels(rows()))
+
+
 class Linear(Packed):
 
     def __init__(self, in_features: int, out_features: int, bias: bool = True):
@@ -59,6 +68,9 @@
     def b(self):
         return None if self.bias is None else self.f32("b", self.bias)
 
+    def wp(self, dtype, M: int):
+        return ring_panels(self, "w", self.weight, M, dtype, lambda: self.w(dtype))
+
     def w8(self):
         pair = self.pk("w8", self.weight, lambda: ops.rows_fp8(self.weight.detach().contiguous()))
         return pair
@@ -75,7 +87,7 @@
 
     def forward(self, x: torch.Tensor) -> torch.Tensor:
         dt = self.weight.dtype
-        y = ops.gemm(ops.cast(x.reshape(-1, self.in_features).contiguous(), dt), self.w(dt), self.b())
+        y = ops.gemm(ops.cast(x.reshape(-1, self.in_features).contiguous(), dt), self.w(dt), self.b(), w_panels=self.wp(dt, x.numel() // self.in_features))
         return y.reshape(*x.shape[:-1], self.out_features)
 
 
@@ -125,6 +137,6 @@
 
     def forward(self, x: torch.Tensor) -> torch.Tensor:
         dt = self.lin1.weight.dtype
-        h = ops.gemm(ops.cast(x.reshape(-1, x.shape[-1]).contiguous(), dt), self.lin1.w(dt), self.lin1.b(), act=self.act_code)
-        y = ops.gemm(h, self.lin2.w(dt), self.lin2.b())
+        h = ops.gemm(ops.cast(x.reshape(-1, x.shape[-1]).contiguous(), dt), self.lin1.w(dt), self.lin1.b(), act=self.act_code, w_panels=self.lin1.wp(dt, x.numel() // x.shape[-1]))
+        y = ops.gemm(h, self.lin2.w(dt), self.lin2.b(), w_panels=self.lin2.wp(dt, h.shape[0]))
         return y.reshape(x.shape)
diff --git a/ullsam_amd/modeling/image_encoder.py b/ullsam_amd/modeling/image_encoder.py
--- a/ullsam_amd/modeling/image_encoder.py
+++ b/ullsam_amd/modeling/image_encoder.py
@@ -127,19 +127,19 @@
                 qkv = ops.gemm_fp8(q8, sa, *at.qkv.w8(), at.qkv.b())
             else:
                 xn = ops.norm(xres, *blk.norm1.wb(), blk.norm1.eps, dt)
-                qkv = ops.gemm(xn, at.qkv.w(dt), at.qkv.b())
+                qkv = ops.gemm(xn, at.qkv.w(dt), at.qkv.b(), w_panels=at.qkv.wp(dt, xn.shape[0]))
             qb = at.qkv.bias if at.qkv.bias is not None else torch.zeros(3 * D, device=x.device)
             n_rel = blk.window_size if blk.window_size > 0 else g
             att = ops.vit_attention(qkv, at.rel_table("rh", at.rel_pos_h, n_rel, dt), at.rel_table("rw", at.rel_pos_w, n_rel, dt), at.cdt("qb", qb, dt),
                                     B, self.num_heads, at.head_dim, g, g, blk.window_size)
-            ops.gemm(att, at.proj.w(dt), at.proj.b(), residual=xres, out_f32=True, out=xres)
+            ops.gemm(att, at.proj.w(dt), at.proj.b(), residual=xres, out_f32=True, out=xres, w_panels=at.proj.wp(dt, att.shape[0]))
             if fp8:
                 q8, sa = ops.rows_fp8(xres, *blk.norm2.wb(), blk.norm2.eps)
                 h = ops.gemm_fp8(q8, sa, *blk.mlp.lin1.w8(), blk.mlp.lin1.b(), act=blk.mlp.act_code)
             else:
                 xn = ops.norm(xres, *blk.norm2.wb(), blk.norm2.eps, dt)
-                h = ops.gemm(xn, blk.mlp.lin1.w(dt), blk.mlp.lin1.b(), act=blk.mlp.act_code)
-            ops.gemm(h, blk.mlp.lin2.w(dt), blk.mlp.lin2.b(), residual=xres, out_f32=True, out=xres)
+                h = ops.gemm(xn, blk.mlp.lin1.w(dt), blk.mlp.lin1.b(), act=blk.mlp.act_code, w_panels=blk.mlp.lin1.wp(dt, xn.shape[0]))
+            ops.gemm(h, blk.mlp.lin2.w(dt), blk.mlp.lin2.b(), residual=xres, out_f32=True, out=xres, w_panels=blk.mlp.lin2.wp(dt, h.shape[0]))
             if self.stage_probe is not None:
                 self.stage_probe(bi, xres)
         n0, n1, n2, n3 = self.neck[0], self.neck[1], self.neck[2], self.neck[3]
diff --git a/ullsam_amd/modeling/modeling_internlm2.py b/ullsam_amd/modeling/modeling_internlm2.py
--- a/ullsam_amd/modeling/modeling_internlm2.py
+++ b/ullsam_amd/modeling/modeling_internlm2.py
@@ -8,7 +8,7 @@
 from .. import ops
 from ..packing import pack_w13
 from ..sampling import row_seeds
-from .common import Linear, Packed
+from .common import Linear, Packed, ring_panels
 from .configuration_internlm2 import InternLM2Config
 from .outputs import BaseModelOutputWithPast, CausalLMOutputWithPast
 
@@ -38,6 +38,9 @@
 
     def w13(self, dt):
         return self.pk("w13", (self.w1.weight, self.w3.weight), lambda: pack_w13(self.w1.weight.detach().to(dt), self.w3.weight.detach().to(dt)))
+
+    def w13p(self, dt, M: int):
+        return ring_panels(self, "w13", (self.w1.weight, self.w3.weight), M, dt, lambda: self.w13(dt))
 
     def w13_w8d(self, dt):
         return self.pk("w13:w8d", (self.w1.weight, self.w3.weight), lambda: ops.rows_fp8_pow2(self.w13(dt)))
@@ -182,9 +185,9 @@
             else:
                 xn = ops.norm(x, layer.attention_norm.w(), None, layer.attention_norm.variance_epsilon, dt, rms=True)
                 if hd == 128 and S > 8:
-                    q = ops.gemm_qkv_rope(xn, at.wqkv.w(dt), at.wqkv.b(), kc, vc, pos, cos, sin, B, S, KVH, G, past)
+                    q = ops.gemm_qkv_rope(xn, at.wqkv.w(dt), at.wqkv.b(), kc, vc, pos, cos, sin, B, S, KVH, G, past, w_panels=at.wqkv.wp(dt, B * S))
                 else:
-                    qkv = ops.gemm(xn, at.wqkv.w(dt), at.wqkv.b())
+                    qkv = ops.gemm(xn, at.wqkv.w(dt), at.wqkv.b(), w_panels=at.wqkv.wp(dt, B * S))
                     q = ops.rope_split(qkv, kc, vc, pos, cos, sin, B, S, KVH, G, hd, past)
             if S > 1:
                 a = ops.causal_attention(q, kc, vc, key_mask, B, H, KVH, hd, S, Sk, past)
@@ -197,18 +200,18 @@
             if w8_wo:
                 ops.gemm_w8(a, *at.wo.w8d(), at.wo.b(), residual=x, out_f32=True, out=x)
             else:
-                ops.gemm(a, at.wo.w(dt), at.wo.b(), residual=x, out_f32=True, out=x)
+                ops.gemm(a, at.wo.w(dt), at.wo.b(), residual=x, out_f32=True, out=x, w_panels=at.wo.wp(dt, B * S))
             if w8:
                 hmid = ops.gemm_w8(x, *ff.w13_w8d(dt), act=ops.ACT_SWIGLU, norm_w=layer.ffn_norm.w(), eps=layer.ffn_norm.variance_epsilon)
             elif fused:
                 hmid = ops.gemm_rmsnorm(x, layer.ffn_norm.w(), layer.ffn_norm.variance_epsilon, ff.w13(dt), act=ops.ACT_SWIGLU)
             else:
                 xn = ops.norm(x, layer.ffn_norm.w(), None, layer.ffn_norm.variance_epsilon, dt, rms=True)
-                hmid = ops.gemm(xn, ff.w13(dt), act=ops.ACT_SWIGLU)
+                hmid = ops.gemm(xn, ff.w13(dt), act=ops.ACT_SWIGLU, w_panels=ff.w13p(dt, B * S))
             if w8_w2:
                 ops.gemm_w8(hmid, *ff.w2.w8d(), None, residual=x, out_f32=True, out=x)
             else:
-                ops.gemm(hmid, ff.w2.w(dt), None, residual=x, out_f32=True, out=x)
+                ops.gemm(hmid, ff.w2.w(dt), None, residual=x, out_f32=True, out=x, w_panels=ff.w2.wp(dt, B * S))
             if self.stage_probe is not None:
                 self.stage_probe(li, x)
         if cache is not None:
diff --git a/ullsam_amd/modeling/modeling_internvl_sam.py b/ullsam_amd/modeling/modeling_internvl_sam.py
--- a/ullsam_amd/modeling/modeling_internvl_sam.py
+++ b/ullsam_amd/modeling/modeling_internvl_sam.py
@@ -66,15 +66,15 @@
         dt = self.dtype
         ln, l1, l3 = self.mlp1[0], self.mlp1[1], self.mlp1[3]
         f = ops.pixel_shuffle_ln(img_tok, *ln.wb(), B, 64, 64, 256, ln.eps, dt)
-        h = ops.gemm(f, l1.w(dt), l1.b(), act=ops.ACT_GELU)
-        return ops.gemm(h, l3.w(dt), l3.b(), out_f32=True)
+        h = ops.gemm(f, l1.w(dt), l1.b(), act=ops.ACT_GELU, w_panels=l1.wp(dt, f.shape[0]))
+        return ops.gemm(h, l3.w(dt), l3.b(), out_f32=True, w_panels=l3.wp(dt, h.shape[0]))
 
     def _mlp2_tokens(self, rows: torch.Tensor, B: int) -> torch.Tensor:
         dt = self.dtype
         ln, l1, l3 = self.mlp2[0], self.mlp2[1], self.mlp2[3]
         f = ops.norm(rows, *ln.wb(), ln.eps, dt)
-        f = ops.gemm(f, l1.w(dt), l1.b(), act=ops.ACT_GELU)
-        f = ops.gemm(f, l3.w(dt), l3.b(), out_f32=True)
+        f = ops.gemm(f, l1.w(dt), l1.b(), act=ops.ACT_GELU, w_panels=l1.wp(dt, f.shape[0]))
+        f = ops.gemm(f, l3.w(dt), l3.b(), out_f32=True, w_panels=l3.wp(dt, f.shape[0]))
         return ops.pixel_unshuffle(f, B, 64, 64, 256)
 
     @torch.no_grad()
diff --git a/ullsam_amd/ops.py b/ullsam_amd/ops.py
--- a/ullsam_amd/ops.py
+++ b/ullsam_amd/ops.py
@@ -1,5 +1,6 @@
 from __future__ import annotations
 
+import os
 from typing import Optional
 
 import numpy as np
@@ -42,6 +43,18 @@
 
 _WS = {}
 
+_RING_PANELS = os.environ.get("ULLSAM_RING_PANELS", "1") != "0"
+
+
+def set_ring_panels(on: bool) -> None:
+    global _RING_PANELS
+    _RING_PANELS = bool(on)
+    _lib.call("ullsam_set_gemm_tuning", 4, 1 if on else 0)
+
+
+def ring_panels_wanted(M: int, N: int, K: int, dtype: torch.dtype) -> bool:
+    return _RING_PANELS and dtype == torch.bfloat16 and M >= 1024 and K >= 256 and K % 64 == 0 and (N % 256 == 0 or N % 320 == 0)
+
 
 def _gemm_workspace(device) -> torch.Tensor:
     key = (str(device), torch.cuda.current_stream().cuda_stream)
@@ -52,7 +65,8 @@
 
 
 def gemm(a: torch.Tensor, w: torch.Tensor, bias: Optional[torch.Tensor] = None, residual: Optional[torch.Tensor] = None,
-         act: int = ACT_NONE, out_f32: bool = False, out: Optional[torch.Tensor] = None, res_row_mod: int = 0, splitk_ok: bool = False) -> torch.Tensor:
+         act: int = ACT_NONE, out_f32: bool = False, out: Optional[torch.Tensor] = None, res_row_mod: int = 0, splitk_ok: bool = False,
+         w_panels: Optional[torch.Tensor] = None) -> torch.Tensor:
     _chk(a, "a"); _chk(w, "w", a.dtype)
     M, K = a.shape
     N = w.shape[0]
@@ -71,6 +85,12 @@
         _chk(residual, "residual", torch.float32)
         ldr = residual.shape[-1]
     ws = _gemm_workspace(a.device)
+    if w_panels is not None:
+        _chk(w_panels, "w_panels", torch.bfloat16)
+        assert w_panels.shape == w.shape and a.dtype == torch.bfloat16, (w_panels.shape, w.shape, a.dtype)
+        _lib.call("ullsam_gemm_panels", dt_code(a.dtype), a.data_ptr(), K, w.data_ptr(), K, w_panels.data_ptr(), out.data_ptr(), n_out, int(out_f32),
+                  _p(bias), _p(residual), ldr, res_row_mod, act | (ACT_SPLITK_OK if splitk_ok else 0), M, N, K, ws.data_ptr(), ws.numel(), _stream())
+        return out
     _lib.call("ullsam_gemm", dt_code(a.dtype), a.data_ptr(), K, w.data_ptr(), K, out.data_ptr(), n_out, int(out_f32),
               _p(bias), _p(residual), ldr, res_row_mod, act | (ACT_SPLITK_OK if splitk_ok else 0), M, N, K, ws.data_ptr(), ws.numel(), _stream())
     return out
@@ -431,7 +451,7 @@
 
 
 def gemm_qkv_rope(x: torch.Tensor, wqkv: torch.Tensor, bias: Optional[torch.Tensor], k_cache, v_cache, pos, cos_tab, sin_tab, B, S, KVH, G,
-                  cache_pos0) -> torch.Tensor:
+                  cache_pos0, w_panels: Optional[torch.Tensor] = None) -> torch.Tensor:
     _chk(x, "x"); _chk(wqkv, "wqkv", x.dtype); _chk(pos, "position_ids", torch.int32); _chk(cos_tab, "cos", torch.float32); _chk(sin_tab, "sin", torch.float32)
     _chk(k_cache, "k_cache", x.dtype); _chk(v_cache, "v_cache", x.dtype)
     K = x.shape[1]
@@ -440,6 +460,13 @@
         _chk(bias, "bias", torch.float32)
     q = torch.empty((B * S, KVH * G * 128), dtype=x.dtype, device=x.device)
     ws = _gemm_workspace(x.device)
+    if w_panels is not None:
+        _chk(w_panels, "w_panels", torch.bfloat16)
+        assert w_panels.shape == wqkv.shape and x.dtype == torch.bfloat16
+        _lib.call("ullsam_gemm_qkv_rope_panels", dt_code(x.dtype), x.data_ptr(), K, wqkv.data_ptr(), K, w_panels.data_ptr(), _p(bias), B, S, K, KVH, G, pos.data_ptr(),
+                  cos_tab.data_ptr(), sin_tab.data_ptr(), cos_tab.shape[0], q.data_ptr(), k_cache.data_ptr(), v_cache.data_ptr(), k_cache.shape[2],
+                  cache_pos0, ws.data_ptr(), ws.numel(), _stream())
+        return q
     _lib.call("ullsam_gemm_qkv_rope", dt_code(x.dtype), x.data_ptr(), K, wqkv.data_ptr(), K, _p(bias), B, S, K, KVH, G, pos.data_ptr(),
               cos_tab.data_ptr(), sin_tab.data_ptr(), cos_tab.shape[0], q.data_ptr(), k_cache.data_ptr(), v_cache.data_ptr(), k_cache.shape[2],
               cache_pos0, ws.data_ptr(), ws.numel(), _stream())
diff --git a/ullsam_amd/packing.py b/ullsam_amd/packing.py
--- a/ullsam_amd/packing.py
+++ b/ullsam_amd/packing.py
@@ -9,6 +9,22 @@
     return torch.stack([w1.reshape(I // 64, 64, K), w3.reshape(I // 64, 64, K)], dim=1).reshape(2 * I, K).contiguous()
 
 
+def pack_ring_panels(w: torch.Tensor) -> torch.Tensor:
+    N, K = w.shape
+    if w.dtype != torch.bfloat16 or N % 16 != 0 or K % 32 != 0:
+        raise ValueError(f"pack_ring_panels: bf16 [N, K] with N % 16 == 0 and K % 32 == 0 needed, got {w.dtype} {tuple(w.shape)}")
+    buf = torch.empty(N * K + 512, dtype=w.dtype, device=w.device)
+    skip = (-buf.data_ptr() % 1024) // 2
+    out = buf[skip:skip + N * K].view(N, K)
+    out.view(N // 16, K // 32, 16, 32).copy_(w.detach().reshape(N // 16, 16, K // 32, 32).permute(0, 2, 1, 3))
+    return out
+
+
+def unpack_ring_panels(p: torch.Tensor) -> torch.Tensor:
+    N, K = p.shape
+    return p.view(N // 16, K // 32, 16, 32).permute(0, 2, 1, 3).reshape(N, K).contiguous()
+
+
 def pack_conv3x3(w: torch.Tensor) -> torch.Tensor:
     return w.permute(0, 2, 3, 1).reshape(w.shape[0], -1).contiguous()
 
```
